# DeepakSridhar/fgdm

Hardware: AMD Instinct MI355X
Metric: 512x512 images/sec @ 50 DDIM steps, seg-ControlNet+CFG (higher is better)
Workload: dtype f16

## Files before the change

fgdm_amd/csrc/attention.hip:

```cpp
#include "common.h"
#include <type_traits>
#include <algorithm>
#include <stdlib.h>

#pragma clang diagnostic ignored "-Winline-asm"
#define ATT_THR 8.0f

template <int D>
__global__ __launch_bounds__(256) void attn_kernel(const half_t* __restrict__ Q, int ldq,
                                                   const half_t* __restrict__ K, int ldk,
                                                   const half_t* __restrict__ Vt, int ldvt,
                                                   half_t* __restrict__ O, int ldo,
                                                   int H, int T, int Tk, float sl2e) {
    constexpr int DP = (D + 15) / 16 * 16;
    constexpr int NKS = DP / 16;
    constexpr int DT = (D + 31) / 32;
    constexpr bool ONES = (DT * 32 > D);
    constexpr bool FOLD = (DP > D) && (D % 8 == 0);
    constexpr int PS = D / 16, PH = (D % 16) / 8;
    constexpr int KS = DP * 2 + 16;
    constexpr int VS = 64 * 2 + 8;
    constexpr int DC = D / 8;
    constexpr int KCH = (64 * DC + 255) / 256;
    constexpr int VCH = (D * 8 + 255) / 256;
    constexpr int KBYTES = 64 * KS, VBYTES = DT * 32 * VS;
    __shared__ __attribute__((aligned(16))) char smem[2 * (KBYTES + VBYTES)];

    const int tid = threadIdx.x, lane = tid & 63, wave = tid >> 6;
    const int lq = lane & 31, lh = lane >> 5;
    const int nqb = (T + 127) / 128;
    const int nb = gridDim.x;
    int logical;
    {
        const int bid = blockIdx.x, xcd = bid & 7, qd = nb >> 3, r = nb & 7;
        logical = (xcd < r ? xcd * (qd + 1) : r * (qd + 1) + (xcd - r) * qd) + (bid >> 3);
    }
    int qblk, b, head;
    if (Tk <= 128) {
        head = logical % H;
        const int rest = logical / H;
        qblk = rest % nqb; b = rest / nqb;
    } else {
        qblk = logical % nqb;
        const int bh = logical / nqb;
        b = bh / H; head = bh - b * H;
    }
    const int q = qblk * 128 + wave * 32 + lq;

    for (int buf = 0; buf < 2; ++buf) {
        char* Ksb = smem + buf * (KBYTES + VBYTES);
        char* Vsb = Ksb + KBYTES;
        if constexpr (DP > D) {
            for (int i = tid; i < 64 * (DP - D) / 8; i += 256) {
                const int key = i / ((DP - D) / 8), c = i % ((DP - D) / 8);
                h8 pad = (h8)(half_t)0;
                if (FOLD && c == 0) pad[0] = (half_t)1;
                *(h8*)(Ksb + key * KS + (D + c * 8) * 2) = pad;
            }
        }
        for (int i = tid; i < (DT * 32 - D) * 16; i += 256) {
            const int r = D + i / 16, c = i % 16;
            *(h4*)(Vsb + r * VS + c * 8) = (r == D) ? (h4)(half_t)1 : (h4)(half_t)0;
        }
    }

    h8 qf[NKS];
#pragma unroll
    for (int s = 0; s < NKS; ++s) {
        const int c = 16 * s + 8 * lh;
        qf[s] = (h8)(half_t)0;
        if (c < D && q < T) qf[s] = *(const h8*)(Q + ((size_t)b * T + q) * ldq + head * D + c);
        if constexpr (FOLD) {
#pragma unroll
            for (int j = 0; j < 8; ++j) qf[s][j] = (half_t)((float)qf[s][j] * sl2e);
        }
    }

    f32x16 oacc[DT];
#pragma unroll
    for (int t = 0; t < DT; ++t)
#pragma unroll
        for (int r = 0; r < 16; ++r) oacc[t][r] = 0.f;
    float m_run = FOLD ? 0.f : -INFINITY, l_run = 0.f;

    const half_t* Kb = K + (size_t)b * Tk * ldk + head * D;
    const half_t* Vb = Vt + ((size_t)b * H + head) * D * ldvt;

    const int wave_u = __builtin_amdgcn_readfirstlane(wave);
    int k_goff[KCH], k_loff[KCH], k_key[KCH], v_goff[VCH], v_loff[VCH];
#pragma unroll
    for (int u = 0; u < KCH; ++u) {
        const int i = tid + u * 256, key = i / DC, c = i - key * DC;
        k_key[u] = key; k_goff[u] = key * ldk + c * 8; k_loff[u] = key * KS + c * 16;
    }
#pragma unroll
    for (int u = 0; u < VCH; ++u) {
        const int i = tid + u * 256, r = i >> 3, c = i & 7;
        v_goff[u] = r * ldvt + c * 8; v_loff[u] = r * VS + c * 16;
    }
    h8 kreg[KCH], vreg[VCH];
    auto load_tile = [&](int k0, bool ragged) {
        const half_t* kb = Kb + (size_t)k0 * ldk;
        const half_t* vb = Vb + k0;
#pragma unroll
        for (int u = 0; u < KCH; ++u)
            if ((u * 4 + wave_u) * 64 < 64 * DC) {
                int off = k_goff[u];
                if (ragged) off += (min(k_key[u], Tk - 1 - k0) - k_key[u]) * ldk;
                kreg[u] = *(const h8*)(kb + off);
            }
#pragma unroll
        for (int u = 0; u < VCH; ++u)
            if ((u * 4 + wave_u) * 64 < D * 8) vreg[u] = *(const h8*)(vb + v_goff[u]);
    };
    auto store_tile = [&](auto bufc) {
        constexpr int buf = decltype(bufc)::value;
        char* Ksb = smem + buf * (KBYTES + VBYTES);
        char* Vsb = Ksb + KBYTES;
#pragma unroll
        for (int u = 0; u < KCH; ++u)
            if ((u * 4 + wave_u) * 64 < 64 * DC) *(h8*)(Ksb + k_loff[u]) = kreg[u];
#pragma unroll
        for (int u = 0; u < VCH; ++u)
            if ((u * 4 + wave_u) * 64 < D * 8) {
                const h8 v = vreg[u];
                h4 lo = {v[0], v[1], v[2], v[3]}, hi = {v[4], v[5], v[6], v[7]};
                *(h4*)(Vsb + v_loff[u]) = lo;
                *(h4*)(Vsb + v_loff[u] + 8) = hi;
            }
    };
    const int kfrag = lq * KS + 8 * lh * 2, vfrag = lq * VS + 4 * lh * 2;

    load_tile(0, Tk < 64);
    store_tile(std::integral_constant<int, 0>{});
    auto tile = [&](int k0, auto curc, auto nsubc) {
        constexpr int cur = decltype(curc)::value;
        constexpr int NSUB = decltype(nsubc)::value;
        const bool more = k0 + 64 < Tk;
        if (more) load_tile(k0 + 64, k0 + 128 > Tk);
        __syncthreads();
        const char* Ks = smem + cur * (KBYTES + VBYTES);
        const char* Vs = Ks + KBYTES;

        h8 kf[2][NKS];
#pragma unroll
        for (int sub = 0; sub < NSUB; ++sub)
#pragma unroll
            for (int s = 0; s < NKS; ++s) kf[sub][s] = *(const h8*)(Ks + kfrag + sub * 32 * KS + 16 * s * 2);
        __builtin_amdgcn_sched_barrier(0);
        f32x16 sacc[2];
#pragma unroll
        for (int sub = 0; sub < NSUB; ++sub) {
#pragma unroll
            for (int r = 0; r < 16; ++r) sacc[sub][r] = 0.f;
#pragma unroll
            for (int s = 0; s < NKS; ++s) sacc[sub] = __builtin_amdgcn_mfma_f32_32x32x16_f16(kf[sub][s], qf[s], sacc[sub], 0, 0, 0);
        }
        __builtin_amdgcn_sched_barrier(0);
        h4 v0f[2][2][DT], v1f[2][2][DT];
#pragma unroll
        for (int sub = 0; sub < NSUB; ++sub)
#pragma unroll
            for (int s = 0; s < 2; ++s)
#pragma unroll
                for (int t = 0; t < DT; ++t) {
                    const char* vp = Vs + vfrag + t * 32 * VS + (sub * 32 + 16 * s) * 2;
                    v0f[sub][s][t] = *(const h4*)vp;
                    v1f[sub][s][t] = *(const h4*)(vp + 16);
                }
        __builtin_amdgcn_sched_barrier(0);
        if (k0 + 64 > Tk) {
#pragma unroll
            for (int sub = 0; sub < NSUB; ++sub)
#pragma unroll
                for (int r = 0; r < 16; ++r) {
                    const int key = k0 + sub * 32 + (r & 3) + 8 * (r >> 2) + 4 * lh;
                    if (key >= Tk) sacc[sub][r] = -INFINITY;
                }
        }
        float psum = 0.f;
        if constexpr (FOLD) {
            float mx = sacc[0][0];
#pragma unroll
            for (int r = 1; r < 16; ++r) mx = fmaxf(mx, sacc[0][r]);
            if constexpr (NSUB == 2) {
#pragma unroll
                for (int r = 0; r < 16; ++r) mx = fmaxf(mx, sacc[1][r]);
            }
            mx = fmaxf(mx, __shfl_xor(mx, 32));
            const bool first = (k0 == 0);
            if (first || !__all(mx <= ATT_THR)) {
                const float m_new = first ? mx : m_run + fmaxf(mx, 0.f);
                const float m_hat = (float)(half_t)m_new;
                const float delta = m_run - m_hat;
                const float alpha = first ? 1.f : __builtin_amdgcn_exp2f(delta);
                m_run = m_hat;
#pragma unroll
                for (int t = 0; t < DT; ++t)
#pragma unroll
                    for (int r = 0; r < 16; ++r) oacc[t][r] *= alpha;
#pragma unroll
                for (int sub = 0; sub < NSUB; ++sub)
#pragma unroll
                    for (int r = 0; r < 16; ++r) sacc[sub][r] += delta;
                if (lh == PH) qf[PS][0] = (half_t)(-m_hat);
            }
#pragma unroll
            for (int sub = 0; sub < NSUB; ++sub)
#pragma unroll
                for (int r = 0; r < 16; ++r) sacc[sub][r] = __builtin_amdgcn_exp2f(sacc[sub][r]);
        } else {
        float mx = sacc[0][0];
#pragma unroll
        for (int r = 1; r < 16; ++r) mx = fmaxf(mx, sacc[0][r]);
        if constexpr (NSUB == 2) {
#pragma unroll
            for (int r = 0; r < 16; ++r) mx = fmaxf(mx, sacc[1][r]);
        }
        mx = fmaxf(mx, __shfl_xor(mx, 32)) * sl2e;
        if (!__all(mx - m_run <= ATT_THR)) {
            const float m_new = fmaxf(m_run, mx);
            const float alpha = __builtin_amdgcn_exp2f(m_run - m_new);
            m_run = m_new;
            l_run *= alpha;
#pragma unroll
            for (int t = 0; t < DT; ++t)
#pragma unroll
                for (int r = 0; r < 16; ++r) oacc[t][r] *= alpha;
        }
#pragma unroll
        for (int sub = 0; sub < NSUB; ++sub)
#pragma unroll
            for (int r = 0; r < 16; ++r) {
                const float p = __builtin_amdgcn_exp2f(sacc[sub][r] * sl2e - m_run);
                sacc[sub][r] = p;
                if constexpr (!ONES) psum += p;
            }
        }
        if constexpr (!ONES) l_run += psum;

#pragma unroll
        for (int sub = 0; sub < NSUB; ++sub) {
#pragma unroll
            for (int s = 0; s < 2; ++s) {
                h8 pf;
#pragma unroll
                for (int j = 0; j < 8; ++j) pf[j] = (half_t)sacc[sub][8 * s + j];
#pragma unroll
                for (int t = 0; t < DT; ++t) {
                    const h4 v0 = v0f[sub][s][t], v1 = v1f[sub][s][t];
                    const h8 vf = {v0[0], v0[1], v0[2], v0[3], v1[0], v1[1], v1[2], v1[3]};
                    oacc[t] = __builtin_amdgcn_mfma_f32_32x32x16_f16(vf, pf, oacc[t], 0, 0, 0);
                }
            }
        }
        if (more) store_tile(std::integral_constant<int, cur ^ 1>{});
    };
    using one_t = std::integral_constant<int, 1>;
    using two_t = std::integral_constant<int, 2>;
    for (int k0 = 0; k0 < Tk; k0 += 128) {
        if (k0 + 32 >= Tk) tile(k0, std::integral_constant<int, 0>{}, one_t{});
        else tile(k0, std::integral_constant<int, 0>{}, two_t{});
        if (k0 + 64 < Tk) {
            if (k0 + 96 >= Tk) tile(k0 + 64, std::integral_constant<int, 1>{}, one_t{});
            else tile(k0 + 64, std::integral_constant<int, 1>{}, two_t{});
        }
    }

    float l_tot;
    if constexpr (ONES) {
        constexpr int rr = D % 32;
        constexpr int reg = (rr & 3) + 4 * (rr >> 3);
        constexpr int owner_half = (rr >> 2) & 1;
        const float mine = oacc[D / 32][reg];
        const float other = __shfl_xor(mine, 32);
        l_tot = (lh == owner_half) ? mine : other;
    } else {
        l_tot = l_run + __shfl_xor(l_run, 32);
    }
    const float inv = 1.0f / l_tot;
    if (q < T) {
        half_t* op = O + ((size_t)b * T + q) * ldo + head * D;
#pragma unroll
        for (int t = 0; t < DT; ++t)
#pragma unroll
            for (int g = 0; g < 4; ++g) {
                const int dd = t * 32 + 8 * g + 4 * lh;
                if (dd < D) {
                    h4 pk = {(half_t)(oacc[t][4 * g] * inv), (half_t)(oacc[t][4 * g + 1] * inv),
                             (half_t)(oacc[t][4 * g + 2] * inv), (half_t)(oacc[t][4 * g + 3] * inv)};
                    *(h4*)(op + dd) = pk;
                }
            }
    }
}


template <int D>
__global__ __launch_bounds__(256) void attn_cross_kernel(const half_t* __restrict__ Q, int ldq,
                                                         const half_t* __restrict__ K, int ldk,
                                                         const half_t* __restrict__ Vt, int ldvt,
                                                         half_t* __restrict__ O, int ldo,
                                                         int H, int T, int Tk, float sl2e, int cpw) {
    constexpr int NS = 3, KEYS = NS * 32;
    constexpr int DP = (D + 15) / 16 * 16, NKS = DP / 16, DT = (D + 31) / 32;
    constexpr bool ONES = (DT * 32 > D);
    constexpr bool FOLD = (DP > D) && (D % 8 == 0);
    constexpr int KS = DP * 2 + 16;
    constexpr int VS = KEYS * 2 + 72;
    constexpr int DC = D / 8;
    constexpr bool RELAY = D <= 80;
    constexpr int RS = D * 2 + 8;
    constexpr int PCS = 32 * (D / 8), KP = (PCS + 63) / 64;
    __shared__ __attribute__((aligned(16))) char smem[KEYS * KS + DT * 32 * VS + (RELAY ? 4 * 32 * RS : 0)];
    char* Ks = smem;
    char* Vs = smem + KEYS * KS;

    const int tid = threadIdx.x, lane = tid & 63, wave = tid >> 6;
    const int lq = lane & 31, lh = lane >> 5;
    const int qpw = 128 * cpw;
    const int ncb = (T + qpw - 1) / qpw;
    const int nb = gridDim.x;
    int logical;
    {
        const int bid = blockIdx.x, xcd = bid & 7, qd = nb >> 3, r = nb & 7;
        logical = (xcd < r ? xcd * (qd + 1) : r * (qd + 1) + (xcd - r) * qd) + (bid >> 3);
    }
    const int head = logical % H, rest = logical / H;
    const int cblk = rest % ncb, b = rest / ncb;

    const half_t* Kb = K + (size_t)b * Tk * ldk + head * D;
    const half_t* Vb = Vt + ((size_t)b * H + head) * D * ldvt;
    constexpr int KPC = KEYS * (DP / 8), VPC = DT * 32 * (KEYS / 8);
    constexpr int KPT = (KPC + 255) / 256, VPT = (VPC + 255) / 256;
    h8 kst[KPT], vst[VPT];
#pragma unroll
    for (int u = 0; u < KPT; ++u) {
        const int i = tid + 256 * u, key = i / (DP / 8), c = i - key * (DP / 8);
        kst[u] = (h8)(half_t)0;
        if (i < KPC && c < DC) kst[u] = *(const h8*)(Kb + (size_t)min(key, Tk - 1) * ldk + c * 8);
    }
#pragma unroll
    for (int u = 0; u < VPT; ++u) {
        const int i = tid + 256 * u, r = i / (KEYS / 8), c = i - r * (KEYS / 8);
        vst[u] = (r == D) ? (h8)(half_t)1 : (h8)(half_t)0;
        if (i < VPC && r < D) vst[u] = *(const h8*)(Vb + (size_t)r * ldvt + c * 8);
    }
    char* scr = smem + KEYS * KS + DT * 32 * VS + (threadIdx.x >> 6) * 32 * RS;
    constexpr int NQ = RELAY ? KP : NKS;
    auto load_q = [&](int q0, h8 (&qr)[NQ]) {
        if constexpr (RELAY) {
#pragma unroll
            for (int u = 0; u < KP; ++u) {
                const int c = lane + 64 * u, row = c / (D / 8), ck = c - row * (D / 8);
                qr[u] = (h8)(half_t)0;
                if (c < PCS && q0 + row < T) qr[u] = *(const h8*)(Q + ((size_t)b * T + q0 + row) * ldq + head * D + ck * 8);
            }
        } else {
#pragma unroll
            for (int s2 = 0; s2 < NKS; ++s2) {
                const int c = 16 * s2 + 8 * lh;
                qr[s2] = (h8)(half_t)0;
                if (c < D && q0 + lq < T) qr[s2] = *(const h8*)(Q + ((size_t)b * T + q0 + lq) * ldq + head * D + c);
            }
        }
    };
    const int q_first = cblk * qpw + wave * 32;
    h8 qn[NQ];
    load_q(q_first, qn);
#pragma unroll
    for (int u = 0; u < KPT; ++u) {
        const int i = tid + 256 * u, key = i / (DP / 8), c = i - key * (DP / 8);
        if (i < KPC) *(h8*)(Ks + key * KS + c * 16) = kst[u];
    }
#pragma unroll
    for (int u = 0; u < VPT; ++u) {
        const int i = tid + 256 * u, r = i / (KEYS / 8), c = i - r * (KEYS / 8);
        if (i < VPC) {
            const h8 v = vst[u];
            const h4 lo = {v[0], v[1], v[2], v[3]}, hi = {v[4], v[5], v[6], v[7]};
            *(h4*)(Vs + r * VS + c * 16) = lo;
            *(h4*)(Vs + r * VS + c * 16 + 8) = hi;
        }
    }
    __syncthreads();

    const int kfrag = lq * KS + 8 * lh * 2, vfrag = lq * VS + 4 * lh * 2;
    for (int i = 0; i < cpw; ++i) {
        const int q0 = __builtin_amdgcn_readfirstlane(q_first + i * 128);
        if (q0 >= T) break;
        const int q = q0 + lq;
        h8 qf[NKS];
        if constexpr (RELAY) {
#pragma unroll
            for (int u = 0; u < KP; ++u) {
                const int c = lane + 64 * u, row = c / (D / 8), ck = c - row * (D / 8);
                if (c < PCS) {
                    const h4 lo = {qn[u][0], qn[u][1], qn[u][2], qn[u][3]}, hi = {qn[u][4], qn[u][5], qn[u][6], qn[u][7]};
                    *(h4*)(scr + row * RS + ck * 16) = lo;
                    *(h4*)(scr + row * RS + ck * 16 + 8) = hi;
                }
            }
            asm volatile("s_waitcnt lgkmcnt(0)" ::: "memory");
#pragma unroll
            for (int s2 = 0; s2 < NKS; ++s2) {
                const int c = 16 * s2 + 8 * lh;
                qf[s2] = (h8)(half_t)0;
                if (c < D) {
                    const h4 lo = *(const h4*)(scr + lq * RS + c * 2), hi = *(const h4*)(scr + lq * RS + c * 2 + 8);
                    qf[s2] = h8{lo[0], lo[1], lo[2], lo[3], hi[0], hi[1], hi[2], hi[3]};
                }
            }
            asm volatile("s_waitcnt lgkmcnt(0)" ::: "memory");
        } else {
#pragma unroll
            for (int s2 = 0; s2 < NKS; ++s2) qf[s2] = qn[s2];
        }
        if (i + 1 < cpw) load_q(q0 + 128, qn);
        if constexpr (FOLD) {
#pragma unroll
            for (int s2 = 0; s2 < NKS; ++s2)
#pragma unroll
                for (int j = 0; j < 8; ++j) qf[s2][j] = (half_t)((float)qf[s2][j] * sl2e);
        }
        f32x16 sacc[NS];
#pragma unroll
        for (int sub = 0; sub < NS; ++sub) {
#pragma unroll
            for (int r = 0; r < 16; ++r) sacc[sub][r] = 0.f;
#pragma unroll
            for (int s2 = 0; s2 < NKS; ++s2) {
                const h8 kf = *(const h8*)(Ks + kfrag + sub * 32 * KS + 16 * s2 * 2);
                sacc[sub] = __builtin_amdgcn_mfma_f32_32x32x16_f16(kf, qf[s2], sacc[sub], 0, 0, 0);
            }
        }
#pragma unroll
        for (int r = 0; r < 16; ++r) {
            const int key = (NS - 1) * 32 + (r & 3) + 8 * (r >> 2) + 4 * lh;
            if (key >= Tk) sacc[NS - 1][r] = -INFINITY;
        }
        float mx = sacc[0][0];
#pragma unroll
        for (int sub = 0; sub < NS; ++sub)
#pragma unroll
            for (int r = 0; r < 16; ++r) mx = fmaxf(mx, sacc[sub][r]);
        mx = fmaxf(mx, __shfl_xor(mx, 32));
        const float sc = FOLD ? 1.0f : sl2e;
        float psum = 0.f;
#pragma unroll
        for (int sub = 0; sub < NS; ++sub)
#pragma unroll
            for (int r = 0; r < 16; ++r) {
                const float pv = __builtin_amdgcn_exp2f((sacc[sub][r] - mx) * sc);
                sacc[sub][r] = pv;
                if constexpr (!ONES) psum += pv;
            }
        f32x16 oacc[DT];
#pragma unroll
        for (int t = 0; t < DT; ++t)
#pragma unroll
            for (int r = 0; r < 16; ++r) oacc[t][r] = 0.f;
#pragma unroll
        for (int sub = 0; sub < NS; ++sub)
#pragma unroll
            for (int s2 = 0; s2 < 2; ++s2) {
                h8 pf;
#pragma unroll
                for (int j = 0; j < 8; ++j) pf[j] = (half_t)sacc[sub][8 * s2 + j];
#pragma unroll
                for (int t = 0; t < DT; ++t) {
                    const char* vp = Vs + vfrag + t * 32 * VS + (sub * 32 + 16 * s2) * 2;
                    const h4 v0 = *(const h4*)vp, v1 = *(const h4*)(vp + 16);
                    const h8 vf = {v0[0], v0[1], v0[2], v0[3], v1[0], v1[1], v1[2], v1[3]};
                    oacc[t] = __builtin_amdgcn_mfma_f32_32x32x16_f16(vf, pf, oacc[t], 0, 0, 0);
                }
            }
        float l_tot;
        if constexpr (ONES) {
            constexpr int rr = D % 32;
            constexpr int reg = (rr & 3) + 4 * (rr >> 3);
            constexpr int owner_half = (rr >> 2) & 1;
            const float mine = oacc[D / 32][reg];
            const float other = __shfl_xor(mine, 32);
            l_tot = (lh == owner_half) ? mine : other;
        } else {
            l_tot = psum + __shfl_xor(psum, 32);
        }
        const float inv = 1.0f / l_tot;
        if constexpr (RELAY) {
#pragma unroll
            for (int t = 0; t < DT; ++t)
#pragma unroll
                for (int g = 0; g < 4; ++g) {
                    const int dd = t * 32 + 8 * g + 4 * lh;
                    if (dd < D) {
                        h4 pk = {(half_t)(oacc[t][4 * g] * inv), (half_t)(oacc[t][4 * g + 1] * inv),
                                 (half_t)(oacc[t][4 * g + 2] * inv), (half_t)(oacc[t][4 * g + 3] * inv)};
                        *(h4*)(scr + lq * RS + dd * 2) = pk;
                    }
                }
            asm volatile("s_waitcnt lgkmcnt(0)" ::: "memory");
#pragma unroll
            for (int u = 0; u < KP; ++u) {
                const int c = lane + 64 * u, row = c / (D / 8), ck = c - row * (D / 8);
                if (c < PCS && q0 + row < T) {
                    const h4 lo = *(const h4*)(scr + row * RS + ck * 16), hi = *(const h4*)(scr + row * RS + ck * 16 + 8);
                    *(h8*)(O + ((size_t)b * T + q0 + row) * ldo + head * D + ck * 8) = h8{lo[0], lo[1], lo[2], lo[3], hi[0], hi[1], hi[2], hi[3]};
                }
            }
            asm volatile("s_waitcnt lgkmcnt(0)" ::: "memory");
        } else if (q < T) {
            half_t* op = O + ((size_t)b * T + q) * ldo + head * D;
#pragma unroll
            for (int t = 0; t < DT; ++t)
#pragma unroll
                for (int g = 0; g < 4; ++g) {
                    const int dd = t * 32 + 8 * g + 4 * lh;
                    if (dd < D) {
                        h4 pk = {(half_t)(oacc[t][4 * g] * inv), (half_t)(oacc[t][4 * g + 1] * inv),
                                 (half_t)(oacc[t][4 * g + 2] * inv), (half_t)(oacc[t][4 * g + 3] * inv)};
                        *(h4*)(op + dd) = pk;
                    }
                }
        }
    }
}

template <int D>
__global__ __launch_bounds__(512) void attn_pp_kernel(const half_t* __restrict__ Q, int ldq,
                                                      const half_t* __restrict__ K, int ldk,
                                                      const half_t* __restrict__ Vt, int ldvt,
                                                      half_t* __restrict__ O, int ldo,
                                                      int H, int T, int Tk, float sl2e) {
    constexpr int DP = (D + 15) / 16 * 16, NKS = DP / 16, DT = (D + 31) / 32;
    constexpr bool ONES = (DT * 32 > D);
    constexpr bool FOLD = (DP > D) && (D % 8 == 0);
    constexpr int PS = D / 16, PH = (D % 16) / 8;
    constexpr int KS = DP * 2 + 16, VS = 64 * 2 + 8, DC = D / 8;
    constexpr int NCH = 64 * DC;
    constexpr int CH = (NCH + 511) / 512;
    constexpr int KBYTES = 64 * KS, VBYTES = DT * 32 * VS, PAIR = KBYTES + VBYTES;
    __shared__ __attribute__((aligned(16))) char smem[2 * PAIR];

    const int tid = threadIdx.x, lane = tid & 63;
    const int wave = __builtin_amdgcn_readfirstlane(tid >> 6);
    const int grp = wave >> 2;
    const int lq = lane & 31, lh = lane >> 5;
    const int nqb = (T + 255) / 256;
    const int nb = gridDim.x;
    int logical;
    {
        const int bid = blockIdx.x, xcd = bid & 7, qd = nb >> 3, r = nb & 7;
        logical = (xcd < r ? xcd * (qd + 1) : r * (qd + 1) + (xcd - r) * qd) + (bid >> 3);
    }
    const int qblk = logical % nqb, bh = logical / nqb;
    const int b = bh / H, head = bh - b * H;
    const int q = qblk * 256 + wave * 32 + lq;
    const int nt = (Tk + 63) / 64;

    for (int buf = 0; buf < 2; ++buf) {
        char* Ksb = smem + buf * PAIR;
        char* Vsb = Ksb + KBYTES;
        if constexpr (DP > D) {
            for (int i = tid; i < 64 * (DP - D) / 8; i += 512) {
                const int key = i / ((DP - D) / 8), c = i % ((DP - D) / 8);
                h8 pad = (h8)(half_t)0;
                if (FOLD && c == 0) pad[0] = (half_t)1;
                *(h8*)(Ksb + key * KS + (D + c * 8) * 2) = pad;
            }
        }
        for (int i = tid; i < (DT * 32 - D) * 16; i += 512) {
            const int r = D + i / 16, c = i % 16;
            *(h4*)(Vsb + r * VS + c * 8) = (r == D) ? (h4)(half_t)1 : (h4)(half_t)0;
        }
    }

    h8 qf[NKS];
#pragma unroll
    for (int s = 0; s < NKS; ++s) {
        const int c = 16 * s + 8 * lh;
        qf[s] = (h8)(half_t)0;
        if (c < D && q < T) qf[s] = *(const h8*)(Q + ((size_t)b * T + q) * ldq + head * D + c);
        if constexpr (FOLD) {
#pragma unroll
            for (int j = 0; j < 8; ++j) qf[s][j] = (half_t)((float)qf[s][j] * sl2e);
        }
    }
    f32x16 oacc[DT];
#pragma unroll
    for (int t = 0; t < DT; ++t)
#pragma unroll
        for (int r = 0; r < 16; ++r) oacc[t][r] = 0.f;
    float m_run = FOLD ? 0.f : -INFINITY, l_run = 0.f;

    const half_t* Kb = K + (size_t)b * Tk * ldk + head * D;
    const half_t* Vb = Vt + ((size_t)b * H + head) * D * ldvt;

    int k_goff[CH], k_loff[CH], k_key[CH], v_goff[CH], v_loff[CH];
#pragma unroll
    for (int u = 0; u < CH; ++u) {
        const int i = tid + u * 512;
        const int key = i / DC, c = i - key * DC;
        k_key[u] = key; k_goff[u] = key * ldk + c * 8; k_loff[u] = key * KS + c * 16;
        const int r = i >> 3, cv = i & 7;
        v_goff[u] = r * ldvt + cv * 8; v_loff[u] = r * VS + cv * 16;
    }
    h8 kreg[CH], vreg[CH];
    auto load_pair = [&](int kt, int vtile) {
        if (kt < nt) {
            const int k0 = kt * 64;
            const half_t* kb = Kb + (size_t)k0 * ldk;
            const bool ragged = k0 + 64 > Tk;
#pragma unroll
            for (int u = 0; u < CH; ++u)
                if ((u * 8 + wave) * 64 < NCH) {
                    int off = k_goff[u];
                    if (ragged) off += (min(k_key[u], Tk - 1 - k0) - k_key[u]) * ldk;
                    kreg[u] = *(const h8*)(kb + off);
                }
        }
        if (vtile >= 0 && vtile < nt) {
            const half_t* vb = Vb + vtile * 64;
#pragma unroll
            for (int u = 0; u < CH; ++u)
                if ((u * 8 + wave) * 64 < NCH) vreg[u] = *(const h8*)(vb + v_goff[u]);
        }
    };
    auto store_pair = [&](int kt, int vtile, int buf) {
        char* Ksb = smem + buf * PAIR;
        char* Vsb = Ksb + KBYTES;
        if (kt < nt) {
#pragma unroll
            for (int u = 0; u < CH; ++u)
                if ((u * 8 + wave) * 64 < NCH) *(h8*)(Ksb + k_loff[u]) = kreg[u];
        }
        if (vtile >= 0 && vtile < nt) {
#pragma unroll
            for (int u = 0; u < CH; ++u)
                if ((u * 8 + wave) * 64 < NCH) {
                    const h8 v = vreg[u];
                    h4 lo = {v[0], v[1], v[2], v[3]}, hi = {v[4], v[5], v[6], v[7]};
                    *(h4*)(Vsb + v_loff[u]) = lo;
                    *(h4*)(Vsb + v_loff[u] + 8) = hi;
                }
        }
    };
    auto barrier = [&]() { __syncthreads(); };
    const int kfrag = lq * KS + 8 * lh * 2, vfrag = lq * VS + 4 * lh * 2;

    f32x16 sacc[2];
    h8 pf[2][2];
    auto qk = [&](int buf) {
        const char* Ks = smem + buf * PAIR;
        h8 kf[2][NKS];
#pragma unroll
        for (int sub = 0; sub < 2; ++sub)
#pragma unroll
            for (int s = 0; s < NKS; ++s) kf[sub][s] = *(const h8*)(Ks + kfrag + sub * 32 * KS + 16 * s * 2);
        __builtin_amdgcn_sched_barrier(0);
#pragma unroll
        for (int sub = 0; sub < 2; ++sub) {
#pragma unroll
            for (int r = 0; r < 16; ++r) sacc[sub][r] = 0.f;
#pragma unroll
            for (int s = 0; s < NKS; ++s) sacc[sub] = __builtin_amdgcn_mfma_f32_32x32x16_f16(kf[sub][s], qf[s], sacc[sub], 0, 0, 0);
        }
    };
    auto pv = [&](int buf) {
        const char* Vs = smem + buf * PAIR + KBYTES;
#pragma unroll
        for (int sub = 0; sub < 2; ++sub)
#pragma unroll
            for (int s = 0; s < 2; ++s)
#pragma unroll
                for (int t = 0; t < DT; ++t) {
                    const char* vp = Vs + vfrag + t * 32 * VS + (sub * 32 + 16 * s) * 2;
                    const h4 v0 = *(const h4*)vp, v1 = *(const h4*)(vp + 16);
                    const h8 vf = {v0[0], v0[1], v0[2], v0[3], v1[0], v1[1], v1[2], v1[3]};
                    oacc[t] = __builtin_amdgcn_mfma_f32_32x32x16_f16(vf, pf[sub][s], oacc[t], 0, 0, 0);
                }
    };
    auto softmax = [&](int k0, bool first) {
// ... 264 lines not shown
        if constexpr ((ABL & 2) != 0) return;
        if (first || !__all(mx <= ATT_THR)) {
            const float m_new = first ? mx : m_run[X] + fmaxf(mx, 0.f);
            const float m_hat = (float)(half_t)m_new;
            const float delta = m_run[X] - m_hat;
            m_run[X] = m_hat;
            if (!first) {
                const float alpha = __builtin_amdgcn_exp2f(delta);
#pragma unroll
                for (int qg = 0; qg < 2; ++qg) {
                    const float aq = __shfl(alpha, 16 * qg + n16);
#pragma unroll
                    for (int t = 0; t < DT; ++t) oacc[X][t][qg] *= aq;
                }
            }
#pragma unroll
            for (int sub = 0; sub < 2; ++sub)
#pragma unroll
                for (int r = 0; r < 16; ++r) sacc[X][sub][r] += delta;
            if (h == PH) qf[X][PS][0] = (half_t)(-m_hat);
        }
    };
    auto expo = [&](int X, int sub, int r0, int r1) {
#pragma unroll
        for (int r = r0; r < r1; ++r) sacc[X][sub][r] = (ABL & 1) ? sacc[X][sub][r] : __builtin_amdgcn_exp2f(sacc[X][sub][r]);
    };
    auto pack = [&](int X, int sub) {
        unsigned pk[8];
#pragma unroll
        for (int i = 0; i < 8; ++i) {
            const h2 t2 = {(half_t)sacc[X][sub][2 * i], (half_t)sacc[X][sub][2 * i + 1]};
            pk[i] = __builtin_bit_cast(unsigned, t2);
        }
        u32x4 lo, hi;
#pragma unroll
        for (int i = 0; i < 4; ++i) {
            const auto r2 = __builtin_amdgcn_permlane16_swap(pk[i], pk[i + 4], false, false);
            lo[i] = r2[0]; hi[i] = r2[1];
        }
        pb[X][sub][0] = __builtin_bit_cast(h8, lo);
        pb[X][sub][1] = __builtin_bit_cast(h8, hi);
    };

    auto tile = [&](int kt, auto slotc) {
        constexpr int slot = decltype(slotc)::value;
        if (!(ABL & 4) && kt + 1 < nt) att_wait_vmcnt<NI>(); else att_wait_vmcnt<0>();
        __builtin_amdgcn_s_waitcnt(0xC07F);
        __builtin_amdgcn_s_barrier();
        if (!(ABL & 4) && kt + 2 < nt) issue(kt + 2, std::integral_constant<int, (slot + 2) % NSLOT>{});
        const char* sl = smem + slot * SLOT;
        const bool first = kt == 0;
#pragma unroll
        for (int sub = 0; sub < 2; ++sub)
#pragma unroll
            for (int s = 0; s < NKS; ++s) rd_k(sl, sub, s);
        ATT_SB();
#pragma unroll
        for (int sub = 0; sub < 2; ++sub)
#pragma unroll
            for (int s = 0; s < NKS; ++s) {
                qk(0, sub, s);
                if (sub * NKS + s < DT * 2) rd_v(sl, (sub * NKS + s) % DT, (sub * NKS + s) / DT);
                ATT_SB();
            }
        float mx = sacc[0][0][0];
        qk(1, 0, 0); mx = max_part(0, 0, mx); ATT_SB();
        qk(1, 0, 1); mx = max_part(0, 1, mx); ATT_SB();
        qk(1, 0, 2 % NKS); mx = max_cross(mx); ATT_SB();
#pragma unroll
        for (int s = 3; s < NKS; ++s) { qk(1, 0, s); ATT_SB(); }
        decide(0, mx, first);
        ATT_SB();
#pragma unroll
        for (int s = 0; s < NKS; ++s) {
            qk(1, 1, s);
            expo(0, 0, 16 * s / NKS, 16 * (s + 1) / NKS);
            ATT_SB();
        }
        pack(0, 0);
        ATT_SB();
        float mxb = sacc[1][0][0];
#pragma unroll
        for (int t = 0; t < DT; ++t)
#pragma unroll
            for (int qg = 0; qg < 2; ++qg) {
                const int i = t * 2 + qg, n = DT * 2;
                pv(0, 0, t, qg);
                expo(0, 1, 16 * i / n, 16 * (i + 1) / n);
                if (i == 1) mxb = max_part(1, 0, mxb);
                if (i == 3) mxb = max_part(1, 1, mxb);
                if (i == 4) mxb = max_cross(mxb);
                ATT_SB();
            }
        pack(0, 1);
        ATT_SB();
        decide(1, mxb, first);
        ATT_SB();
#pragma unroll
        for (int t = 0; t < DT; ++t)
#pragma unroll
            for (int qg = 0; qg < 2; ++qg) {
                const int i = t * 2 + qg, n = DT * 2;
                pv(0, 1, t, qg);
                expo(1, 0, 16 * i / n, 16 * (i + 1) / n);
                ATT_SB();
            }
        pack(1, 0);
        ATT_SB();
#pragma unroll
        for (int t = 0; t < DT; ++t)
#pragma unroll
            for (int qg = 0; qg < 2; ++qg) {
                const int i = t * 2 + qg, n = DT * 2;
                pv(1, 0, t, qg);
                expo(1, 1, 16 * i / n, 16 * (i + 1) / n);
                ATT_SB();
            }
        pack(1, 1);
        ATT_SB();
#pragma unroll
        for (int t = 0; t < DT; ++t)
#pragma unroll
            for (int qg = 0; qg < 2; ++qg) pv(1, 1, t, qg);
        ATT_SB();
    };
    for (int kt = 0; kt < nt; kt += NSLOT) {
        tile(kt, std::integral_constant<int, 0>{});
        if (kt + 1 < nt) tile(kt + 1, std::integral_constant<int, 1>{});
        if (kt + 2 < nt) tile(kt + 2, std::integral_constant<int, 2>{});
    }
#undef ATT_SB

    constexpr int LT = D / 16, LG = (D % 16) / 4, LR = D % 4;
#pragma unroll
    for (int X = 0; X < 2; ++X)
#pragma unroll
        for (int qg = 0; qg < 2; ++qg) {
            const float l = __shfl(oacc[X][LT][qg][LR], 16 * LG + n16);
            const float inv = 1.0f / l;
            half_t* op = O + ((size_t)b * T + q0w + 32 * X + 16 * qg + n16) * ldo + head * D;
#pragma unroll
            for (int t = 0; t < DT; ++t) {
                const int dd = 16 * t + 4 * g;
                if (dd < D) {
                    const h4 o4 = {(half_t)(oacc[X][t][qg][0] * inv), (half_t)(oacc[X][t][qg][1] * inv),
                                   (half_t)(oacc[X][t][qg][2] * inv), (half_t)(oacc[X][t][qg][3] * inv)};
                    *(h4*)(op + dd) = o4;
                }
            }
        }
}

template <int D, int NW, int ABL = 0>
__global__ __launch_bounds__(NW * 64, D <= 40 ? 2 : 1) void attn_dq32_kernel(const half_t* __restrict__ Q, int ldq,
                                                           const half_t* __restrict__ K, int ldk,
                                                           const half_t* __restrict__ Vt, int ldvt,
                                                           half_t* __restrict__ O, int ldo,
                                                           int H, int T, int Tk, float sl2e) {
    constexpr int DP = (D + 16) / 16 * 16, NKS = DP / 16;
    constexpr int DT = (D + 32) / 32;
    constexpr int DC = D / 8;
    constexpr int PS = D / 16, PH = (D % 16) / 8;
    constexpr int KROW = DC * 16, KBYTES = 64 * KROW, VDATA = D * 128, VBYTES = DT * 32 * 128, SLOT = KBYTES + VBYTES;
    constexpr int NSLOT = 3;
    constexpr int NDMA = (KBYTES + VDATA) / 1024, NI = (NDMA + NW - 1) / NW;
    static_assert(KBYTES % 1024 == 0 && VDATA % 1024 == 0 && NDMA >= NW, "whole wave-instructions per image");
    constexpr int ROT = (KROW / 4) % 8 == 4 ? 0 : DC / 2;
    static_assert(ROT == 0 || ((KROW / 4) % 16 == 8 && DC % 2 == 0), "K row stride");
    __shared__ __attribute__((aligned(1024))) char smem[NSLOT * SLOT + 64];

    const int tid = threadIdx.x, lane = tid & 63;
    const int wave = __builtin_amdgcn_readfirstlane(tid >> 6);
    const int n32 = lane & 31, h = lane >> 5;
    const int nqb = T / (NW * 64);
    const int nb = gridDim.x;
    int logical;
    {
        const int bid = blockIdx.x, xcd = bid & 7, qd = nb >> 3, r = nb & 7;
        logical = (xcd < r ? xcd * (qd + 1) : r * (qd + 1) + (xcd - r) * qd) + (bid >> 3);
    }
    const int qblk = logical % nqb, bh = logical / nqb;
    const int b = bh / H, head = bh - b * H;
    const int q0w = qblk * (NW * 64) + wave * 64;
    const int nt = Tk >> 6;

    char* const cst = smem + NSLOT * SLOT;
    if (tid < 2) {
        h8 v = (h8)(half_t)0;
        if (tid == 0) v[0] = (half_t)1;
        *(h8*)(cst + tid * 16) = v;
    }
    for (int i = tid; i < NSLOT * (DT * 32 - D) * 8; i += NW * 64) {
        const int sl_i = i / ((DT * 32 - D) * 8), rem = i - sl_i * ((DT * 32 - D) * 8), row = D + rem / 8, pc = rem & 7;
        *(h8*)(smem + sl_i * SLOT + KBYTES + row * 128 + pc * 16) = row == D ? (h8)(half_t)1 : (h8)(half_t)0;
    }

    const half_t* Kb = K + (size_t)b * Tk * ldk + head * D;
    const half_t* Vb = Vt + ((size_t)b * H + head) * D * ldvt;
    unsigned voff[NI], ldst[NI];
    bool isk[NI];
#pragma unroll
    for (int u = 0; u < NI; ++u) {
        int j = wave + NW * u;
        if (j >= NDMA) j -= NW;
        isk[u] = j < KBYTES / 1024;
        ldst[u] = (unsigned)j * 1024u;
        if (isk[u]) {
            const int L = 64 * j + lane, rp = L / DC, c = L - rp * DC;
            const int rho = rp & 31, a = rho >> 3;
            const int key = (rp & 32) + 16 * (a >> 1) + 8 * ((rho >> 2) & 1) + 4 * (a & 1) + (rho & 3);
            const int cs = (c + DC - ROT * ((rho >> 3) & 1)) % DC;
            voff[u] = (unsigned)(key * ldk + cs * 8) * 2u;
        } else {
            const int L = 64 * (j - KBYTES / 1024) + lane, d = L >> 3, x = L & 7;
            voff[u] = (unsigned)(d * ldvt + ((x ^ ((d >> 1) & 7)) * 8)) * 2u;
        }
    }
    const unsigned lds0 = (unsigned)(size_t)(__attribute__((address_space(3))) const void*)smem;
    auto issue = [&](int t, auto slotc) {
        const char* kb = (const char*)(Kb + (size_t)t * 64 * ldk);
        const char* vb = (const char*)(Vb + t * 64);
        const unsigned base = lds0 + (unsigned)decltype(slotc)::value * SLOT;
#pragma unroll
        for (int u = 0; u < NI; ++u) att_dma16(voff[u], isk[u] ? kb : vb, base + ldst[u]);
    };
    issue(0, std::integral_constant<int, 0>{});
    if (nt > 1) issue(1, std::integral_constant<int, 1>{});

    h8 qf[2][NKS];
#pragma unroll
    for (int X = 0; X < 2; ++X)
#pragma unroll
        for (int s = 0; s < NKS; ++s) {
            const int c = 16 * s + 8 * h;
            qf[X][s] = (h8)(half_t)0;
            if (c < D) qf[X][s] = *(const h8*)(Q + ((size_t)b * T + q0w + 32 * X + n32) * ldq + head * D + c);
#pragma unroll
            for (int e = 0; e < 8; ++e) qf[X][s][e] = (half_t)((float)qf[X][s][e] * sl2e);
        }
    f32x16 oacc[2][DT];
#pragma unroll
    for (int X = 0; X < 2; ++X)
#pragma unroll
        for (int t = 0; t < DT; ++t)
#pragma unroll
            for (int r = 0; r < 16; ++r) oacc[X][t][r] = 0.f;
    float m_run[2] = {0.f, 0.f};

    int k_lane[NKS];
#pragma unroll
    for (int s2 = 0; s2 < NKS; ++s2) k_lane[s2] = n32 * KROW + ((2 * s2 + h + ROT * ((n32 >> 3) & 1)) % DC) * 16;
    int v_lane[2][2];
#pragma unroll
    for (int sub = 0; sub < 2; ++sub)
#pragma unroll
        for (int s2 = 0; s2 < 2; ++s2) v_lane[sub][s2] = KBYTES + n32 * 128 + (((4 * sub + 2 * s2 + h) ^ ((n32 >> 1) & 7)) * 16);
    const char* const c_one = cst, *const c_zero = cst + 16;

    f32x16 sacc[2][2];
    h8 kf[2][NKS], vf[DT][2][2], pf[2][2][2];
    const f32x16 zero16 = {0.f, 0.f, 0.f, 0.f, 0.f, 0.f, 0.f, 0.f, 0.f, 0.f, 0.f, 0.f, 0.f, 0.f, 0.f, 0.f};
#define ATT_SB() __builtin_amdgcn_sched_barrier(0)
    auto rd_k = [&](const char* sl, int sub, int s) {
        const int ci0 = 2 * s;
        const char* p = sl + k_lane[s] + sub * 32 * KROW;
        if (ci0 + 1 >= DC) {
            const char* cp0 = ci0 < DC ? p : (ci0 == DC ? c_one : c_zero);
            const char* cp1 = ci0 + 1 == DC ? c_one : c_zero;
            p = h ? cp1 : cp0;
        }
        kf[sub][s] = *(const h8*)p;
    };
    auto rd_v = [&](const char* sl, int t, int sub, int s2) { vf[t][sub][s2] = *(const h8*)(sl + v_lane[sub][s2] + t * 32 * 128); };
    auto qk = [&](int X, int sub, int s) {
        if constexpr ((ABL & 32) != 0) { if (s == 0) asm volatile("" : "=v"(sacc[X][sub])); return; }
        sacc[X][sub] = __builtin_amdgcn_mfma_f32_32x32x16_f16(kf[sub][s], qf[X][s], s == 0 ? zero16 : sacc[X][sub], 0, 0, 0);
    };
    auto pv = [&](int X, int sub, int t, int s2) {
        if constexpr ((ABL & 16) != 0) { asm volatile("" : "+v"(oacc[X][t]) : "v"(vf[t][sub][s2]), "v"(pf[X][sub][s2])); return; }
        oacc[X][t] = __builtin_amdgcn_mfma_f32_32x32x16_f16(vf[t][sub][s2], pf[X][sub][s2], oacc[X][t], 0, 0, 0);
    };
    auto max_part = [&](int X, int sub, float mx) {
        if constexpr ((ABL & 2) != 0) return mx;
#pragma unroll
        for (int r = 0; r < 16; r += 2) mx = fmaxf(fmaxf(mx, sacc[X][sub][r]), sacc[X][sub][r + 1]);
        return mx;
    };
    auto max_cross = [&](float mx) {
        float lo = mx, hi = mx;
        asm volatile("s_nop 1\n\tv_permlane32_swap_b32 %0, %1" : "+v"(lo), "+v"(hi));
        return fmaxf(lo, hi);
    };
    auto decide = [&](int X, float mx, bool first) {
        if constexpr ((ABL & 2) != 0) return;
        if (first || !__all(mx <= ATT_THR)) {
            const float m_new = first ? mx : m_run[X] + fmaxf(mx, 0.f);
            const float m_hat = (float)(half_t)m_new;
            const float delta = m_run[X] - m_hat;
            m_run[X] = m_hat;
            if (!first) {
                const float alpha = __builtin_amdgcn_exp2f(delta);
#pragma unroll
                for (int t = 0; t < DT; ++t)
#pragma unroll
                    for (int r = 0; r < 16; ++r) oacc[X][t][r] *= alpha;
            }
#pragma unroll
            for (int sub = 0; sub < 2; ++sub)
#pragma unroll
                for (int r = 0; r < 16; ++r) sacc[X][sub][r] += delta;
            if (h == PH) qf[X][PS][0] = (half_t)(-m_hat);
        }
    };
    auto expo = [&](int X, int sub, int r0, int r1) {
#pragma unroll
        for (int r = r0; r < r1; ++r) sacc[X][sub][r] = (ABL & 1) ? sacc[X][sub][r] : __builtin_amdgcn_exp2f(sacc[X][sub][r]);
    };
    auto pack = [&](int X, int sub) {
#pragma unroll
        for (int s2 = 0; s2 < 2; ++s2)
#pragma unroll
            for (int e = 0; e < 8; ++e) pf[X][sub][s2][e] = (half_t)sacc[X][sub][8 * s2 + e];
    };
    constexpr int NPV = DT * 2;
    auto tile = [&](int kt, auto slotc) {
        constexpr int slot = decltype(slotc)::value;
        if (!(ABL & 4) && kt + 1 < nt) att_wait_vmcnt<NI>(); else att_wait_vmcnt<0>();
        __builtin_amdgcn_s_waitcnt(0xC07F);
        __builtin_amdgcn_s_barrier();
        if (!(ABL & 4) && kt + 2 < nt) issue(kt + 2, std::integral_constant<int, (slot + 2) % NSLOT>{});
        const char* sl = smem + slot * SLOT;
        const bool first = kt == 0;
#pragma unroll
        for (int sub = 0; sub < 2; ++sub)
#pragma unroll
            for (int s = 0; s < NKS; ++s) rd_k(sl, sub, s);
        ATT_SB();
#pragma unroll
        for (int sub = 0; sub < 2; ++sub)
#pragma unroll
            for (int s = 0; s < NKS; ++s) {
                const int i = sub * NKS + s;
                qk(0, sub, s);
                if (i < NPV) rd_v(sl, i / 2, 0, i & 1);
                ATT_SB();
            }
        float mx = sacc[0][0][0];
        qk(1, 0, 0); mx = max_part(0, 0, mx); ATT_SB();
        qk(1, 0, 1); mx = max_part(0, 1, mx); ATT_SB();
        qk(1, 0, 2 % NKS); mx = max_cross(mx); ATT_SB();
#pragma unroll
        for (int s = 3; s < NKS; ++s) { qk(1, 0, s); ATT_SB(); }
        decide(0, mx, first);
        ATT_SB();
#pragma unroll
        for (int s = 0; s < NKS; ++s) {
            qk(1, 1, s);
            expo(0, 0, 16 * s / NKS, 16 * (s + 1) / NKS);
            if (s < NPV) rd_v(sl, s / 2, 1, s & 1);
            ATT_SB();
        }
#pragma unroll
        for (int i = NKS; i < NPV; ++i) rd_v(sl, i / 2, 1, i & 1);
        pack(0, 0);
        ATT_SB();
        float mxb = sacc[1][0][0];
#pragma unroll
        for (int i = 0; i < NPV; ++i) {
            pv(0, 0, i / 2, i & 1);
            expo(0, 1, 16 * i / NPV, 16 * (i + 1) / NPV);
            if (i == NPV - 3) mxb = max_part(1, 0, mxb);
            if (i == NPV - 2) mxb = max_part(1, 1, mxb);
            if (i == NPV - 1) mxb = max_cross(mxb);
            ATT_SB();
        }
        pack(0, 1);
        ATT_SB();
        decide(1, mxb, first);
        ATT_SB();
#pragma unroll
        for (int i = 0; i < NPV; ++i) {
            pv(0, 1, i / 2, i & 1);
            expo(1, 0, 16 * i / NPV, 16 * (i + 1) / NPV);
            ATT_SB();
        }
        pack(1, 0);
        ATT_SB();
#pragma unroll
        for (int i = 0; i < NPV; ++i) {
            pv(1, 0, i / 2, i & 1);
            expo(1, 1, 16 * i / NPV, 16 * (i + 1) / NPV);
            ATT_SB();
        }
        pack(1, 1);
        ATT_SB();
#pragma unroll
        for (int i = 0; i < NPV; ++i) pv(1, 1, i / 2, i & 1);
        ATT_SB();
    };
    for (int kt = 0; kt < nt; kt += NSLOT) {
        tile(kt, std::integral_constant<int, 0>{});
        if (kt + 1 < nt) tile(kt + 1, std::integral_constant<int, 1>{});
        if (kt + 2 < nt) tile(kt + 2, std::integral_constant<int, 2>{});
    }
#undef ATT_SB

    constexpr int rr = D % 32, reg = (rr & 3) + 4 * (rr >> 3), owner_half = (rr >> 2) & 1;
#pragma unroll
    for (int X = 0; X < 2; ++X) {
        const float mine = oacc[X][D / 32][reg];
        const float other = __shfl_xor(mine, 32);
        const float inv = 1.0f / (h == owner_half ? mine : other);
        half_t* op = O + ((size_t)b * T + q0w + 32 * X + n32) * ldo + head * D;
#pragma unroll
        for (int t = 0; t < DT; ++t)
#pragma unroll
            for (int g4 = 0; g4 < 4; ++g4) {
                const int dd = t * 32 + 8 * g4 + 4 * h;
                if (dd < D) {
                    const h4 o4 = {(half_t)(oacc[X][t][4 * g4] * inv), (half_t)(oacc[X][t][4 * g4 + 1] * inv),
                                   (half_t)(oacc[X][t][4 * g4 + 2] * inv), (half_t)(oacc[X][t][4 * g4 + 3] * inv)};
                    *(h4*)(op + dd) = o4;
                }
            }
    }
}

int attention_launch(const half_t* Q, int ldq, const half_t* K, int ldk, const half_t* Vt, int ldvt, half_t* O,
                     int ldo, int B, int H, int T, int Tk, int d, int q_prescaled, hipStream_t s) {
    if (B <= 0 || H <= 0 || T <= 0 || Tk <= 0) return FGDM_ERR_ARG;
    if (ldvt < (Tk + 63) / 64 * 64 || (ldvt & 7) || (ldq & 7) || (ldk & 7) || (ldo & 3)) return FGDM_ERR_ARG;
    const float sl2e = q_prescaled ? 1.0f : 1.4426950408889634f / sqrtf((float)d);
    static const bool pp_on = !(getenv("FGDM_ATTN_PP") && atoi(getenv("FGDM_ATTN_PP")) == 0);
    static const int dq = getenv("FGDM_ATTN_DQ") ? atoi(getenv("FGDM_ATTN_DQ")) : 3;
    if (dq > 0 && d == 40 && T % 256 == 0 && Tk % 64 == 0 && Tk >= 128 && (size_t)64 * ldk * 2 < (1u << 31) &&
        (size_t)d * ldvt * 2 < (1u << 31)) {
        const dim3 gridq((T / 256) * H * B), blockq(256);
        static const int abl = getenv("FGDM_ATTN_ABL") ? atoi(getenv("FGDM_ATTN_ABL")) : 0;
        if (abl) {
            switch (abl + (dq == 3 ? 1000 : 0)) {
#define ATT_ABL_CASE(v) case v: FGDM_LAUNCH((attn_dq_kernel<40, 4, v>), gridq, blockq, 0, s, Q, ldq, K, ldk, Vt, ldvt, O, ldo, H, T, Tk, sl2e); break; \
                        case 1000 + v: FGDM_LAUNCH((attn_dq32_kernel<40, 4, v>), gridq, blockq, 0, s, Q, ldq, K, ldk, Vt, ldvt, O, ldo, H, T, Tk, sl2e); break;
                ATT_ABL_CASE(1) ATT_ABL_CASE(2) ATT_ABL_CASE(3) ATT_ABL_CASE(4) ATT_ABL_CASE(16) ATT_ABL_CASE(32) ATT_ABL_CASE(48) ATT_ABL_CASE(51) ATT_ABL_CASE(7)
#undef ATT_ABL_CASE
                default: return FGDM_ERR_ARG;
            }
            return hipGetLastError() == hipSuccess ? FGDM_OK : FGDM_ERR_HIP;
        }
        if (dq == 1) FGDM_LAUNCH((attn_dq_kernel<40, 4>), gridq, blockq, 0, s, Q, ldq, K, ldk, Vt, ldvt, O, ldo, H, T, Tk, sl2e);
        else FGDM_LAUNCH((attn_dq32_kernel<40, 4>), gridq, blockq, 0, s, Q, ldq, K, ldk, Vt, ldvt, O, ldo, H, T, Tk, sl2e);
        return hipGetLastError() == hipSuccess ? FGDM_OK : FGDM_ERR_HIP;
    }
    static const int dq80 = getenv("FGDM_ATTN_DQ80") ? atoi(getenv("FGDM_ATTN_DQ80")) : 1;
    if (dq80 > 0 && d == 80 && T % 256 == 0 && Tk % 64 == 0 && Tk >= 128 && (size_t)64 * ldk * 2 < (1u << 31) &&
        (size_t)d * ldvt * 2 < (1u << 31)) {
        const dim3 gridq((T / 256) * H * B), blockq(256);
        FGDM_LAUNCH((attn_dq32_kernel<80, 4>), gridq, blockq, 0, s, Q, ldq, K, ldk, Vt, ldvt, O, ldo, H, T, Tk, sl2e);
        return hipGetLastError() == hipSuccess ? FGDM_OK : FGDM_ERR_HIP;
    }
    if (pp_on && T >= 256 && Tk >= 256 && (d == 40 || d == 80)) {
        const dim3 grid2(((T + 255) / 256) * H * B), block2(512);
        if (d == 40) FGDM_LAUNCH(attn_pp_kernel<40>, grid2, block2, 0, s, Q, ldq, K, ldk, Vt, ldvt, O, ldo, H, T, Tk, sl2e);
        else FGDM_LAUNCH(attn_pp_kernel<80>, grid2, block2, 0, s, Q, ldq, K, ldk, Vt, ldvt, O, ldo, H, T, Tk, sl2e);
        return hipGetLastError() == hipSuccess ? FGDM_OK : FGDM_ERR_HIP;
    }
    static const int cross = getenv("FGDM_ATTN_CROSS") ? atoi(getenv("FGDM_ATTN_CROSS")) : 4;
    if (cross > 0 && Tk > 64 && Tk <= 96 && ldvt >= 96 && T >= 128) {
        const int cpw = std::min(cross, T / 128);
        const dim3 gridc(((T + 128 * cpw - 1) / (128 * cpw)) * H * B), blockc(256);
        switch (d) {
            case 40: FGDM_LAUNCH(attn_cross_kernel<40>, gridc, blockc, 0, s, Q, ldq, K, ldk, Vt, ldvt, O, ldo, H, T, Tk, sl2e, cpw); break;
            case 80: FGDM_LAUNCH(attn_cross_kernel<80>, gridc, blockc, 0, s, Q, ldq, K, ldk, Vt, ldvt, O, ldo, H, T, Tk, sl2e, cpw); break;
            case 160: FGDM_LAUNCH(attn_cross_kernel<160>, gridc, blockc, 0, s, Q, ldq, K, ldk, Vt, ldvt, O, ldo, H, T, Tk, sl2e, cpw); break;
            default: return FGDM_ERR_ARG;
        }
        return hipGetLastError() == hipSuccess ? FGDM_OK : FGDM_ERR_HIP;
    }
    const dim3 grid(((T + 127) / 128) * H * B), block(256);
    switch (d) {
        case 40: FGDM_LAUNCH(attn_kernel<40>, grid, block, 0, s, Q, ldq, K, ldk, Vt, ldvt, O, ldo, H, T, Tk, sl2e); break;
        case 80: FGDM_LAUNCH(attn_kernel<80>, grid, block, 0, s, Q, ldq, K, ldk, Vt, ldvt, O, ldo, H, T, Tk, sl2e); break;
        case 160: FGDM_LAUNCH(attn_kernel<160>, grid, block, 0, s, Q, ldq, K, ldk, Vt, ldvt, O, ldo, H, T, Tk, sl2e); break;
        default: return FGDM_ERR_ARG;
    }
    return hipGetLastError() == hipSuccess ? FGDM_OK : FGDM_ERR_HIP;
}
```

fgdm_amd/csrc/common.h:

```cpp
#pragma once
#include <hip/hip_runtime.h>
#include <stdint.h>

typedef _Float16 half_t;
typedef _Float16 h8 __attribute__((ext_vector_type(8)));
typedef _Float16 h4 __attribute__((ext_vector_type(4)));
typedef _Float16 h2 __attribute__((ext_vector_type(2)));
typedef float f32x16 __attribute__((ext_vector_type(16)));
typedef float f32x4 __attribute__((ext_vector_type(4)));

__device__ __forceinline__ float gelu_f(float x) {
    const float z = fminf(fabsf(x), 6.0f);
    float p = -4.7132482596e-04f;
    p = __builtin_fmaf(p, z, 7.0652551839e-03f);
    p = __builtin_fmaf(p, z, -5.1762067461e-02f);
    p = __builtin_fmaf(p, z, -4.6008771426e-01f);
    p = __builtin_fmaf(p, z, -1.1507295505e+00f);
    p = __builtin_fmaf(p, z, -4.8959157159e-05f - 1.0f);
    const float t = __builtin_amdgcn_exp2f(p);
    return __builtin_fmaf(fabsf(x), 0.5f - t, 0.5f * x);
}

typedef float f32x2 __attribute__((ext_vector_type(2)));
__device__ __forceinline__ f32x2 gelu2_f(f32x2 x) {
    const f32x2 ax = {fabsf(x[0]), fabsf(x[1])};
    const f32x2 z = {fminf(ax[0], 6.0f), fminf(ax[1], 6.0f)};
    auto c = [](float k) { return f32x2{k, k}; };
    f32x2 p = c(-4.7132482596e-04f);
    p = __builtin_elementwise_fma(p, z, c(7.0652551839e-03f));
    p = __builtin_elementwise_fma(p, z, c(-5.1762067461e-02f));
    p = __builtin_elementwise_fma(p, z, c(-4.6008771426e-01f));
    p = __builtin_elementwise_fma(p, z, c(-1.1507295505e+00f));
    p = __builtin_elementwise_fma(p, z, c(-4.8959157159e-05f - 1.0f));
    const f32x2 t = {__builtin_amdgcn_exp2f(p[0]), __builtin_amdgcn_exp2f(p[1])};
    return __builtin_elementwise_fma(ax, c(0.5f) - t, c(0.5f) * x);
}

__device__ __forceinline__ float silu_f(float x, float k = 1.0f) {
    return x * __builtin_amdgcn_rcpf(1.0f + __builtin_amdgcn_exp2f(-1.4426950408889634f * k * x));
}

#define FGDM_OK 0
#define FGDM_ERR_ARG -1
#define FGDM_ERR_HIP -2
#define FGDM_ERR_STATE -3
#define FGDM_ERR_NOMEM -4

enum IgemmMode { IG_LINEAR = 0, IG_CONV3 = 1, IG_CONV3_S2 = 2, IG_CONV3_UP2 = 3, IG_CONV3_S2_BR = 4 };
enum IgemmAct { ACT_NONE = 0, ACT_SILU = 1, ACT_RELU = 2, ACT_GEGLU = 3, ACT_QGELU = 4  };
enum IgemmOut { OUT_F16 = 0, OUT_F32 = 1, OUT_F32_NCHW = 2, OUT_F16_T = 3 };

struct IgemmArgs {
    const half_t* A0;
    const half_t* A1;
    const half_t* Wt;
    const float* bias;
    const float* rowvec;
    const half_t* resid;
    void* out;
    const half_t* zero;
    int C0, C1;
    int B, H, W;
    int Ho, Wo;
    int M, N;
    int K;
    int mode, act, out_kind;
    int ld_out, ld_res;
    int rv_stride;
    int rows_per_sample;
    float scale;
    int force_cfg;
    int splitk;
    float* ws;
    int debug;
    const float* ln_stats;
    const float* ln_u;
    int ln_slots;
    float ln_eps;
    float* stats_out;
    void* out2;
    int split_n, out_kind2, ld_out2;
};

int igemm_launch(const IgemmArgs& a, hipStream_t s);
void igemm_set_force_cfg(int cfg);
void igemm_set_twin_layers(bool on);
void igemm_set_pair_hint(int mult);
int igemm2_launch(const IgemmArgs& a, int cfg, hipStream_t s);
int igemm_stats_slots(const IgemmArgs& a);
int row_stats_slots(int C);
int row_stats_launch(const half_t* x, int rows, int C, float* stats , hipStream_t s);
int igemm_splitk_factor(const IgemmArgs& a);
int igemm_splitk_reduce(const IgemmArgs& a, hipStream_t s);
size_t igemm_npad(int n);

void groupnorm_set_group(bool on);
int groupnorm_launch(const half_t* x0, int C0, const half_t* x1, int C1, int B, int HW,
                     const float* gamma, const float* beta, float eps, int silu,
                     half_t* out, float* ws , hipStream_t s);
size_t groupnorm_ws_floats(int B, int HW);
int layernorm_launch(const half_t* x, int rows, int C, const float* gamma, const float* beta, float eps,
                     half_t* out, hipStream_t s);

int attention_launch(const half_t* Q, int ldq, const half_t* K, int ldk, const half_t* Vt, int ldvt,
                     half_t* O, int ldo, int B, int H, int T, int Tk, int d, int q_prescaled, hipStream_t s);

int nchw_f32_to_nhwc_f16(const float* x, half_t* y, int B, int C, int HW, int Cpad, hipStream_t s);
int f32_to_f16(const float* x, half_t* y, size_t n, hipStream_t s);
int silu_f32_to_f16(const float* x, half_t* y, size_t n, hipStream_t s);
int nhwc_f16_to_nchw_f32(const half_t* x, float* y, int B, int C, int HW, hipStream_t s);
int im2col3x3(const half_t* x, half_t* A, int B, int H, int W, int C, int stride, int Kpad, hipStream_t s);
int avgpool2(const half_t* x, half_t* y, int B, int H, int W, int C, hipStream_t s);
int add_f16(const half_t* a, const half_t* b, half_t* y, size_t n, hipStream_t s);
int add_f16_to_f32(const float* a, const half_t* b, float* y, size_t n, hipStream_t s);
int timestep_embed(const int64_t* t, const float* t_float, half_t* y, int B, int dim, int rows_pad, hipStream_t s);
int vae_prequant(const float* z, const float* wb, float scale, half_t* y, int B, int HW, hipStream_t s);
int vae_moments(const float* h, const float* wb, float* moments, int B, int HW, hipStream_t s);
int posterior_sample(const float* moments, const float* noise, float scale, float* z, int B, int zc, int HW, hipStream_t s);
int softmax_rows(const float* S, half_t* P, int rows, int cols, hipStream_t s);
int image_to_u8(const float* x, uint8_t* y, int B, int C, int HW, int mode, hipStream_t s);
int resize_linear_u8(const uint8_t* src, uint8_t* dst, int B, int H, int W, int C, int Ho, int Wo, hipStream_t s);
int u8_to_hint(const uint8_t* src, float* dst, int B, int HW, int C, hipStream_t s);
int embed_tokens(const int64_t* ids, const float* tok, const float* pos, float* out, int rows, int T, int W, int vocab,
                 hipStream_t s);
int layernorm32_launch(const float* x, int rows, int C, const float* gamma, const float* beta, float eps, half_t* out16,
                       float* out32, hipStream_t s);
int f16_to_f32(const half_t* x, float* y, size_t n, hipStream_t s);
int small_attention_launch(const half_t* qkv, int ld, int koff, int voff, half_t* out, int ldo, int B, int heads, int T,
                           int d, int causal, hipStream_t s);
int transpose_pad_keys(const half_t* v, half_t* vt, int B, int Tk, int C, int Tkpad, hipStream_t s);
int ddim_step(const float* x, const float* e_cond, const float* e_uncond, float cfg_scale,
              float a_t, float a_prev, float sigma_t, float sqrt_one_minus_at, const float* noise,
              float* x_prev, float* pred_x0, float* e_out, size_t n, hipStream_t s);
int plms_combine(const float* e_t, const float* e1, const float* e2, const float* e3, int order,
                 float* e_prime, size_t n, hipStream_t s);
int axpby(const float* a, float ca, const float* b, float cb, float* y, size_t n, hipStream_t s);
int mask_blend(const float* a, const float* b, const float* m, float* y, size_t n, hipStream_t s);
int ancestral_step(const float* x, const float* eps, float sqrt_recip, float sqrt_recipm1, float coef1, float coef2,
                   float std, const float* noise, float* out, size_t n, hipStream_t s);

#define HIP_TRY(expr) do { hipError_t _e = (expr); if (_e != hipSuccess) return FGDM_ERR_HIP; } while (0)

#include <functional>
#define FGDM_MAX_GROUP 5
typedef int (*IgemmGroupFn)(const IgemmArgs* const* a, int n, unsigned grid_x, hipStream_t s);
bool fgdm_recording();
void fgdm_record(std::function<int(hipStream_t)> run, const void* pair_key = nullptr, IgemmGroupFn pair = nullptr,
                 const IgemmArgs* ia = nullptr, unsigned grid_x = 0);
#define FGDM_GROUP_BLOB 96
typedef int (*GenericGroupFn)(const void* const* args, int n, unsigned grid_x, hipStream_t s);
void fgdm_record_generic(std::function<int(hipStream_t)> run, const void* key, GenericGroupFn fn, const void* args, size_t nbytes,
                         unsigned grid_x, unsigned long long shape);
#define FGDM_LAUNCH(kernel, grid, block, smem, stream, ...)                                                                  \
    do {                                                                                                                     \
        if (fgdm_recording()) {                                                                                              \
            fgdm_record([=](hipStream_t fgdm_s_) -> int {                                                                    \
                hipLaunchKernelGGL(kernel, grid, block, smem, fgdm_s_, __VA_ARGS__);                                         \
                return hipGetLastError() == hipSuccess ? FGDM_OK : FGDM_ERR_HIP;                                             \
            });                                                                                                              \
        } else {                                                                                                             \
            hipLaunchKernelGGL(kernel, grid, block, smem, stream, __VA_ARGS__);                                              \
        }                                                                                                                    \
    } while (0)
```

fgdm_amd/csrc/engine.hip:

```cpp
#include "common.h"
#include "../../include/fgdm.h"

#include <algorithm>
#include <array>
#include <cmath>
#include <cstdlib>
#include <cstdio>
#include <cstring>
#include <map>
#include <memory>
#include <string>
#include <unordered_map>
#include <vector>

namespace {

struct Arena {
    struct Blk { char* p; size_t sz; bool free; };
    std::vector<std::vector<Blk>> slabs;
    std::vector<char*> bases;
    size_t slab_bytes = (size_t)4 << 30;
    size_t in_use = 0, peak = 0;
    bool scoped = false;
    std::vector<void*> live;
// ... 63 lines not shown
    float* bias = nullptr;
    int N = 0, K = 0;
    bool im2col = false;
    int cin_pad = 0;
    int k_real = 0;
    float* ln_u = nullptr;
    float ln_eps = 1e-5f;
};
struct NormW { float* g = nullptr; float* b = nullptr; int C = 0; };

enum LType { L_CONV, L_RES, L_ATTN, L_DOWN, L_UP };
struct Layer {
    LType type = L_CONV;
    int cin = 0, cout = 0, heads = 0;
    bool down = false;
    std::string pre;
    GemmW conv;
    NormW gn1, gn2; GemmW c1, c2, skip; int emb_off = 0;
    NormW gn, ln1, ln2, ln3;
    GemmW pin, pout, qkv1, o1, q2, k2, v2, o2, ffp, ffo;
};
typedef std::vector<Layer> Block;

struct AdapterBlk { int ic = 0, oc = 0; bool down = false; std::string pre; GemmW in_conv, b1, b2; };

struct Net {
    std::string prefix;
    bool control = false;
    GemmW time0, time2, emb_all;
    int emb_total = 0;
    std::vector<Block> input, output;
    Block middle;
    NormW out_gn; GemmW out_conv;
    bool has_adapter = false;
    GemmW ad_conv_in; std::vector<AdapterBlk> ad_body;
    std::vector<GemmW> xad_conv_in; std::vector<std::vector<AdapterBlk>> xad_body;
    Tensor xad_sum[4]; bool xad_valid = false;
    bool time_adapter = false; Block tad_body;
    std::vector<GemmW> zero_convs; GemmW mid_out;
    std::vector<int> zero_ch;
    GemmW hint_convs[8];
    Tensor guided;
};

struct VRes { int cin = 0, cout = 0; std::string pre; NormW n1, n2; GemmW c1, c2, nin; };
struct VLevel { std::vector<VRes> blocks; bool up = false; std::string up_pre; GemmW upconv; };
struct VAttn { std::string pre; NormW norm; GemmW q, k, v, o; };
struct VDown { std::vector<VRes> blocks; bool down = false; std::string down_pre; GemmW downconv; };
struct VEnc {
    bool on = false;
    GemmW conv_in, conv_out;
    std::vector<VDown> levels;
    VRes mid1, mid2;
    VAttn attn;
    NormW norm_out;
    float* qc = nullptr;
};
struct Vae {
    bool on = false, packed = false;
    std::string prefix;
    int top = 0, factor = 1;
    GemmW conv_in, conv_out;
    VRes mid1, mid2;
    VAttn attn;
    std::vector<VLevel> levels;
    NormW norm_out;
    float* pq = nullptr;
    VEnc enc;
};

struct ClipLayer { std::string pre; NormW ln1, ln2; GemmW qkv, o, fc1, fc2; };
struct Clip {
    bool on = false, packed = false;
    std::string prefix;
    float* tok = nullptr;
    float* pos = nullptr;
    std::vector<ClipLayer> layers;
    NormW final_ln;
};

static int roundup(int x, int m) { return (x + m - 1) / m * m; }

enum ProfClass { PC_IGEMM = 0, PC_ATTN = 1, PC_NORM = 2, PC_ELEM = 3, PC_COUNT = 4 };
struct RecOp {
    enum Kind { RUN, PROF_BEGIN, PROF_END } kind = RUN;
    std::function<int(hipStream_t)> run;
    const void* pair_key = nullptr;
    IgemmGroupFn pair = nullptr;
    IgemmArgs ia{};
    unsigned grid_x = 0;
    GenericGroupFn gfn = nullptr;
    unsigned long long gshape = 0;
    alignas(8) char gargs[FGDM_GROUP_BLOB] = {0};
    int cls = 0;
    double w = 0, bytes = 0;
    char tag[56] = {0};
};
thread_local std::vector<RecOp>* g_rec = nullptr;

struct Prof {
    bool on = false;
    std::vector<hipEvent_t> pool;
    size_t used = 0;
    struct Rec { int cls; size_t e0, e1; double w; char tag[56]; };
    std::vector<Rec> recs;
    double work[PC_COUNT] = {0, 0, 0, 0};
    double bytes[PC_COUNT] = {0, 0, 0, 0};
    hipEvent_t get() {
        if (used == pool.size()) { hipEvent_t e; if (hipEventCreate(&e) != hipSuccess) return nullptr; pool.push_back(e); }
        return pool[used++];
    }
    int stride = 1;
    long counter = 0;
    bool armed = false;
    void begin(int cls, hipStream_t s, double w, const char* tag = "", double nbytes = 0.0) {
        if (g_rec) {
            if (!on) return;
            RecOp o; o.kind = RecOp::PROF_BEGIN; o.cls = cls; o.w = w; o.bytes = nbytes;
            snprintf(o.tag, sizeof(o.tag), "%s", tag);
            g_rec->push_back(std::move(o));
            return;
        }
        armed = false;
        if (!on || (counter++ % stride) != 0) return;
        armed = true;
        hipEvent_t e = get();
        if (!e) return;
        (void)hipEventRecord(e, s);
        Rec r{cls, used - 1, 0, w, {0}};
        snprintf(r.tag, sizeof(r.tag), "%s", tag);
        recs.push_back(r);
        work[cls] += w;
        bytes[cls] += nbytes;
    }
    void end(hipStream_t s) {
        if (g_rec) {
            if (!on) return;
            RecOp o; o.kind = RecOp::PROF_END;
            g_rec->push_back(std::move(o));
            return;
        }
        if (!on || !armed || recs.empty()) return;
        armed = false;
        hipEvent_t e = get();
        if (!e) return;
        (void)hipEventRecord(e, s);
        recs.back().e1 = used - 1;
    }
};

}

bool fgdm_recording() { return g_rec != nullptr; }
void fgdm_record(std::function<int(hipStream_t)> run, const void* pair_key, IgemmGroupFn pair, const IgemmArgs* ia, unsigned grid_x) {
    RecOp o;
    o.run = std::move(run);
    o.pair_key = pair_key; o.pair = pair; o.grid_x = grid_x;
    if (ia) o.ia = *ia;
    g_rec->push_back(std::move(o));
}

void fgdm_record_generic(std::function<int(hipStream_t)> run, const void* key, GenericGroupFn fn, const void* args, size_t nbytes,
                         unsigned grid_x, unsigned long long shape) {
    RecOp o;
    o.run = std::move(run);
    if (fn && args && nbytes <= FGDM_GROUP_BLOB) {
        o.pair_key = key; o.gfn = fn; o.grid_x = grid_x; o.gshape = shape;
        memcpy(o.gargs, args, nbytes);
    }
    g_rec->push_back(std::move(o));
}

#define CHK0(x) do { int _rc0 = (x); if (_rc0 != FGDM_OK) return _rc0; } while (0)
struct fgdm_engine {
    fgdm_config cfg{};
    int device = -1;
    bool device_ready = false, finalized = false;
    std::string err;
    std::vector<std::string> order;
    std::unordered_map<std::string, ParamSlot> params;
    Net unet;
    std::vector<Net> cns;
    Vae vae;
    Clip clip;
    struct CtxKV { Tensor k, vt; };
    std::unordered_map<const Layer*, CtxKV> ctx_cache;
    int ctx_B = 0, ctx_T = 0;
    Arena arena;
    half_t* zero = nullptr;
    std::unordered_map<std::string, std::vector<void*>> weight_allocs;
    std::unordered_map<std::string, bool> comp_dirty, comp_packed;
    std::string cur_comp;
    bool ln_fold = true;
    hipStream_t s = nullptr;
    std::vector<std::unique_ptr<Arena>> cn_arena;
    Arena* ar = &arena;
    hipStream_t s2 = nullptr;
    hipEvent_t ev_fork = nullptr, ev_join = nullptr;
    bool twin_streams = false;
    bool pair_launch = true;
    int group_max = FGDM_MAX_GROUP;
    bool gn_group = true;
    long paired_launches = 0, replayed_launches = 0, paired_problems = 0;
    struct Deferred { const GemmW* w; Tensor src; int idx; float scale; Arena* owner; };
    Prof prof;

    int fail(int code, const std::string& m) { err = m; return code; }

    void reg(const std::string& name, std::vector<int64_t> shape) {
        order.push_back(name);
        params[name].shape = std::move(shape);
    }
    void reg_wb(const std::string& pre, std::vector<int64_t> wshape) {
        const int64_t n = wshape[0];
        reg(pre + ".weight", std::move(wshape));
        reg(pre + ".bias", {n});
    }
    void reg_res(const std::string& p, int cin, int cout, int temb) {
        reg_wb(p + "in_layers.0", {cin});
        reg_wb(p + "in_layers.2", {cout, cin, 3, 3});
        reg_wb(p + "emb_layers.1", {cout, temb});
        reg_wb(p + "out_layers.0", {cout});
        reg_wb(p + "out_layers.3", {cout, cout, 3, 3});
        if (cin != cout) reg_wb(p + "skip_connection", {cout, cin, 1, 1});
    }
    void reg_attn(const std::string& p, int ch, int ctx) {
        reg_wb(p + "norm", {ch});
        reg_wb(p + "proj_in", {ch, ch, 1, 1});
        const std::string t = p + "transformer_blocks.0.";
        reg(t + "attn1.to_q.weight", {ch, ch});
        reg(t + "attn1.to_k.weight", {ch, ch});
        reg(t + "attn1.to_v.weight", {ch, ch});
        reg_wb(t + "attn1.to_out.0", {ch, ch});
        reg_wb(t + "ff.net.0.proj", {8 * ch, ch});
        reg_wb(t + "ff.net.2", {ch, 4 * ch});
        reg(t + "attn2.to_q.weight", {ch, ch});
        reg(t + "attn2.to_k.weight", {ch, ctx});
        reg(t + "attn2.to_v.weight", {ch, ctx});
        reg_wb(t + "attn2.to_out.0", {ch, ch});
        reg_wb(t + "norm1", {ch});
        reg_wb(t + "norm2", {ch});
        reg_wb(t + "norm3", {ch});
        reg_wb(p + "proj_out", {ch, ch, 1, 1});
    }
    void reg_block(const std::string& pre, Block& blk, int temb, int ctx) {
        for (size_t j = 0; j < blk.size(); ++j) {
            Layer& l = blk[j];
            l.pre = pre + std::to_string(j) + ".";
            switch (l.type) {
                case L_CONV: reg_wb(l.pre.substr(0, l.pre.size() - 1), {l.cout, l.cin, 3, 3}); break;
                case L_RES: reg_res(l.pre, l.cin, l.cout, temb); break;
                case L_ATTN: reg_attn(l.pre, l.cin, ctx); break;
                case L_DOWN: reg_wb(l.pre + "op", {l.cin, l.cin, 3, 3}); break;
                case L_UP: reg_wb(l.pre + "conv", {l.cin, l.cin, 3, 3}); break;
            }
        }
    }
    static Layer mk(LType t, int cin, int cout, int heads = 0) {
        Layer l; l.type = t; l.cin = cin; l.cout = cout; l.heads = heads; return l;
    }
    bool in_ares(int ds) const {
        for (int i = 0; i < cfg.n_attention_resolutions; ++i) if (cfg.attention_resolutions[i] == ds) return true;
        return false;
    }
    void build_net(Net& n, const std::string& prefix, bool control, int adapter_kind) {
        const bool adapter = adapter_kind == 1;
        n.prefix = prefix; n.control = control; n.has_adapter = adapter_kind != 0; n.time_adapter = adapter_kind == 2;
        const int mc = cfg.model_channels, temb = 4 * mc, ctx = cfg.context_dim, heads = cfg.num_heads;
        reg_wb(prefix + "time_embed.0", {temb, mc});
        reg_wb(prefix + "time_embed.2", {temb, temb});
        if (adapter) {
            static const int chs[4] = {320, 640, 1280, 1280};
            const std::string ap = prefix + "adapter.";
            for (int i = 0; i < 4; ++i)
                for (int j = 0; j < 2; ++j) {
                    AdapterBlk b;
                    b.down = (i != 0 && j == 0);
                    b.ic = b.down ? chs[i - 1] : chs[i];
                    b.oc = chs[i];
                    b.pre = ap + "body." + std::to_string(i * 2 + j) + ".";
                    if (b.ic != b.oc) reg_wb(b.pre + "in_conv", {b.oc, b.ic, 1, 1});
                    reg_wb(b.pre + "block1", {b.oc, b.oc, 3, 3});
                    reg_wb(b.pre + "block2", {b.oc, b.oc, 1, 1});
                    n.ad_body.push_back(b);
                }
            reg_wb(ap + "conv_in", {chs[0], cfg.in_channels, 3, 3});
            const int nx = control ? 0 : cfg.n_extra_adapters;
            n.xad_conv_in.resize(nx); n.xad_body.resize(nx);
            for (int kk = 0; kk < nx; ++kk) {
                const std::string xp = prefix + "adapters." + std::to_string(kk) + ".";
                for (int i = 0; i < 4; ++i)
                    for (int j = 0; j < 2; ++j) {
                        AdapterBlk b;
                        b.down = (i != 0 && j == 0);
                        b.ic = b.down ? chs[i - 1] : chs[i];
                        b.oc = chs[i];
                        b.pre = xp + "body." + std::to_string(i * 2 + j) + ".";
                        if (b.ic != b.oc) reg_wb(b.pre + "in_conv", {b.oc, b.ic, 1, 1});
                        reg_wb(b.pre + "block1", {b.oc, b.oc, 3, 3});
                        reg_wb(b.pre + "block2", {b.oc, b.oc, 1, 1});
                        n.xad_body[kk].push_back(b);
                    }
                reg_wb(xp + "conv_in", {chs[0], cfg.in_channels, 3, 3});
            }
        }
        if (n.time_adapter) {
            static const int chs[4] = {320, 640, 1280, 1280};
            const std::string ap = prefix + "adapter.";
            for (int i = 0; i < 4; ++i)
                for (int j = 0; j < 2; ++j) {
                    const bool down = (i != 0 && j == 0);
                    Layer l = mk(L_RES, down ? chs[i - 1] : chs[i], chs[i]);
                    l.down = down;
                    l.pre = ap + "body." + std::to_string(i * 2 + j) + ".";
                    reg_res(l.pre, l.cin, l.cout, temb);
                    n.tad_body.push_back(l);
                }
            reg_wb(ap + "conv_in", {chs[0], cfg.in_channels, 3, 3});
        }
        std::vector<int> chans;
        int ch = mc, ds = 1;
        n.input.push_back({mk(L_CONV, cfg.in_channels, mc)});
        chans.push_back(mc);
        for (int level = 0; level < cfg.n_levels; ++level) {
            const int mult = cfg.channel_mult[level];
            for (int r = 0; r < cfg.num_res_blocks; ++r) {
                Block b{mk(L_RES, ch, mult * mc)};
                ch = mult * mc;
                if (in_ares(ds)) b.push_back(mk(L_ATTN, ch, ch, heads));
                n.input.push_back(b);
                chans.push_back(ch);
            }
            if (level != cfg.n_levels - 1) {
                n.input.push_back({mk(L_DOWN, ch, ch)});
                chans.push_back(ch);
                ds *= 2;
            }
        }
        n.middle = {mk(L_RES, ch, ch), mk(L_ATTN, ch, ch, heads), mk(L_RES, ch, ch)};
        for (size_t i = 0; i < n.input.size(); ++i) reg_block(prefix + "input_blocks." + std::to_string(i) + ".", n.input[i], temb, ctx);
        if (control) {
            for (size_t i = 0; i < n.input.size(); ++i) {
                const int zc = n.input[i].back().type == L_DOWN ? n.input[i].back().cin : n.input[i][0].cout;
                n.zero_ch.push_back(zc);
                reg_wb(prefix + "zero_convs." + std::to_string(i) + ".0", {zc, zc, 1, 1});
            }
            static const int hc[7] = {16, 16, 32, 32, 96, 96, 256};
            int prev = cfg.hint_channels;
            for (int k = 0; k < 8; ++k) {
                const int oc = k < 7 ? hc[k] : mc;
                reg_wb(prefix + "input_hint_block." + std::to_string(2 * k), {oc, prev, 3, 3});
                prev = oc;
            }
            reg_block(prefix + "middle_block.", n.middle, temb, ctx);
            reg_wb(prefix + "middle_block_out.0", {ch, ch, 1, 1});
// ... 880 lines not shown
        for (Tensor& t : unet.xad_sum) { if (t.p) (void)hipFree(t.p); t = Tensor{}; }
        unet.xad_valid = false;
    }
    int set_adapter_conds(const float* const* conds, int nc, int B, int H, int W) {
        if (!finalized) return fail(FGDM_ERR_STATE, "weights not finalized");
        Net& n = unet;
        drop_adapter_conds();
        if (nc == 0) return FGDM_OK;
        if (nc < 0 || nc > (int)n.xad_body.size() || !conds) return fail(FGDM_ERR_ARG, "more conds than extra adapters (n_extra_adapters)");
        if (B <= 0 || (H & 7) || (W & 7)) return fail(FGDM_ERR_ARG, "latent size must be divisible by 8 for the adapter");
        for (int kk = 0; kk < nc; ++kk) {
            Tensor c4 = talloc(B, H, W, 4), f[4];
            if (!c4.p) return fail(FGDM_ERR_NOMEM, "workspace");
            if (nchw_f32_to_nhwc_f16(conds[kk], c4.p, B, 4, H * W, 4, s) != FGDM_OK) return fail(FGDM_ERR_HIP, "layout kernel");
            CHK(adapter_run(n.xad_conv_in[kk], n.xad_body[kk], c4, f));
            tfree(c4);
            for (int i = 0; i < 4; ++i) {
                Tensor& acc = n.xad_sum[i];
                if (kk == 0) {
                    acc = f[i];
                    if (hipMalloc(&acc.p, acc.numel() * sizeof(half_t)) != hipSuccess) return fail(FGDM_ERR_NOMEM, "hipMalloc (adapter cache)");
                    HIP_TRY(hipMemcpyAsync(acc.p, f[i].p, acc.numel() * sizeof(half_t), hipMemcpyDeviceToDevice, s));
                } else if (add_f16(acc.p, f[i].p, acc.p, acc.numel(), s) != FGDM_OK) {
                    return fail(FGDM_ERR_HIP, "add kernel");
                }
                tfree(f[i]);
            }
        }
        n.xad_valid = true;
        return FGDM_OK;
    }

    int time_adapter_fwd(Net& n, const Tensor& x4, const EmbCtx& ec, Tensor feats[4]) {
        Tensor cur;
        CHK(conv3(n.ad_conv_in, x4, nullptr, 1, false, Epi{}, &cur));
        for (size_t k = 0; k < n.tad_body.size(); ++k) {
            Tensor y;
            CHK(res_fwd(n.tad_body[k], cur, nullptr, ec, &y));
            bool keep = false;
            for (int f = 0; f < 4; ++f) if (feats[f].p == cur.p) keep = true;
            if (!keep) tfree(cur);
            cur = y;
            if (k % 2 == 1) feats[k / 2] = cur;
        }
        return FGDM_OK;
    }

    int run_block(const std::string& prefix, const float* x, int C, const float* x_skip, int Cs, const float* emb,
                  const float* ctx, int B, int H, int W, float* out, int64_t cap, int64_t* out_numel) {
        if (!finalized) return fail(FGDM_ERR_STATE, "weights not finalized");
        if (B <= 0 || H <= 0 || W <= 0 || C <= 0) return fail(FGDM_ERR_ARG, "bad shape");
        Net* net = nullptr;
        const Block* blk = nullptr;
        auto scan = [&](Net& n) {
            auto chk = [&](const Block& b) {
                if (b.empty() || blk) return;
                const std::string& lp = b[0].pre;
                if (lp.size() >= 2 && lp.compare(0, lp.size() - 2, prefix) == 0 && lp.size() - 2 == prefix.size()) { blk = &b; net = &n; }
            };
            for (auto& b : n.input) chk(b);
            chk(n.middle);
            for (auto& b : n.output) chk(b);
        };
        scan(unet);
        for (auto& n : cns) scan(n);
        Block single;
        if (!blk) {
            auto scan1 = [&](Net& n) {
                auto chk = [&](const Block& b) { for (const Layer& l : b) if (single.empty() && l.pre == prefix) { single.push_back(l); net = &n; } };
                for (auto& b : n.input) chk(b);
                chk(n.middle);
                for (auto& b : n.output) chk(b);
            };
            scan1(unet);
            for (auto& n : cns) scan1(n);
            if (!single.empty()) blk = &single;
        }
        const bool adapter = !blk && unet.has_adapter && !unet.time_adapter && prefix == unet.prefix + "adapter.";
        if (!blk && !adapter) return fail(FGDM_ERR_ARG, "fgdm_run_block: no such block: " + prefix);
        const int HW = H * W;
        auto emit = [&](const Tensor& t, int64_t& off) -> int {
            if (off + (int64_t)t.numel() > cap) return fail(FGDM_ERR_ARG, "fgdm_run_block: output buffer too small");
            if (nhwc_f16_to_nchw_f32(t.p, out + off, t.B, t.C, t.H * t.W, s) != FGDM_OK) return fail(FGDM_ERR_HIP, "layout kernel");
            off += (int64_t)t.numel();
            return FGDM_OK;
        };
        int64_t off = 0;
        Tensor xin = talloc(B, H, W, C);
        if (!xin.p) return fail(FGDM_ERR_NOMEM, "workspace");
        if (nchw_f32_to_nhwc_f16(x, xin.p, B, C, HW, C, s) != FGDM_OK) return fail(FGDM_ERR_HIP, "layout kernel");
        if (adapter) {
            if (C != 4) return fail(FGDM_ERR_ARG, "adapter input has 4 channels");
            Tensor fa[4];
            CHK(adapter_fwd(unet, xin, fa));
            for (int i = 0; i < 4; ++i) { CHK(emit(fa[i], off)); tfree(fa[i]); }
            tfree(xin);
            if (out_numel) *out_numel = off;
            return FGDM_OK;
        }
        Tensor xsk, ctx16;
        if (x_skip) {
            xsk = talloc(B, H, W, Cs);
            if (!xsk.p) return fail(FGDM_ERR_NOMEM, "workspace");
            if (nchw_f32_to_nhwc_f16(x_skip, xsk.p, B, Cs, HW, Cs, s) != FGDM_OK) return fail(FGDM_ERR_HIP, "layout kernel");
        }
        if ((*blk)[0].cin != C + (x_skip ? Cs : 0) || (C & 63) || (x_skip && (Cs & 63)))
            return fail(FGDM_ERR_ARG, "fgdm_run_block: channel count does not match the block");
        bool needs_ctx = false, needs_emb = false;
        for (const Layer& l : *blk) { needs_ctx |= l.type == L_ATTN; needs_emb |= l.type == L_RES; }
        if ((needs_ctx && !ctx) || (needs_emb && !emb)) return fail(FGDM_ERR_ARG, "fgdm_run_block: this block needs ctx / emb");
        if (needs_ctx) {
            ctx16 = talloc(B, 1, 77, cfg.context_dim);
            if (!ctx16.p) return fail(FGDM_ERR_NOMEM, "workspace");
            if (f32_to_f16(ctx, ctx16.p, ctx16.numel(), s) != FGDM_OK) return fail(FGDM_ERR_HIP, "convert kernel");
        }
        float* emb_all = nullptr;
        if (needs_emb) {
            const int temb = 4 * cfg.model_channels;
            Tensor e2 = talloc(1, 1, B, temb);
            emb_all = (float*)ar->alloc((size_t)B * net->emb_total * sizeof(float));
            if (!e2.p || !emb_all) return fail(FGDM_ERR_NOMEM, "workspace");
            if (silu_f32_to_f16(emb, e2.p, e2.numel(), s) != FGDM_OK) return fail(FGDM_ERR_HIP, "silu kernel");
            { Epi e; e.out_kind = OUT_F32; e.out = emb_all; e.ld_out = net->emb_total; e.rps = 1; CHK(linear(net->emb_all, e2, e, nullptr)); }
            tfree(e2);
        }
        EmbCtx ec{emb_all, net->emb_total};
        Tensor y;
        CHK(block_fwd(*blk, xin, false, x_skip ? &xsk : nullptr, ec, ctx16, nullptr, &y));
        CHK(emit(y, off));
        tfree(y); tfree(xin);
        if (xsk.p) tfree(xsk);
        if (ctx16.p) tfree(ctx16);
        if (emb_all) ar->release(emb_all);
        if (out_numel) *out_numel = off;
        return FGDM_OK;
    }

    int ensure_device() {
        if (device_ready) return FGDM_OK;
        if (hipSetDevice(device) != hipSuccess) return fail(FGDM_ERR_HIP, "hipSetDevice failed (no GPU?)");
        if (hipMalloc(&zero, 4096) != hipSuccess || hipMemset(zero, 0, 4096) != hipSuccess) return fail(FGDM_ERR_HIP, "hipMalloc failed");
        if (cfg.workspace_bytes > 0) arena.slab_bytes = (size_t)cfg.workspace_bytes;
        device_ready = true;
        return FGDM_OK;
    }

    int run_op(RecOp& o) {
        switch (o.kind) {
            case RecOp::PROF_BEGIN: prof.begin(o.cls, s, o.w, o.tag, o.bytes); return FGDM_OK;
            case RecOp::PROF_END: prof.end(s); return FGDM_OK;
            default: ++replayed_launches; return o.run(s);
        }
    }
    struct Unit { size_t first, last; long launch; };
    static Unit unit_at(std::vector<RecOp>& v, size_t i) {
        if (v[i].kind == RecOp::PROF_BEGIN && i + 2 < v.size() + 0 && v[i + 1].kind == RecOp::RUN && v[i + 2].kind == RecOp::PROF_END)
            return Unit{i, i + 2, (v[i + 1].pair || v[i + 1].gfn) ? (long)(i + 1) : -1};
        if (v[i].kind == RecOp::RUN) return Unit{i, i, (v[i].pair || v[i].gfn) ? (long)i : -1};
        return Unit{i, i, -1};
    }
    int run_unit(std::vector<RecOp>& v, const Unit& u) {
        for (size_t k = u.first; k <= u.last; ++k) CHK(run_op(v[k]));
        return FGDM_OK;
    }
    int replay_group(std::vector<std::vector<RecOp>*> L) {
        constexpr int LOOK = 24;
        while (L.size() > FGDM_MAX_GROUP) {
            std::vector<RecOp>& v = *L.back();
            for (size_t i = 0; i < v.size();) { const Unit u = unit_at(v, i); CHK(run_unit(v, u)); i = u.last + 1; }
            L.pop_back();
        }
        std::vector<size_t> at(L.size(), 0);
        for (size_t lead = 0; lead < L.size(); ++lead) {
            std::vector<RecOp>& A = *L[lead];
            while (at[lead] < A.size()) {
                const Unit ua = unit_at(A, at[lead]);
                size_t who[FGDM_MAX_GROUP];
                Unit un[FGDM_MAX_GROUP];
                int n = 0;
                if (ua.launch >= 0) {
                    who[n] = lead; un[n++] = ua;
                    for (size_t m = lead + 1; m < L.size(); ++m) {
                        std::vector<RecOp>& B = *L[m];
                        size_t jj = at[m];
                        for (int d = 0; d < LOOK && jj < B.size(); ++d) {
                            const Unit u = unit_at(B, jj);
                            if (u.launch >= 0 && B[u.launch].pair_key == A[ua.launch].pair_key && B[u.launch].grid_x == A[ua.launch].grid_x &&
                                B[u.launch].gshape == A[ua.launch].gshape) {
                                who[n] = m; un[n++] = u;
                                break;
                            }
                            jj = u.last + 1;
                        }
                    }
                }
                if (n < 2) { CHK(run_unit(A, ua)); at[lead] = ua.last + 1; continue; }
                for (int k = 1; k < n; ++k) {
                    std::vector<RecOp>& B = *L[who[k]];
                    while (at[who[k]] < un[k].first) { const Unit u = unit_at(B, at[who[k]]); CHK(run_unit(B, u)); at[who[k]] = u.last + 1; }
                }
                const IgemmArgs* av[FGDM_MAX_GROUP];
                const void* gv[FGDM_MAX_GROUP];
                double w = 0.0, bytes = 0.0;
                const RecOp* br = nullptr;
                for (int k = 0; k < n; ++k) {
                    std::vector<RecOp>& B = *L[who[k]];
                    av[k] = &B[un[k].launch].ia;
                    gv[k] = B[un[k].launch].gargs;
                    if (un[k].first != un[k].last) { w += B[un[k].first].w; bytes += B[un[k].first].bytes; if (!br) br = &B[un[k].first]; }
                }
                if (br) prof.begin(br->cls, s, w, br->tag, bytes);
                if (A[ua.launch].pair) CHK(A[ua.launch].pair(av, n, A[ua.launch].grid_x, s));
                else CHK(A[ua.launch].gfn(gv, n, A[ua.launch].grid_x, s));
                if (br) prof.end(s);
                ++paired_launches; ++replayed_launches; paired_problems += n;
                for (int k = 0; k < n; ++k) at[who[k]] = un[k].last + 1;
            }
        }
        return FGDM_OK;
    }

    int zero_conv_into(const GemmW& zw, const Tensor& src, Tensor& dst, float scale) {
        Epi e;
        e.scale = scale;
        if (src.B * 2 == dst.B) {
            for (int half = 0; half < 2; ++half) {
                half_t* d = dst.p + (size_t)half * (dst.numel() / 2);
                e.resid = d; e.ld_res = dst.C; e.out = d; e.ld_out = dst.C;
                CHK(linear(zw, src, e, nullptr));
            }
            return FGDM_OK;
        }
        e.resid = dst.p; e.ld_res = dst.C; e.out = dst.p; e.ld_out = dst.C;
        return linear(zw, src, e, nullptr);
    }

    int controlnet_fwd(Net& n, const Tensor& x4, const int64_t* t, const float* tf, const Tensor& ctx16, const float* scales,
                       std::vector<Tensor>* hs, Tensor* h_mid, bool only_mid, float* out32, int64_t out_cap, bool pairs = false,
                       std::vector<Deferred>* defer = nullptr) {
        const int B = x4.B;
        struct TwinGuard { TwinGuard() { igemm_set_twin_layers(true); } ~TwinGuard() { igemm_set_twin_layers(false); } } twin_guard;
        const bool shared = pairs && !out32 && 2 * n.guided.B == B && n.input.size() > 1;
        if (!n.guided.p) return fail(FGDM_ERR_STATE, "fgdm_set_hint has not been called for this ControlNet");
        if (!(n.guided.B == B || 2 * n.guided.B == B) || n.guided.H != x4.H || n.guided.W != x4.W)
            return fail(FGDM_ERR_ARG, "cached hint does not match the batch / latent size");
        float* emb = nullptr;
        CHK(embed(n, t, tf, B, &emb));
        EmbCtx ec{emb, n.emb_total};
        Tensor h;
        int64_t off = 0;
        auto zero_conv = [&](const GemmW& zw, const Tensor& src, int idx) -> int {
            Epi e;
            if (out32) {
                const int64_t cnt = (int64_t)src.numel();
                if (off + cnt > out_cap) return fail(FGDM_ERR_ARG, "fgdm_controlnet: output buffer too small");
                e.out_kind = OUT_F32_NCHW; e.out = out32 + off; e.ld_out = src.H * src.W;
                off += cnt;
                return linear(zw, src, e, nullptr);
            }
            if (idx >= 0 && only_mid) return FGDM_OK;
            e.scale = scales ? scales[idx < 0 ? (int)n.input.size() : idx] : 1.f;
            if (defer) { defer->push_back({&zw, src, idx, e.scale, ar}); return FGDM_OK; }
            return zero_conv_into(zw, src, idx < 0 ? *h_mid : (*hs)[idx], e.scale);
        };
        for (size_t i = 0; i < n.input.size(); ++i) {
            Tensor nxt;
            if (i == 0) {
                const Layer& l = n.input[0][0];
                if (shared) {
                    Tensor xh = x4; xh.B = B / 2;
                    CHK(block_fwd(n.input[0], xh, false, nullptr, ec, ctx16, n.guided.p, &nxt));
                } else if (n.guided.B == B) {
                    CHK(block_fwd(n.input[0], x4, false, nullptr, ec, ctx16, n.guided.p, &nxt));
                } else {
                    nxt = talloc(B, x4.H, x4.W, l.cout);
                    if (!nxt.p) return fail(FGDM_ERR_NOMEM, "workspace");
                    for (int half = 0; half < 2; ++half) {
                        Tensor xs = x4; xs.B = B / 2; xs.p = x4.p + (size_t)half * xs.numel();
                        Epi e; e.resid = n.guided.p; e.ld_res = l.cout;
                        e.out = nxt.p + (size_t)half * (nxt.numel() / 2); e.ld_out = l.cout;
                        CHK(conv3(l.conv, xs, nullptr, 1, false, e, nullptr));
                    }
                }
            } else if (shared && i == 1) {
                CHK(block_fwd_shared(n.input[1], h, !defer, ec, ctx16, &nxt));
            } else {
                CHK(block_fwd(n.input[i], h, !defer, nullptr, ec, ctx16, nullptr, &nxt));
            }
            h = nxt;
            CHK(zero_conv(n.zero_convs[i], h, (int)i));
        }
        Tensor m;
        CHK(block_fwd(n.middle, h, !defer, nullptr, ec, ctx16, nullptr, &m));
        CHK(zero_conv(n.mid_out, m, -1));
        if (!defer) tfree(m);
        ar->release(emb);
        return FGDM_OK;
    }

    int apply_model(const float* x, const int64_t* t, const float* tf, const float* ctx, const float* pcond,
                    const float* scales, int B, int H, int W, int flags, float* eps_out) {
        if (!finalized) return fail(FGDM_ERR_STATE, "weights not finalized");
        if (B <= 0 || H <= 0 || W <= 0) return fail(FGDM_ERR_ARG, "bad shape");
        Net& n = unet;
        const int HW = H * W;
        Tensor x4 = talloc(B, H, W, 4), ctx16;
        if (ctx) ctx16 = talloc(B, 1, 77, cfg.context_dim);
        else if (ctx_B != B) return fail(FGDM_ERR_STATE, "ctx is NULL but no context of this batch size was registered (fgdm_set_context)");
        if (!x4.p || (ctx && !ctx16.p)) return fail(FGDM_ERR_NOMEM, "workspace");
        if (nchw_f32_to_nhwc_f16(x, x4.p, B, 4, HW, 4, s) != FGDM_OK) return fail(FGDM_ERR_HIP, "layout kernel");
        if (ctx && f32_to_f16(ctx, ctx16.p, ctx16.numel(), s) != FGDM_OK) return fail(FGDM_ERR_HIP, "convert kernel");
        float* emb = nullptr;
        CHK(embed(n, t, tf, B, &emb));
        EmbCtx ec{emb, n.emb_total};

        const bool use_adapter = n.has_adapter && !(flags & FGDM_FLAG_USE_ORIGINAL);
        const bool pairs = (flags & FGDM_FLAG_CFG_PAIRS) && (B % 2 == 0) && n.input.size() > 1;
        const int Bs = pairs ? B / 2 : B;
        Tensor x4s = x4; x4s.B = Bs;
        Tensor fa[4];
        if (use_adapter) {
            if (pcond) {
                Tensor p4 = talloc(Bs, H, W, 4);
                if (!p4.p) return fail(FGDM_ERR_NOMEM, "workspace");
                if (nchw_f32_to_nhwc_f16(pcond, p4.p, Bs, 4, HW, 4, s) != FGDM_OK) return fail(FGDM_ERR_HIP, "layout kernel");
                CHK(n.time_adapter ? time_adapter_fwd(n, p4, ec, fa) : adapter_fwd(n, p4, fa));
                tfree(p4);
            } else {
                CHK(n.time_adapter ? time_adapter_fwd(n, x4s, ec, fa) : adapter_fwd(n, x4s, fa));
            }
        }
        const bool with_cn = !cns.empty() && !(flags & FGDM_FLAG_NO_CONTROL);
        const bool twin = twin_streams && with_cn && s2 && !(flags & FGDM_FLAG_ONLY_MID_CONTROL);
        std::vector<Deferred> deferred;
        const bool paired = pair_launch && with_cn && !twin && !(flags & FGDM_FLAG_ONLY_MID_CONTROL);
        std::vector<std::vector<RecOp>> rec_cn(paired ? cns.size() : 0);
        std::vector<RecOp> rec_un;
        struct RecGuard { ~RecGuard() { g_rec = nullptr; igemm_set_pair_hint(1); } } rec_guard;
        if (paired) {
            static const bool fat = !(getenv("FGDM_PAIR_FAT_TILES") && atoi(getenv("FGDM_PAIR_FAT_TILES")) == 0);
            if (fat) igemm_set_pair_hint(std::min<int>(group_max, 1 + (int)cns.size()));
            groupnorm_set_group(gn_group);
            int rc = FGDM_OK;
            for (size_t c = 0; c < cns.size() && rc == FGDM_OK; ++c) {
                ar = cn_arena[c].get();
                g_rec = &rec_cn[c];
                rc = controlnet_fwd(cns[c], x4, t, tf, ctx16, scales ? scales + 13 * c : nullptr, nullptr, nullptr, false, nullptr, 0, pairs,
                                    &deferred);
            }
            g_rec = nullptr;
            ar = &arena;
            if (rc != FGDM_OK) return rc;
            g_rec = &rec_un;
        }
        if (twin) {
            if (hipEventRecord(ev_fork, s) != hipSuccess || hipStreamWaitEvent(s2, ev_fork, 0) != hipSuccess) return fail(FGDM_ERR_HIP, "stream fork");
            hipStream_t main_s = s;
            s = s2; ar = cn_arena[0].get();
            int rc = FGDM_OK;
            for (size_t c = 0; c < cns.size() && rc == FGDM_OK; ++c)
                rc = controlnet_fwd(cns[c], x4, t, tf, ctx16, scales ? scales + 13 * c : nullptr, nullptr, nullptr, false, nullptr, 0, pairs,
                                    &deferred);
            s = main_s; ar = &arena;
            if (rc != FGDM_OK) return rc;
            if (hipEventRecord(ev_join, s2) != hipSuccess) return fail(FGDM_ERR_HIP, "stream join");
        }
        struct TwinOff { ~TwinOff() { igemm_set_twin_layers(false); } } twin_off;
        igemm_set_twin_layers(with_cn);
        std::vector<Tensor> hs;
        Tensor h;
        int k = 0;
        Tensor h0s;
        for (size_t i = 0; i < n.input.size(); ++i) {
            Tensor nxt;
            if (pairs && i == 0) {
                CHK(block_fwd(n.input[0], x4s, false, nullptr, ec, ctx16, nullptr, &h0s));
                CHK(dup_rows(h0s, &nxt));
            } else if (pairs && i == 1) {
                CHK(block_fwd_shared(n.input[1], h0s, true, ec, ctx16, &nxt));
            } else {
                CHK(block_fwd(n.input[i], i == 0 ? x4 : h, false, nullptr, ec, ctx16, nullptr, &nxt));
            }
            if (use_adapter && (i + 1) % 3 == 0) {
                if (k >= 4 || fa[k].numel() * (size_t)(B / Bs) != nxt.numel()) return fail(FGDM_ERR_ARG, "adapter feature shape mismatch (latent size must be divisible by 8)");
                for (int half = 0; half < B / Bs; ++half) {
                    half_t* dst = nxt.p + (size_t)half * fa[k].numel();
                    if (n.xad_valid) {
                        if (n.xad_sum[k].numel() != nxt.numel()) return fail(FGDM_ERR_ARG, "registered adapter conds do not match this batch / latent size");
                        const half_t* xs = n.xad_sum[k].p + (size_t)half * fa[k].numel();
                        if (add_f16(dst, xs, dst, fa[k].numel(), s) != FGDM_OK) return fail(FGDM_ERR_HIP, "add kernel");
                    }
                    if (add_f16(dst, fa[k].p, dst, fa[k].numel(), s) != FGDM_OK) return fail(FGDM_ERR_HIP, "add kernel");
                }
                tfree(fa[k]);
                ++k;
            }
            h = nxt;
            hs.push_back(h);
        }
        Tensor hm;
        CHK(block_fwd(n.middle, h, false, nullptr, ec, ctx16, nullptr, &hm));
        igemm_set_twin_layers(false);
        if (paired) {
            g_rec = nullptr;
            igemm_set_pair_hint(1);
            std::vector<std::vector<RecOp>*> lists{&rec_un};
            for (size_t c = 0; c < rec_cn.size(); ++c) {
                if ((int)lists.size() == group_max) { CHK(replay_group(lists)); lists.clear(); }
                lists.push_back(&rec_cn[c]);
            }
            CHK(replay_group(lists));
        }
        if (twin || paired) {
            if (twin && hipStreamWaitEvent(s, ev_join, 0) != hipSuccess) return fail(FGDM_ERR_HIP, "stream join");
            for (const Deferred& d : deferred) CHK(zero_conv_into(*d.w, d.src, d.idx < 0 ? hm : hs[d.idx], d.scale));
            for (Deferred& d : deferred) { d.owner->release(d.src.p); d.src.p = nullptr; }
        } else if (with_cn) {
            for (size_t c = 0; c < cns.size(); ++c)
                CHK(controlnet_fwd(cns[c], x4, t, tf, ctx16, scales ? scales + 13 * c : nullptr, &hs, &hm,
                                   (flags & FGDM_FLAG_ONLY_MID_CONTROL) != 0, nullptr, 0, pairs));
        }
        h = hm;
        for (size_t i = 0; i < n.output.size(); ++i) {
            Tensor skip = hs.back();
            hs.pop_back();
            Tensor nxt;
            CHK(block_fwd(n.output[i], h, true, &skip, ec, ctx16, nullptr, &nxt));
            tfree(skip);
            h = nxt;
        }
        Tensor g;
        CHK(gnorm(n.out_gn, h, nullptr, 1e-5f, true, &g));
        tfree(h);
        { Epi e; e.out_kind = OUT_F32_NCHW; e.out = eps_out; e.ld_out = HW; CHK(conv3(n.out_conv, g, nullptr, 1, false, e, nullptr)); }
        tfree(g);
        tfree(x4);
        if (ctx16.p) tfree(ctx16);
        ar->release(emb);
        return FGDM_OK;
    }

    int clip_encode(const int64_t* ids, int B, int T, float* out) {
        if (!clip.on) return fail(FGDM_ERR_STATE, "engine was created without a text encoder (clip_layers = 0)");
        if (!clip.packed) return fail(FGDM_ERR_STATE, "weights not finalized");
        if (B <= 0 || T <= 0 || T > cfg.clip_max_len) return fail(FGDM_ERR_ARG, "bad shape (T must be <= clip_max_len)");
        const int W = cfg.clip_width, rows = B * T;
        Tensor n, qkv, a, f;
        float* h = (float*)ar->alloc((size_t)rows * W * sizeof(float));
        float* h2 = (float*)ar->alloc((size_t)rows * W * sizeof(float));
        if (!h || !h2) return fail(FGDM_ERR_NOMEM, "workspace");
        if (embed_tokens(ids, clip.tok, clip.pos, h, rows, T, W, cfg.clip_vocab, s) != FGDM_OK) return fail(FGDM_ERR_HIP, "embedding kernel");
        auto ln32 = [&](const NormW& nw, const float* src, Tensor* dst) -> int {
            *dst = talloc(1, 1, rows, W);
            if (!dst->p) return fail(FGDM_ERR_NOMEM, "workspace");
            return layernorm32_launch(src, rows, W, nw.g, nw.b, 1e-5f, dst->p, nullptr, s) == FGDM_OK ? FGDM_OK : fail(FGDM_ERR_HIP, "layernorm");
        };
        for (const ClipLayer& l : clip.layers) {
            CHK(ln32(l.ln1, h, &n));
            CHK(linear(l.qkv, n, Epi{}, &qkv));
            tfree(n);
            a = talloc(1, 1, rows, W);
            if (!a.p) return fail(FGDM_ERR_NOMEM, "workspace");
            if (small_attention_launch(qkv.p, 3 * W, W, 2 * W, a.p, W, B, cfg.clip_heads, T, W / cfg.clip_heads, 1, s) != FGDM_OK)
                return fail(FGDM_ERR_HIP, "text attention kernel");
            tfree(qkv);
            Tensor br;
            CHK(linear(l.o, a, Epi{}, &br));
            tfree(a);
            if (add_f16_to_f32(h, br.p, h2, br.numel(), s) != FGDM_OK) return fail(FGDM_ERR_HIP, "add kernel");
            tfree(br);
            CHK(ln32(l.ln2, h2, &n));
            { Epi e; e.act = ACT_QGELU; CHK(linear(l.fc1, n, e, &f)); }
            tfree(n);
            CHK(linear(l.fc2, f, Epi{}, &br));
            tfree(f);
            if (add_f16_to_f32(h2, br.p, h, br.numel(), s) != FGDM_OK) return fail(FGDM_ERR_HIP, "add kernel");
            tfree(br);
        }
        if (layernorm32_launch(h, rows, W, clip.final_ln.g, clip.final_ln.b, 1e-5f, nullptr, out, s) != FGDM_OK) return fail(FGDM_ERR_HIP, "layernorm");
        ar->release(h); ar->release(h2);
        return FGDM_OK;
    }

    int vres_fwd(const VRes& r, const Tensor& x, Tensor* out) {
        Tensor g1, h, g2, sk;
        CHK(gnorm(r.n1, x, nullptr, 1e-6f, true, &g1));
        CHK(conv3(r.c1, g1, nullptr, 1, false, Epi{}, &h));
        tfree(g1);
        CHK(gnorm(r.n2, h, nullptr, 1e-6f, true, &g2));
        tfree(h);
        Epi e2;
        if (r.cin != r.cout) { CHK(linear(r.nin, x, Epi{}, &sk)); e2.resid = sk.p; e2.ld_res = sk.C; }
        else { e2.resid = x.p; e2.ld_res = x.C; }
        CHK(conv3(r.c2, g2, nullptr, 1, false, e2, out));
        tfree(g2);
// ... 51 lines not shown
            CHK(vres_fwd(v.mid1, h, &t)); tfree(h); h = t;
            CHK(vattn_fwd(v.attn, h, &t)); tfree(h); h = t;
            CHK(vres_fwd(v.mid2, h, &t)); tfree(h); h = t;
            for (const VLevel& lv : v.levels) {
                for (const VRes& r : lv.blocks) { CHK(vres_fwd(r, h, &t)); tfree(h); h = t; }
                if (lv.up) { CHK(conv3(lv.upconv, h, nullptr, 1, true, Epi{}, &t)); tfree(h); h = t; }
            }
            Tensor g;
            CHK(gnorm(v.norm_out, h, nullptr, 1e-6f, true, &g));
            tfree(h);
            { Epi e; e.out_kind = OUT_F32_NCHW; e.out = out + (size_t)b0 * out_per_img; e.ld_out = g.H * g.W;
              CHK(conv3(v.conv_out, g, nullptr, 1, false, e, nullptr)); }
            tfree(g);
        }
        return FGDM_OK;
    }

    int vae_encode(const float* image, int B, int H, int W, float* moments) {
        if (!vae.on || !vae.enc.on) return fail(FGDM_ERR_STATE, "engine was created without a first-stage encoder (vae_encoder = 0)");
        if (!vae.packed) return fail(FGDM_ERR_STATE, "weights not finalized");
        const VEnc& en = vae.enc;
        const int f = vae.factor;
        if (B <= 0 || H <= 0 || W <= 0 || H % f || W % f || (((H / f) * (W / f)) & 63))
            return fail(FGDM_ERR_ARG, "first-stage encoder: H and W must be multiples of " + std::to_string(f) + " and (H/" + std::to_string(f) +
                                      ")*(W/" + std::to_string(f) + ") a multiple of 64 (smallest image 64 x 64)");
        const int hw = (H / f) * (W / f), zc2 = 2 * cfg.vae_z_channels;
        const size_t big = (size_t)H * W * cfg.vae_ch * sizeof(half_t) * 8;
        const int chunk = (int)std::max<size_t>(1, std::min<size_t>((size_t)B, ((size_t)3 << 30) / std::max<size_t>(big, 1)));
        for (int b0 = 0; b0 < B; b0 += chunk) {
            const int nb = std::min(chunk, B - b0);
            Tensor x4 = talloc(nb, H, W, en.conv_in.cin_pad), h, t;
            if (!x4.p) return fail(FGDM_ERR_NOMEM, "workspace");
            if (nchw_f32_to_nhwc_f16(image + (size_t)b0 * 3 * H * W, x4.p, nb, 3, H * W, x4.C, s) != FGDM_OK) return fail(FGDM_ERR_HIP, "layout kernel");
            CHK(conv3(en.conv_in, x4, nullptr, 1, false, Epi{}, &h));
            tfree(x4);
            for (const VDown& lv : en.levels) {
                for (const VRes& r : lv.blocks) { CHK(vres_fwd(r, h, &t)); tfree(h); h = t; }
                if (lv.down) { CHK(conv3(lv.downconv, h, nullptr, FGDM_STRIDE2_PAD_BR, false, Epi{}, &t)); tfree(h); h = t; }
            }
            CHK(vres_fwd(en.mid1, h, &t)); tfree(h); h = t;
            CHK(vattn_fwd(en.attn, h, &t)); tfree(h); h = t;
            CHK(vres_fwd(en.mid2, h, &t)); tfree(h); h = t;
            Tensor g;
            CHK(gnorm(en.norm_out, h, nullptr, 1e-6f, true, &g));
            tfree(h);
            float* h32 = (float*)ar->alloc((size_t)nb * hw * zc2 * sizeof(float));
            if (!h32) return fail(FGDM_ERR_NOMEM, "workspace");
            { Epi e; e.out_kind = OUT_F32; e.out = h32; e.ld_out = zc2; CHK(conv3(en.conv_out, g, nullptr, 1, false, e, nullptr)); }
            tfree(g);
            if (vae_moments(h32, en.qc, moments + (size_t)b0 * zc2 * hw, nb, hw, s) != FGDM_OK) return fail(FGDM_ERR_HIP, "moments kernel");
            ar->release(h32);
        }
        return FGDM_OK;
    }

    int set_hint(int cn, const float* hint, int B, int Hh, int Wh) {
        if (!finalized) return fail(FGDM_ERR_STATE, "weights not finalized");
        if (cn < 0 || cn >= (int)cns.size()) return fail(FGDM_ERR_ARG, "no such ControlNet");
        if ((Hh & 7) || (Wh & 7) || B <= 0) return fail(FGDM_ERR_ARG, "hint size must be a multiple of 8");
        Net& n = cns[cn];
        const int mc = cfg.model_channels, Hl = Hh / 8, Wl = Wh / 8;
        if (n.guided.p && (n.guided.B != B || n.guided.H != Hl || n.guided.W != Wl)) { (void)hipFree(n.guided.p); n.guided.p = nullptr; }
        if (!n.guided.p) {
            n.guided.B = B; n.guided.H = Hl; n.guided.W = Wl; n.guided.C = mc;
            if (hipMalloc(&n.guided.p, n.guided.numel() * sizeof(half_t)) != hipSuccess) return fail(FGDM_ERR_NOMEM, "hipMalloc (hint cache)");
        }
        const int hc = n.hint_convs[0].cin_pad;
        const int chunk = std::max(1, std::min(B, (int)(((size_t)512 << 20) / ((size_t)Hh * Wh * 192 * 2 + 1))));
        for (int b0 = 0; b0 < B; b0 += chunk) {
            const int nb = std::min(chunk, B - b0);
            Tensor cur = talloc(nb, Hh, Wh, hc);
            if (!cur.p) return fail(FGDM_ERR_NOMEM, "workspace");
            if (nchw_f32_to_nhwc_f16(hint + (size_t)b0 * cfg.hint_channels * Hh * Wh, cur.p, nb, cfg.hint_channels, Hh * Wh, hc, s) != FGDM_OK)
                return fail(FGDM_ERR_HIP, "layout kernel");
            for (int k = 0; k < 8; ++k) {
                const int stride = (k == 2 || k == 4 || k == 6) ? 2 : 1;
                Epi e;
                e.act = k < 7 ? ACT_SILU : ACT_NONE;
                Tensor nxt;
                if (k == 7) { e.out = n.guided.p + (size_t)b0 * Hl * Wl * mc; e.ld_out = mc; }
                CHK(conv3(n.hint_convs[k], cur, nullptr, stride, false, e, k == 7 ? nullptr : &nxt));
                tfree(cur);
                cur = nxt;
            }
        }
        return FGDM_OK;
    }
};

static hipStream_t as_stream(void* p) { return (hipStream_t)p; }

struct TmpDev {
    std::vector<void*> ptrs;
    ~TmpDev() { for (void* p : ptrs) (void)hipFree(p); }
    template <typename T> T* up(const std::vector<T>& h) {
        T* d = nullptr;
        if (hipMalloc(&d, std::max<size_t>(h.size() * sizeof(T), 256)) != hipSuccess) return nullptr;
        (void)hipMemcpy(d, h.data(), h.size() * sizeof(T), hipMemcpyHostToDevice);
        ptrs.push_back(d);
        return d;
    }
};
static half_t* g_zero_page() {
    static half_t* z = nullptr;
    if (!z) { if (hipMalloc(&z, 4096) != hipSuccess) return nullptr; (void)hipMemset(z, 0, 4096); }
    return z;
}


static int make_desc(const fgdm_config* cfg, fgdm_engine** out) {
    fgdm_engine* e = new fgdm_engine();
    e->cfg = *cfg;
    const int rc = e->build();
    if (rc != FGDM_OK) { delete e; return rc; }
    *out = e;
    return FGDM_OK;
}

template <typename F> static int scoped_call(fgdm_engine* e, void* stream, F f) {
    e->s = as_stream(stream);
    e->ar = &e->arena;
    e->arena.begin_scope();
    for (auto& a : e->cn_arena) a->begin_scope();
    const int rc = f();
    e->s = as_stream(stream);
    e->ar = &e->arena;
    if (rc != FGDM_OK && e->s2) (void)hipStreamSynchronize(e->s2);
    e->arena.end_scope(rc != FGDM_OK);
    for (auto& a : e->cn_arena) a->end_scope(rc != FGDM_OK);
    return rc;
}

extern "C" {

static std::string g_create_err;

int fgdm_create(const fgdm_config* cfg, int device, fgdm_engine** out) {
    if (!cfg || !out) return FGDM_ERR_ARG;
    fgdm_engine* e = nullptr;
    int rc = make_desc(cfg, &e);
    if (rc != FGDM_OK) { g_create_err = "unsupported configuration"; return rc; }
    e->device = device;
    if (const char* v = getenv("FGDM_LN_FOLD")) e->ln_fold = atoi(v) != 0;
    rc = e->ensure_device();
    if (rc != FGDM_OK) {
        g_create_err = e->err + " [" + hipGetErrorString(hipGetLastError()) + "]";
        delete e;
        return rc;
    }
    if (const char* v = getenv("FGDM_TWIN_STREAMS")) e->twin_streams = atoi(v) != 0;
    if (const char* v = getenv("FGDM_PAIR_LAUNCH")) e->pair_launch = atoi(v) != 0;
    if (const char* v = getenv("FGDM_GROUP_MAX")) e->group_max = std::max(2, std::min(FGDM_MAX_GROUP, atoi(v)));
    if (const char* v = getenv("FGDM_GN_GROUP")) e->gn_group = atoi(v) != 0;
    if (e->twin_streams && !e->cns.empty()) {
        if (hipStreamCreateWithFlags(&e->s2, hipStreamNonBlocking) != hipSuccess ||
            hipEventCreateWithFlags(&e->ev_fork, hipEventDisableTiming) != hipSuccess ||
            hipEventCreateWithFlags(&e->ev_join, hipEventDisableTiming) != hipSuccess) {
            g_create_err = "second stream could not be created";
            delete e;
            return FGDM_ERR_HIP;
        }
    }
    for (size_t c = 0; c < e->cns.size(); ++c) {
        e->cn_arena.emplace_back(new Arena());
        if (e->cfg.workspace_bytes > 0) e->cn_arena.back()->slab_bytes = (size_t)e->cfg.workspace_bytes;
    }
    *out = e;
    return FGDM_OK;
}

void fgdm_destroy(fgdm_engine* e) {
    if (!e) return;
    for (hipEvent_t ev : e->prof.pool) (void)hipEventDestroy(ev);
    for (auto& kv : e->weight_allocs) for (void* p : kv.second) (void)hipFree(p);
    if (e->zero) (void)hipFree(e->zero);
    for (auto& n : e->cns) if (n.guided.p) (void)hipFree(n.guided.p);
    e->drop_context();
    e->drop_adapter_conds();
    if (getenv("FGDM_PAIR_DEBUG") && e->replayed_launches)
        fprintf(stderr, "[fgdm] grouped twin launches: %ld of %ld replayed launches were fused (%ld problems)\n", e->paired_launches, e->replayed_launches, e->paired_problems);
    if (e->s2) { (void)hipStreamSynchronize(e->s2); (void)hipStreamDestroy(e->s2); }
    if (e->ev_fork) (void)hipEventDestroy(e->ev_fork);
    if (e->ev_join) (void)hipEventDestroy(e->ev_join);
    delete e;
}

const char* fgdm_last_error(const fgdm_engine* e) { return e ? e->err.c_str() : g_create_err.c_str(); }

static fgdm_engine* g_desc = nullptr;
static fgdm_config g_desc_cfg;
static fgdm_engine* desc_for(const fgdm_config* cfg) {
    if (g_desc && memcmp(&g_desc_cfg, cfg, sizeof(*cfg)) == 0) return g_desc;
    if (g_desc) { delete g_desc; g_desc = nullptr; }
    if (make_desc(cfg, &g_desc) != FGDM_OK) return nullptr;
    g_desc_cfg = *cfg;
    return g_desc;
}
int fgdm_param_count(const fgdm_config* cfg) {
    if (!cfg) return FGDM_ERR_ARG;
    fgdm_engine* d = desc_for(cfg);
    return d ? (int)d->order.size() : FGDM_ERR_ARG;
}
int fgdm_param_info(const fgdm_config* cfg, int index, char* name, int name_cap, int64_t* shape, int* ndim) {
    if (!cfg || !name || !shape || !ndim) return FGDM_ERR_ARG;
    fgdm_engine* d = desc_for(cfg);
    if (!d || index < 0 || index >= (int)d->order.size()) return FGDM_ERR_ARG;
    const std::string& n = d->order[index];
    if ((int)n.size() + 1 > name_cap) return FGDM_ERR_ARG;
    memcpy(name, n.c_str(), n.size() + 1);
    const auto& sh = d->params[n].shape;
    *ndim = (int)sh.size();
    for (size_t i = 0; i < sh.size(); ++i) shape[i] = sh[i];
    return FGDM_OK;
}

int fgdm_load_tensor(fgdm_engine* e, const char* key, const void* data, int dtype, const int64_t* shape, int ndim) {
    if (!e || !key || !data || !shape) return FGDM_ERR_ARG;
    auto it = e->params.find(key);
    if (it == e->params.end()) return e->fail(FGDM_ERR_ARG, std::string("unknown parameter key: ") + key);
    ParamSlot& ps = it->second;
    if ((int)ps.shape.size() != ndim) return e->fail(FGDM_ERR_ARG, std::string("rank mismatch for ") + key);
    for (int i = 0; i < ndim; ++i)
        if (ps.shape[i] != shape[i]) return e->fail(FGDM_ERR_ARG, std::string("shape mismatch for ") + key);
    const size_t n = ps.numel();
    ps.host.resize(n);
    if (dtype == FGDM_DTYPE_F32) {
        if (hipMemcpy(ps.host.data(), data, n * sizeof(float), hipMemcpyDefault) != hipSuccess) return e->fail(FGDM_ERR_HIP, "hipMemcpy failed");
    } else if (dtype == FGDM_DTYPE_F16) {
        std::vector<half_t> tmp(n);
        if (hipMemcpy(tmp.data(), data, n * sizeof(half_t), hipMemcpyDefault) != hipSuccess) return e->fail(FGDM_ERR_HIP, "hipMemcpy failed");
        for (size_t i = 0; i < n; ++i) ps.host[i] = (float)tmp[i];
    } else {
        return e->fail(FGDM_ERR_ARG, "unsupported dtype");
    }
    ps.loaded = true;
    e->comp_dirty[e->component_of(key)] = true;
    e->finalized = false;
    return FGDM_OK;
}

int fgdm_finalize_weights(fgdm_engine* e) {
    if (!e) return FGDM_ERR_ARG;
    int rc = e->ensure_device();
    if (rc != FGDM_OK) return rc;
    e->drop_context();
    e->drop_adapter_conds();
    for (auto& n : e->cns) if (n.guided.p) { (void)hipFree(n.guided.p); n.guided = Tensor{}; }
    rc = e->repack(e->unet.prefix, [&] { return e->pack_net(e->unet); });
    if (rc != FGDM_OK) return rc;
    for (auto& n : e->cns) { rc = e->repack(n.prefix, [&] { return e->pack_net(n); }); if (rc != FGDM_OK) return rc; }
    if (e->vae.on) { rc = e->repack(e->vae.prefix, [&] { return e->pack_vae(); }); if (rc != FGDM_OK) return rc; }
    if (e->clip.on) { rc = e->repack(e->clip.prefix, [&] { return e->pack_clip(); }); if (rc != FGDM_OK) return rc; }
    e->finalized = true;
    return FGDM_OK;
}

int fgdm_profile_begin(fgdm_engine* e, int stride) {
    if (!e) return FGDM_ERR_ARG;
    e->prof.on = true;
    e->prof.stride = stride > 0 ? stride : 1;
    e->prof.counter = 0;
    e->prof.used = 0;
    e->prof.recs.clear();
    for (int c = 0; c < PC_COUNT; ++c) { e->prof.work[c] = 0; e->prof.bytes[c] = 0; }
    return FGDM_OK;
}
int fgdm_profile_end(fgdm_engine* e, double* out) {
    if (!e || !out) return FGDM_ERR_ARG;
    e->prof.on = false;
    if (hipDeviceSynchronize() != hipSuccess) return e->fail(FGDM_ERR_HIP, "hipDeviceSynchronize failed");
    for (int c = 0; c < PC_COUNT * 4; ++c) out[c] = 0;
    for (auto& r : e->prof.recs) {
        if (!r.e1) continue;
        float ms = 0.f;
        if (hipEventElapsedTime(&ms, e->prof.pool[r.e0], e->prof.pool[r.e1]) != hipSuccess) continue;
        out[r.cls * 4 + 0] += ms;
        out[r.cls * 4 + 1] += 1;
    }
    for (int c = 0; c < PC_COUNT; ++c) { out[c * 4 + 2] = e->prof.work[c]; out[c * 4 + 3] = e->prof.bytes[c]; }
    if (const char* path = getenv("FGDM_PROF_DUMP")) {
        std::map<std::string, std::array<double, 3>> agg;
        for (auto& r : e->prof.recs) {
            if (!r.e1) continue;
            float ms = 0.f;
            if (hipEventElapsedTime(&ms, e->prof.pool[r.e0], e->prof.pool[r.e1]) != hipSuccess) continue;
            auto& a = agg[r.tag];
            a[0] += 1; a[1] += ms; a[2] += r.w;
        }
        if (FILE* f = fopen(path, "w")) {
            for (auto& kv : agg) fprintf(f, "%s\t%.0f\t%.4f\t%.6g\n", kv.first.c_str(), kv.second[0], kv.second[1], kv.second[2]);
            fclose(f);
        }
    }
    return FGDM_OK;
}
int fgdm_workspace_stats(fgdm_engine* e, int64_t* peak_bytes, int64_t* reserved_bytes) {
    if (!e || !peak_bytes || !reserved_bytes) return FGDM_ERR_ARG;
    size_t pk = e->arena.peak, r = 0;
    for (auto& sl : e->arena.slabs) for (auto& b : sl) r += b.sz;
    for (auto& a : e->cn_arena) {
        pk += a->peak;
        for (auto& sl : a->slabs) for (auto& b : sl) r += b.sz;
    }
    *peak_bytes = (int64_t)pk;
    *reserved_bytes = (int64_t)r;
    return FGDM_OK;
// ... 502 lines not shown
```

fgdm_amd/csrc/igemm2.hip:

```cpp
#include "common.h"
#include <algorithm>
#include <type_traits>

#pragma clang diagnostic ignored "-Winline-asm"
#define LDS_AS __attribute__((address_space(3)))
#define GLB_AS __attribute__((address_space(1)))

namespace {

__device__ __forceinline__ void glds16(const void* g, unsigned lds_wave_addr) {
    unsigned keep;
    asm volatile("s_mov_b32 %0, m0\n\ts_mov_b32 m0, %2\n\ts_nop 0\n\tglobal_load_lds_dwordx4 %1, off\n\ts_mov_b32 m0, %0"
                 : "=&s"(keep)
                 : "v"(g), "s"(lds_wave_addr)
                 : "memory", "m0");
}
__device__ __forceinline__ void glds16_m0(const void* g, unsigned lds_wave_addr) {
    asm volatile("s_mov_b32 m0, %1\n\ts_nop 0\n\tglobal_load_lds_dwordx4 %0, off" ::"v"(g), "s"(lds_wave_addr) : "memory", "m0");
}
__device__ __forceinline__ void glds16_sv(unsigned voff, const void* sbase, unsigned lds_wave_addr) {
    asm volatile("s_mov_b32 m0, %2\n\ts_nop 0\n\tglobal_load_lds_dwordx4 %0, %1" ::"v"(voff), "s"(sbase), "s"(lds_wave_addr) : "memory", "m0");
}
__device__ __forceinline__ unsigned lds_addr(const void* p) { return (unsigned)(size_t)(LDS_AS const void*)p; }
__device__ __forceinline__ float ln_scale(float acc, float mean, float rstd, float u) {
// ... 855 lines not shown
            const char* wbase = (const char*)a.Wt + ((size_t)(kt + STAGES - 1) << 6);
            const unsigned lbase = lds0 + (unsigned)((kt + STAGES - 1) & 3) * STAGE_BYTES;
#pragma unroll
            for (int j = 0; j < NI; ++j) {
                __builtin_amdgcn_sched_barrier(0);
                if constexpr (REFILL) {
#pragma unroll
                    for (int p2 = 0; p2 < LPS; ++p2)
                        if (p2 * NI / LPS == j) {
                            if (p2 < LA) glds16_m0(a_ok[p2] ? sbase + a_b0[p2] : (const char*)a.zero, lbase + (unsigned)(wave + p2 * NW) * 1024u);
                            else glds16_sv(b_b[p2 - LA], wbase, lbase + (unsigned)b_lds[p2 - LA]);
                        }
                }
                { const int jn = j + WD; wr[jn % RW] = jn < NI ? rdW(kt, jn) : rdW(kt + 1, jn - NI); }
#pragma unroll
                for (int i = 0; i < MI; ++i)
                    if (i * NI / MI == j) nxt[i] = rdX(kt + 1, i);
#pragma unroll
                for (int i = 0; i < MI; ++i)
                    acc[j][i] = __builtin_amdgcn_mfma_f32_16x16x32_f16(wr[j % RW], cur[i], acc[j][i], 0, 0, 0);
            }
            __builtin_amdgcn_sched_barrier(0);
        };
        {
            const int nr = max(nk - (STAGES - 1), 0);
            int kt = 0;
            for (; kt + 1 < nr; kt += 2) {
                step(std::true_type{}, kt, xa, xb);
                step(std::true_type{}, kt + 1, xb, xa);
            }
            if (kt < nr) {
                step(std::true_type{}, kt, xa, xb);
                ++kt;
#pragma unroll
                for (int i = 0; i < MI; ++i) xa[i] = xb[i];
            }
            if (kt < nk) step(std::false_type{}, kt, xa, xb);
            if (kt + 1 < nk) step(std::false_type{}, kt + 1, xb, xa);
            if (kt + 2 < nk) step(std::false_type{}, kt + 2, xa, xb);
            wait_vmcnt<0>();
        }
        asm volatile("s_waitcnt lgkmcnt(0)" ::: "memory");
        __builtin_amdgcn_s_barrier();
        local += 1;
        const bool more = local < t_count;
        const int m0c = m0, n0c = n0;
        if (more) {
            logical = t_first + local * t_step;
            m0 = (logical / ntn) * BM; n0 = (logical % ntn) * BN;
            setup(m0, n0);
            if (nk > 0) issue_stage(0);
            if (nk > 1) issue_stage(1);
        }
        const float* bias_l = ops + set * OPS_FLOATS, *mr_l = bias_l + BN, *u_l = mr_l + 2 * BM;
        if constexpr (LN) {
            const float* uw = u_l + wn * TN;
#pragma unroll
            for (int j = 0; j < NI; ++j) {
                const f32x4 uq = *(const f32x4*)(uw + j * MS + lq);
#pragma unroll
                for (int i = 0; i < MI; ++i) {
                    const int trow = wm * TM + i * MS + lrow;
                    const float mean = mr_l[2 * trow], rstd = mr_l[2 * trow + 1];
#pragma unroll
                    for (int e = 0; e < 4; ++e) acc[j][i][e] = ln_scale(acc[j][i][e], mean, rstd, uq[e]);
                }
            }
        }
        constexpr int OUT_TN = TN / 2, PITCH = OUT_TN * 2 + 8, CPR = OUT_TN / 8, WB_IT = (32 * CPR + 63) / 64, CST_BYTES = 32 * PITCH;
        static_assert(NW * CST_BYTES <= 2 * STAGE_BYTES, "epilogue staging must fit ring slots 2 and 3");
        char* cst = smem + 2 * STAGE_BYTES + wave * CST_BYTES;
        const int ocol0 = (n0c + wn * TN) >> 1, nvalid = a.N / 2;
        const float* bw = bias_l + wn * TN;
#pragma unroll
        for (int ip = 0; ip < TM / 32; ++ip) {
#pragma unroll
            for (int hf = 0; hf < 2; ++hf) {
                const int i = ip * 2 + hf;
                const int prow = hf * MS + lrow;
#pragma unroll
                for (int j = 0; j < NI; ++j) {
                    if (j & 2) continue;
                    const int wc = j * MS + lq;
                    const f32x4 bq = *(const f32x4*)(bw + wc);
                    float v[4];
#pragma unroll
                    for (int e = 0; e < 4; ++e) v[e] = acc[j][i][e] + bq[e];
                    const f32x4 gq = *(const f32x4*)(bw + wc + 32);
                    const f32x2 g01 = gelu2_f(f32x2{acc[j + 2][i][0] + gq[0], acc[j + 2][i][1] + gq[1]});
                    const f32x2 g23 = gelu2_f(f32x2{acc[j + 2][i][2] + gq[2], acc[j + 2][i][3] + gq[3]});
                    v[0] *= g01[0]; v[1] *= g01[1]; v[2] *= g23[0]; v[3] *= g23[1];
#pragma unroll
                    for (int e = 0; e < 4; ++e) v[e] *= a.scale;
                    const int oc = (j >> 2) * 32 + (j & 1) * 16 + lq;
                    const h4 pk = {(half_t)v[0], (half_t)v[1], (half_t)v[2], (half_t)v[3]};
                    *(h4*)(cst + prow * PITCH + oc * 2) = pk;
                }
            }
            asm volatile("s_waitcnt lgkmcnt(0)" ::: "memory");
#pragma unroll
            for (int it = 0; it < WB_IT; ++it) {
                const int c = lane + it * 64, pr = c / CPR, ck = c - pr * CPR;
                const int grow = m0c + wm * TM + ip * 32 + pr, gcol = ocol0 + ck * 8;
                if (c < 32 * CPR && grow < a.M && gcol < nvalid) {
                    const char* sp = cst + pr * PITCH + ck * 16;
                    const h4 lo = *(const h4*)sp, hi = *(const h4*)(sp + 8);
                    *(h8*)((half_t*)a.out + (size_t)grow * a.ld_out + gcol) = h8{lo[0], lo[1], lo[2], lo[3], hi[0], hi[1], hi[2], hi[3]};
                }
            }
            asm volatile("s_waitcnt lgkmcnt(0)" ::: "memory");
        }
        if (!more) break;
        set ^= 1;
        stage_ops(m0, n0, set, m0 == m0c);
        asm volatile("s_waitcnt lgkmcnt(0)" ::: "memory");
        __builtin_amdgcn_s_barrier();
        if (nk > 2) issue_stage(2);
        first = false;
    }
}

template <bool LN>
int launch_geglu_persist(const IgemmArgs& a, int ntiles, int contiguous, hipStream_t s) {
    constexpr int smem = 4 * (256 + 256) * ROWB + 2 * (256 + 2 * 256 + 256) * 4;
    static_assert(smem <= 160 * 1024, "LDS budget");
    static bool attr_set = false;
    auto k = igemm2_geglu_persist_kernel<LN>;
    if (!attr_set) {
        HIP_TRY(hipFuncSetAttribute((const void*)k, hipFuncAttributeMaxDynamicSharedMemorySize, smem));
        attr_set = true;
    }
    FGDM_LAUNCH(k, dim3(256), dim3(512), smem, s, a, ntiles, contiguous);
    return hipGetLastError() == hipSuccess ? FGDM_OK : FGDM_ERR_HIP;
}

template <int BM, int BN, int WM, int WN, int STAGES, bool CONV, bool GEGLU, bool SPLIT, int MS, bool LN, int PATH, int PIPE, bool ABL>
int launch2p(const IgemmArgs& a, hipStream_t s) {
    constexpr int ring = ring_bytes<BM, BN, STAGES, PIPE>();
    constexpr int smem = ring + (1 + RV_MAX) * BN * 4 + (2 * BM + BN) * 4;
    static_assert(smem <= 160 * 1024, "LDS budget");
    static bool attr_set = false;
    auto k = igemm2_kernel<BM, BN, WM, WN, STAGES, CONV, GEGLU, SPLIT, MS, LN, PATH, PIPE, ABL>;
    if (!attr_set) {
        HIP_TRY(hipFuncSetAttribute((const void*)k, hipFuncAttributeMaxDynamicSharedMemorySize, smem));
        attr_set = true;
    }
    const int ntm = (a.M + BM - 1) / BM, ntn = (a.N + BN - 1) / BN;
    const unsigned gx = (unsigned)(ntm * ntn * (SPLIT ? a.splitk : 1));
    if (fgdm_recording()) {
        auto single = [=](hipStream_t rs) -> int {
            hipLaunchKernelGGL(k, dim3(gx), dim3(WM * WN * 64), smem, rs, a);
            return hipGetLastError() == hipSuccess ? FGDM_OK : FGDM_ERR_HIP;
        };
        if constexpr (PIPE != 0 && PATH != 0 && !SPLIT && !ABL && MS == 16) {
            static bool pair_attr_set = false;
            auto kp = igemm2_pair_kernel<BM, BN, WM, WN, STAGES, CONV, GEGLU, SPLIT, MS, LN, PATH, PIPE, ABL>;
            if (!pair_attr_set) {
                HIP_TRY(hipFuncSetAttribute((const void*)kp, hipFuncAttributeMaxDynamicSharedMemorySize, smem));
                pair_attr_set = true;
            }
            IgemmGroupFn pf = [](const IgemmArgs* const* av, int n, unsigned grid_x, hipStream_t rs) -> int {
                if (n < 2 || n > FGDM_MAX_GROUP) return FGDM_ERR_ARG;
                IgemmArgsG pg;
                for (int i = 0; i < FGDM_MAX_GROUP; ++i) pg.g[i] = *av[i < n ? i : 0];
                hipLaunchKernelGGL((igemm2_pair_kernel<BM, BN, WM, WN, STAGES, CONV, GEGLU, SPLIT, MS, LN, PATH, PIPE, ABL>), dim3(grid_x, n),
                                   dim3(WM * WN * 64), smem, rs, pg);
                return hipGetLastError() == hipSuccess ? FGDM_OK : FGDM_ERR_HIP;
            };
            fgdm_record(single, (const void*)kp, pf, &a, gx);
        } else {
            fgdm_record(single);
        }
        return FGDM_OK;
    }
    hipLaunchKernelGGL(k, dim3(gx), dim3(WM * WN * 64), smem, s, a);
    return hipGetLastError() == hipSuccess ? FGDM_OK : FGDM_ERR_HIP;
}
template <int BM, bool GEGLU, bool LN>
int epilogue_path(const IgemmArgs& a) {
    if (a.out_kind != OUT_F16 || !(a.act == ACT_NONE || GEGLU)) return 0;
    if (a.out2 && a.out_kind2 != OUT_F16) {
        const bool staged = LN && a.out_kind2 == OUT_F16_T && a.rows_per_sample % 32 == 0 && a.M % 32 == 0 && a.ld_out2 % 8 == 0 &&
                            ((size_t)a.out2 & 15) == 0;
        if (!staged || a.rowvec) return 0;
    }
    if (!a.rowvec) return 1;
    return (BM - 1) / a.rows_per_sample + 2 <= RV_MAX ? 2 : 0;
}
template <int BM, int BN, int WM, int WN, int STAGES, bool CONV, bool GEGLU, bool SPLIT, int MS, bool LN, bool FAST, int PIPE>
int launch2(const IgemmArgs& a, hipStream_t s) {
    static const bool fast_on = !(getenv("FGDM_IGEMM_EPI_PATHS") && atoi(getenv("FGDM_IGEMM_EPI_PATHS")) == 0);
    if constexpr (FAST && !SPLIT && !LN) {
        if (a.debug)
            return epilogue_path<BM, GEGLU, LN>(a) == 1 ? launch2p<BM, BN, WM, WN, STAGES, CONV, GEGLU, SPLIT, MS, LN, 1, (PIPE == 2 ? 1 : PIPE), true>(a, s)
                                                        : FGDM_ERR_ARG;
    }
    if (a.debug) return FGDM_ERR_ARG;
    if constexpr (SPLIT) return launch2p<BM, BN, WM, WN, STAGES, CONV, GEGLU, SPLIT, MS, LN, 0, PIPE, false>(a, s);
    if constexpr (FAST && !SPLIT) {
        switch (fast_on ? epilogue_path<BM, GEGLU, LN>(a) : 0) {
            case 1: return launch2p<BM, BN, WM, WN, STAGES, CONV, GEGLU, SPLIT, MS, LN, 1, PIPE, false>(a, s);
            case 2: if constexpr (!GEGLU && !LN) return launch2p<BM, BN, WM, WN, STAGES, CONV, GEGLU, SPLIT, MS, LN, 2, PIPE, false>(a, s);
            default: break;
        }
    }
    return launch2p<BM, BN, WM, WN, STAGES, CONV, GEGLU, SPLIT, MS, LN, 0, 0, false>(a, s);
}
template <int BM, int BN, bool GEGLU, int MS, int PIPE, int WM, int WN>
int launch2m(const IgemmArgs& a, hipStream_t s) {
    constexpr int PL = PIPE == 2 ? 1 : PIPE;
    return a.mode == IG_LINEAR ? launch2<BM, BN, WM, WN, 4, false, GEGLU, false, MS, false, MS == 16, PL>(a, s)
                               : launch2<BM, BN, WM, WN, 4, true, GEGLU, false, MS, false, MS == 16, (GEGLU ? PL : PIPE)>(a, s);
}
template <int BM, int BN, bool GEGLU, int MS, int PIPE, int WM, int WN>
int launch2ln(const IgemmArgs& a, hipStream_t s) {
    return launch2<BM, BN, WM, WN, 4, false, GEGLU, false, MS, true, MS == 16, (PIPE == 2 ? 1 : PIPE)>(a, s);
}
template <int BM, int BN, int MS, int PIPE, int WM = 4, int WN = 2>
int launch_tile(const IgemmArgs& a, hipStream_t s) {
    const bool g = a.act == ACT_GEGLU;
    if (a.ln_stats) {
        if constexpr (BN == 256) { if (g) return launch2ln<BM, BN, true, MS, PIPE, WM, WN>(a, s); }
        if constexpr (BN == 128) return FGDM_ERR_ARG;
        else return launch2ln<BM, BN, false, MS, PIPE, WM, WN>(a, s);
    }
    if constexpr (BN == 256) { if (g) return launch2m<BM, BN, true, MS, PIPE, WM, WN>(a, s); }
    return launch2m<BM, BN, false, MS, PIPE, WM, WN>(a, s);
}

__global__ __launch_bounds__(256) void splitk_reduce_kernel(const IgemmArgs a) {
    const size_t total4 = (size_t)a.M * a.N / 4, plane = (size_t)a.M * a.N;
    for (size_t i = (size_t)blockIdx.x * 256 + threadIdx.x; i < total4; i += (size_t)gridDim.x * 256) {
        const size_t e0 = i * 4;
        const int row = (int)(e0 / a.N), col = (int)(e0 - (size_t)row * a.N);
        f32x4 v = *(const f32x4*)(a.ws + e0);
        for (int s = 1; s < a.splitk; ++s) {
            const f32x4 u = *(const f32x4*)(a.ws + (size_t)s * plane + e0);
            v[0] += u[0]; v[1] += u[1]; v[2] += u[2]; v[3] += u[3];
        }
        h4 r = {(half_t)0, (half_t)0, (half_t)0, (half_t)0};
        if (a.resid) r = *(const h4*)(a.resid + (size_t)row * a.ld_res + col);
        h4 o;
#pragma unroll
        for (int e = 0; e < 4; ++e) {
            float x = v[e] + (a.bias ? a.bias[col + e] : 0.f);
            if (a.rowvec) x += a.rowvec[(size_t)(row / a.rows_per_sample) * a.rv_stride + col + e];
            if (a.act == ACT_SILU) x = silu_f(x);
            else if (a.act == ACT_RELU) x = fmaxf(x, 0.f);
            else if (a.act == ACT_QGELU) x = silu_f(x, 1.702f);
            const half_t y = (half_t)(x * a.scale);
            o[e] = a.resid ? (half_t)((float)y + (float)r[e]) : y;
        }
        *(h4*)((half_t*)a.out + (size_t)row * a.ld_out + col) = o;
    }
}

}

static thread_local bool g_twin_layers = false;
void igemm_set_twin_layers(bool on) { g_twin_layers = on; }

int igemm_splitk_factor(const IgemmArgs& a) {
    if (a.force_cfg || a.act == ACT_GEGLU || a.out_kind != OUT_F16 || a.N % 320 || (a.K & 31)) return 1;
    const int nk = a.K >> 5;
    static const bool fat = !(getenv("FGDM_SPLITK_FAT") && atoi(getenv("FGDM_SPLITK_FAT")) == 0);
    if (fat && a.rows_per_sample > 64 && a.rows_per_sample <= 256 && (nk >= 540 || (nk >= 360 && !g_twin_layers))) return 2;
    if (a.rows_per_sample > 64 || nk < 96) return 1;
    return (fat && nk >= 360) ? 8 : 4;
}
int igemm_splitk_reduce(const IgemmArgs& a, hipStream_t s) {
    const size_t total4 = (size_t)a.M * a.N / 4;
    const int grid = (int)std::min<size_t>(2048, (total4 + 255) / 256);
    FGDM_LAUNCH(splitk_reduce_kernel, dim3(grid), dim3(256), 0, s, a);
    return hipGetLastError() == hipSuccess ? FGDM_OK : FGDM_ERR_HIP;
}

static bool halo_geometry(const IgemmArgs& a) {
    if (a.mode != IG_CONV3 || a.Ho != a.H || a.Wo != a.W || (a.C0 & 63) || (a.C1 & 63) || (a.K % 288) || a.debug) return false;
    if ((a.W == 16 || a.W == 32 || a.W == 64) && (a.H * a.W) % 256 == 0) return true;
    return a.W == 8 && a.H == 8;
}

int igemm2_launch(const IgemmArgs& a, int cfg, hipStream_t s) {
    if ((a.K & 31) || (a.C0 & 31) || (a.C1 & 31)) return FGDM_ERR_ARG;
    static const int pipe_default = getenv("FGDM_IGEMM_PIPE") ? atoi(getenv("FGDM_IGEMM_PIPE")) : 1;
    const int tile = cfg & 15, psel = cfg >> 4;
    const size_t px = a.mode == IG_LINEAR ? (size_t)a.M : (size_t)a.B * a.H * a.W;
    const bool small = px * (size_t)std::max(a.C0, a.C1) * 2 < (1ull << 32) && (size_t)(a.N + 320) * a.K * 2 < (1ull << 32);
    const bool pipe = (psel == 0 ? pipe_default != 0 : psel == 2) && small;
    const int bn = (tile == 1 || tile == 4) ? 256 : tile == 6 ? 128 : tile == 7 ? 160 : 320;
    if (a.N % bn) return FGDM_ERR_ARG;
    if (a.act == ACT_GEGLU && bn != 256) return FGDM_ERR_ARG;
    if (a.splitk > 1) {
        if ((tile != 2 && tile != 0) || a.ln_stats) return FGDM_ERR_ARG;
        static const bool halo_sk = !(getenv("FGDM_IGEMM_HALO") && atoi(getenv("FGDM_IGEMM_HALO")) == 0);
        const int nk_all = a.K >> 5;
        if (halo_sk && pipe && halo_geometry(a) && nk_all % a.splitk == 0 && (nk_all / a.splitk) % 9 == 0)
            return tile == 0 ? launch2<256, 320, 4, 2, 4, true, false, true, 16, false, false, 2>(a, s)
                             : launch2<128, 320, 4, 2, 4, true, false, true, 16, false, false, 2>(a, s);
        if (tile == 0 && pipe)
            return a.mode == IG_LINEAR ? launch2<256, 320, 4, 2, 4, false, false, true, 16, false, false, 1>(a, s)
                                       : launch2<256, 320, 4, 2, 4, true, false, true, 16, false, false, 1>(a, s);
        if (pipe)
            return a.mode == IG_LINEAR ? launch2<128, 320, 4, 2, 4, false, false, true, 16, false, false, 1>(a, s)
                                       : launch2<128, 320, 4, 2, 4, true, false, true, 16, false, false, 1>(a, s);
        return a.mode == IG_LINEAR ? launch2<128, 320, 4, 2, 4, false, false, true, 16, false, false, 0>(a, s)
                                   : launch2<128, 320, 4, 2, 4, true, false, true, 16, false, false, 0>(a, s);
    }
    if (a.ln_stats && a.mode != IG_LINEAR) return FGDM_ERR_ARG;
    static const int persist_mode = getenv("FGDM_IGEMM_PERSIST") ? atoi(getenv("FGDM_IGEMM_PERSIST")) : 1;
    const bool persist_on = persist_mode != 0;
    if (persist_on && tile == 1 && pipe && a.act == ACT_GEGLU && a.mode == IG_LINEAR && !a.C1 && a.out_kind == OUT_F16 && !a.rowvec &&
        !a.resid && !a.out2 && !a.stats_out && !a.debug && a.N % 256 == 0) {
        const int ntiles = ((a.M + 255) / 256) * (a.N / 256);
        if (ntiles > 256) return a.ln_stats ? launch_geglu_persist<true>(a, ntiles, persist_mode == 2, s) : launch_geglu_persist<false>(a, ntiles, persist_mode == 2, s);
    }
    static const bool halo_on = !(getenv("FGDM_IGEMM_HALO") && atoi(getenv("FGDM_IGEMM_HALO")) == 0);
    const bool halo = halo_on && pipe && halo_geometry(a);
    switch (tile) {
        case 0: return halo ? launch_tile<256, 320, 16, 2>(a, s) : pipe ? launch_tile<256, 320, 16, 1>(a, s) : launch_tile<256, 320, 16, 0>(a, s);
        case 1: return pipe ? launch_tile<256, 256, 16, 1>(a, s) : launch_tile<256, 256, 16, 0>(a, s);
        case 2: return halo ? launch_tile<128, 320, 16, 2>(a, s) : pipe ? launch_tile<128, 320, 16, 1>(a, s) : launch_tile<128, 320, 16, 0>(a, s);
        case 3: return launch_tile<256, 320, 32, 0>(a, s);
        case 4: return launch_tile<256, 256, 32, 0>(a, s);
        case 5: return launch_tile<128, 320, 32, 0>(a, s);
        case 6: return pipe ? launch_tile<256, 128, 16, 1>(a, s) : launch_tile<256, 128, 16, 0>(a, s);
        case 7: return a.mode != IG_LINEAR ? FGDM_ERR_ARG : pipe ? launch_tile<64, 160, 16, 1, 2, 2>(a, s) : launch_tile<64, 160, 16, 0, 2, 2>(a, s);
        default: return FGDM_ERR_ARG;
    }
}
```

fgdm_amd/csrc/norm.hip:

```cpp
#include "common.h"
#include <algorithm>
#include <cstdlib>
#include <cstring>

#define GN_PIX_PER_CHUNK 256

__device__ __forceinline__ const half_t* src_octet(const half_t* x0, int C0, const half_t* x1, int C1,
                                                   size_t pix, int o) {
    const int c = o << 3;
    return c < C0 ? x0 + pix * C0 + c : x1 + pix * C1 + (c - C0);
}

__global__ __launch_bounds__(256) void gn_stats_kernel(const half_t* __restrict__ x0, int C0,
                                                        const half_t* __restrict__ x1, int C1, int HW,
                                                        float* __restrict__ partial, int pix_per_chunk) {
    extern __shared__ float red[];
    const int C = C0 + C1, P = C >> 3, cpg = C >> 5;
    const int b = blockIdx.y, chunk = blockIdx.x, nchunk = gridDim.x;
    const int tid = threadIdx.x;
    const int p_begin = chunk * pix_per_chunk;
    const int p_end = min(HW, p_begin + pix_per_chunk);
    const int PI = P <= 256 ? 256 / P : 1;
    const int nslot = P <= 256 ? 1 : 2;
    for (int slot = 0; slot < nslot; ++slot) {
        int o, pi;
        bool active;
        if (P <= 256) { o = tid % P; pi = tid / P; active = pi < PI; }
        else { o = tid + slot * 256; pi = 0; active = o < P; }
        if (active) {
            float s[8], q[8];
#pragma unroll
            for (int e = 0; e < 8; ++e) { s[e] = 0.f; q[e] = 0.f; }
            int p = p_begin + pi;
            for (; p + 3 * PI < p_end; p += 4 * PI) {
                h8 v[4];
#pragma unroll
                for (int u = 0; u < 4; ++u) v[u] = *(const h8*)src_octet(x0, C0, x1, C1, (size_t)b * HW + p + u * PI, o);
#pragma unroll
                for (int u = 0; u < 4; ++u)
#pragma unroll
                    for (int e = 0; e < 8; ++e) { const float f = (float)v[u][e]; s[e] += f; q[e] += f * f; }
            }
            for (; p < p_end; p += PI) {
                const h8 v = *(const h8*)src_octet(x0, C0, x1, C1, (size_t)b * HW + p, o);
#pragma unroll
                for (int e = 0; e < 8; ++e) { const float f = (float)v[e]; s[e] += f; q[e] += f * f; }
            }
#pragma unroll
            for (int e = 0; e < 8; ++e) {
                red[((size_t)pi * C + (o << 3) + e) * 2] = s[e];
                red[((size_t)pi * C + (o << 3) + e) * 2 + 1] = q[e];
            }
        }
    }
    __syncthreads();
    if (tid < 64) {
        const int g = tid >> 1, which = tid & 1;
        float acc = 0.f;
        for (int pi = 0; pi < PI; ++pi)
            for (int c = g * cpg; c < (g + 1) * cpg; ++c) acc += red[((size_t)pi * C + c) * 2 + which];
        partial[((size_t)b * nchunk + chunk) * 64 + tid] = acc;
    }
}

__global__ __launch_bounds__(256) void gn_apply_kernel(const half_t* __restrict__ x0, int C0,
                                                        const half_t* __restrict__ x1, int C1, int HW,
                                                        const float* __restrict__ partial, int nchunk,
                                                        float inv_count, float eps,
                                                        const float* __restrict__ gamma,
                                                        const float* __restrict__ beta, int silu,
                                                        half_t* __restrict__ out) {
    extern __shared__ __attribute__((aligned(16))) float sc[];
    const int C = C0 + C1, P = C >> 3, cpg = C >> 5;
    const int b = blockIdx.y;
    float* scale = sc;
    float* shift = sc + C;
    float* stats = sc + 2 * C;
    {
        const int g = threadIdx.x >> 3, part = threadIdx.x & 7;
        double s = 0.0, q = 0.0;
        for (int c = part; c < nchunk; c += 8) {
            s += (double)partial[((size_t)b * nchunk + c) * 64 + g * 2];
            q += (double)partial[((size_t)b * nchunk + c) * 64 + g * 2 + 1];
        }
#pragma unroll
        for (int off = 4; off > 0; off >>= 1) { s += __shfl_xor(s, off); q += __shfl_xor(q, off); }
        if (part == 0) {
            const double mean = s * inv_count;
            double var = q * inv_count - mean * mean;
            if (var < 0.0) var = 0.0;
            stats[g * 2] = (float)mean;
            stats[g * 2 + 1] = (float)(1.0 / sqrt(var + (double)eps));
        }
    }
    __syncthreads();
    for (int c = threadIdx.x; c < C; c += 256) {
        const int g = c / cpg;
        const float mean = stats[g * 2], rstd = stats[g * 2 + 1];
        const float w = gamma[c] * rstd;
        scale[c] = w;
        shift[c] = beta[c] - mean * w;
    }
    __syncthreads();
    const unsigned total = (unsigned)HW * (unsigned)P;
    for (unsigned i0 = blockIdx.x * 1024u + threadIdx.x; i0 < total; i0 += gridDim.x * 1024u) {
        h8 v[4];
        unsigned pix[4];
        int oct[4];
#pragma unroll
        for (int u = 0; u < 4; ++u) {
            const unsigned i = i0 + (unsigned)u * 256u;
            pix[u] = i / (unsigned)P;
            oct[u] = (int)(i - pix[u] * (unsigned)P);
            if (i < total) v[u] = *(const h8*)src_octet(x0, C0, x1, C1, (size_t)b * HW + pix[u], oct[u]);
        }
#pragma unroll
        for (int u = 0; u < 4; ++u) {
            if (i0 + (unsigned)u * 256u >= total) break;
            h8 r;
            const f32x4 sc0 = *(const f32x4*)(scale + (oct[u] << 3)), sc1 = *(const f32x4*)(scale + (oct[u] << 3) + 4);
            const f32x4 sh0 = *(const f32x4*)(shift + (oct[u] << 3)), sh1 = *(const f32x4*)(shift + (oct[u] << 3) + 4);
#pragma unroll
            for (int e = 0; e < 8; ++e) {
                float f = (float)v[u][e] * (e < 4 ? sc0[e & 3] : sc1[e & 3]) + (e < 4 ? sh0[e & 3] : sh1[e & 3]);
                if (silu) f = silu_f(f);
                r[e] = (half_t)f;
            }
            *(h8*)(out + ((size_t)b * HW + pix[u]) * C + (oct[u] << 3)) = r;
        }
    }
}

struct GnProb { const half_t* x0; const half_t* x1; const float* gamma; const float* beta; half_t* out; };
struct GnArgsG { GnProb p[FGDM_MAX_GROUP]; int C0, C1, B, HW, NG, silu; float eps; };
struct GnRec { GnProb p; int C0, C1, B, HW, NG, silu; float eps; int np_sel; unsigned smem; };
static_assert(sizeof(GnRec) <= FGDM_GROUP_BLOB, "GroupNorm record must fit the recorder's blob");

template <int NT>
__device__ __forceinline__ void gn_fused_body(const half_t* __restrict__ x0, int C0,
                                                        const half_t* __restrict__ x1, int C1, int B, int HW, int NG,
                                                        float eps, const float* __restrict__ gamma,
                                                        const float* __restrict__ beta, int silu,
                                                        half_t* __restrict__ out) {
    extern __shared__ __attribute__((aligned(16))) char gsm[];
    const int C = C0 + C1, cpg = C >> 5, CW = NG * cpg, OW = CW >> 3;
    const int NS = 32 / NG, xcd = blockIdx.x & 7, k = blockIdx.x >> 3;
    const int b = (k / NS) * 8 + xcd, c_lo = (k % NS) * CW;
    if (b >= B) return;
    const int tid = threadIdx.x;
    half_t* tile = (half_t*)gsm;
    float* red = (float*)(gsm + (size_t)HW * CW * 2);
    const int PI = NT / OW;
    float* stats = red + (size_t)PI * CW * 2;
    float* scale = stats + 8;
    float* shift = scale + CW;
    const int o = tid % OW, pi = tid / OW;
    if (pi < PI) {
        float sm[8], sq[8];
#pragma unroll
        for (int e = 0; e < 8; ++e) { sm[e] = 0.f; sq[e] = 0.f; }
        int p = pi;
        for (; p + 7 * PI < HW; p += 8 * PI) {
            h8 v[8];
#pragma unroll
            for (int u = 0; u < 8; ++u) v[u] = *(const h8*)src_octet(x0, C0, x1, C1, (size_t)b * HW + p + u * PI, (c_lo >> 3) + o);
#pragma unroll
            for (int u = 0; u < 8; ++u) {
                *(h8*)(tile + (size_t)(p + u * PI) * CW + (o << 3)) = v[u];
#pragma unroll
                for (int e = 0; e < 8; ++e) { const float f = (float)v[u][e]; sm[e] += f; sq[e] += f * f; }
            }
        }
        for (; p < HW; p += PI) {
            const h8 v = *(const h8*)src_octet(x0, C0, x1, C1, (size_t)b * HW + p, (c_lo >> 3) + o);
            *(h8*)(tile + (size_t)p * CW + (o << 3)) = v;
#pragma unroll
            for (int e = 0; e < 8; ++e) { const float f = (float)v[e]; sm[e] += f; sq[e] += f * f; }
        }
#pragma unroll
        for (int e = 0; e < 8; ++e) {
            red[((size_t)pi * CW + (o << 3) + e) * 2] = sm[e];
            red[((size_t)pi * CW + (o << 3) + e) * 2 + 1] = sq[e];
        }
    }
    __syncthreads();
    for (int i = tid; i < 2 * CW; i += NT) {
        float acc = 0.f;
        for (int l = 0; l < PI; ++l) acc += red[(size_t)l * CW * 2 + i];
        red[i] = acc;
    }
    __syncthreads();
    if (tid < 2 * NG) {
        const int g = tid >> 1, which = tid & 1;
        double acc = 0.0;
        for (int c = g * cpg; c < (g + 1) * cpg; ++c) acc += (double)red[c * 2 + which];
        stats[tid] = (float)(acc / ((double)HW * cpg));
    }
    __syncthreads();
    if (tid < NG) {
        const double mean = stats[2 * tid];
        double var = (double)stats[2 * tid + 1] - mean * mean;
        if (var < 0.0) var = 0.0;
        stats[2 * tid + 1] = (float)(1.0 / sqrt(var + (double)eps));
    }
    __syncthreads();
    for (int c = tid; c < CW; c += NT) {
        const int g = c / cpg;
        const float w = gamma[c_lo + c] * stats[2 * g + 1];
        scale[c] = w;
        shift[c] = beta[c_lo + c] - stats[2 * g] * w;
    }
    __syncthreads();
    const int total = HW * OW;
    for (int i = tid; i < total; i += NT) {
        const int p = i / OW, oo = i - p * OW;
        const h8 v = *(const h8*)(tile + (size_t)p * CW + (oo << 3));
        h8 r;
        const f32x4 sc0 = *(const f32x4*)(scale + (oo << 3)), sc1 = *(const f32x4*)(scale + (oo << 3) + 4);
        const f32x4 sh0 = *(const f32x4*)(shift + (oo << 3)), sh1 = *(const f32x4*)(shift + (oo << 3) + 4);
#pragma unroll
        for (int e = 0; e < 8; ++e) {
            float f = (float)v[e] * (e < 4 ? sc0[e & 3] : sc1[e & 3]) + (e < 4 ? sh0[e & 3] : sh1[e & 3]);
            if (silu) f = silu_f(f);
            r[e] = (half_t)f;
        }
        *(h8*)(out + ((size_t)b * HW + p) * C + c_lo + (oo << 3)) = r;
    }
}

template <int NT>
__global__ __launch_bounds__(NT) void gn_fused_kernel(const half_t* __restrict__ x0, int C0, const half_t* __restrict__ x1, int C1, int B, int HW,
                                                        int NG, float eps, const float* __restrict__ gamma, const float* __restrict__ beta,
                                                        int silu, half_t* __restrict__ out) {
    gn_fused_body<NT>(x0, C0, x1, C1, B, HW, NG, eps, gamma, beta, silu, out);
}
template <int NT>
__global__ __launch_bounds__(NT) void gn_fused_group_kernel(const GnArgsG g) {
    const GnProb& p = g.p[blockIdx.y];
    gn_fused_body<NT>(p.x0, g.C0, p.x1, g.C1, g.B, g.HW, g.NG, g.eps, p.gamma, p.beta, g.silu, p.out);
}

template <int NP>
__device__ __forceinline__ void gn_reg_body(const half_t* __restrict__ x0, int C0,
                                                      const half_t* __restrict__ x1, int C1, int B, int HW, int NG,
                                                      float eps, const float* __restrict__ gamma,
                                                      const float* __restrict__ beta, int silu,
                                                      half_t* __restrict__ out) {
    extern __shared__ __attribute__((aligned(16))) char gsm[];
    const int C = C0 + C1, cpg = C >> 5, CW = NG * cpg, OW = CW >> 3;
    const int NS = 32 / NG, xcd = blockIdx.x & 7, k = blockIdx.x >> 3;
    const int b = (k / NS) * 8 + xcd, c_lo = (k % NS) * CW;
    if (b >= B) return;
    const int tid = threadIdx.x;
    const int PI = 1024 / OW;
    float* red = (float*)gsm;
    float* stats = red + (size_t)PI * CW * 2;
    float* scale = stats + 8;
    float* shift = scale + CW;
    const int o = tid % OW, pi = tid / OW;
    const bool active = pi < PI;
    h8 v[NP];
    if (active) {
#pragma unroll
        for (int u = 0; u < NP; ++u) {
            const int p = pi + u * PI;
            v[u] = (h8)(half_t)0;
            if (p < HW) v[u] = *(const h8*)src_octet(x0, C0, x1, C1, (size_t)b * HW + p, (c_lo >> 3) + o);
        }
        float sm[8], sq[8];
#pragma unroll
        for (int e = 0; e < 8; ++e) { sm[e] = 0.f; sq[e] = 0.f; }
#pragma unroll
        for (int u = 0; u < NP; ++u)
#pragma unroll
            for (int e = 0; e < 8; ++e) { const float f = (float)v[u][e]; sm[e] += f; sq[e] += f * f; }
#pragma unroll
        for (int e = 0; e < 8; ++e) {
            red[((size_t)pi * CW + (o << 3) + e) * 2] = sm[e];
            red[((size_t)pi * CW + (o << 3) + e) * 2 + 1] = sq[e];
        }
    }
    __syncthreads();
    for (int i = tid; i < 2 * CW; i += 1024) {
        float acc = 0.f;
        for (int l = 0; l < PI; ++l) acc += red[(size_t)l * CW * 2 + i];
        stats[8 + 2 * CW + i] = acc;
    }
    __syncthreads();
    const float* tot = stats + 8 + 2 * CW;
    if (tid < 2 * NG) {
        const int g = tid >> 1, which = tid & 1;
        double acc = 0.0;
        for (int c = g * cpg; c < (g + 1) * cpg; ++c) acc += (double)tot[c * 2 + which];
        stats[tid] = (float)(acc / ((double)HW * cpg));
    }
    __syncthreads();
    if (tid < NG) {
        const double mean = stats[2 * tid];
        double var = (double)stats[2 * tid + 1] - mean * mean;
        if (var < 0.0) var = 0.0;
        stats[2 * tid + 1] = (float)(1.0 / sqrt(var + (double)eps));
    }
    __syncthreads();
    for (int c = tid; c < CW; c += 1024) {
        const int g = c / cpg;
        const float w = gamma[c_lo + c] * stats[2 * g + 1];
        scale[c] = w;
        shift[c] = beta[c_lo + c] - stats[2 * g] * w;
    }
    __syncthreads();
    if (active) {
        const f32x4 sc0 = *(const f32x4*)(scale + (o << 3)), sc1 = *(const f32x4*)(scale + (o << 3) + 4);
        const f32x4 sh0 = *(const f32x4*)(shift + (o << 3)), sh1 = *(const f32x4*)(shift + (o << 3) + 4);
#pragma unroll
        for (int u = 0; u < NP; ++u) {
            const int p = pi + u * PI;
            if (p < HW) {
                h8 r;
#pragma unroll
                for (int e = 0; e < 8; ++e) {
                    float f = (float)v[u][e] * (e < 4 ? sc0[e & 3] : sc1[e & 3]) + (e < 4 ? sh0[e & 3] : sh1[e & 3]);
                    if (silu) f = silu_f(f);
                    r[e] = (half_t)f;
                }
                *(h8*)(out + ((size_t)b * HW + p) * C + c_lo + (o << 3)) = r;
            }
        }
    }
}

template <int NP>
__global__ __launch_bounds__(1024) void gn_reg_kernel(const half_t* __restrict__ x0, int C0, const half_t* __restrict__ x1, int C1, int B, int HW,
                                                      int NG, float eps, const float* __restrict__ gamma, const float* __restrict__ beta,
                                                      int silu, half_t* __restrict__ out) {
    gn_reg_body<NP>(x0, C0, x1, C1, B, HW, NG, eps, gamma, beta, silu, out);
}
template <int NP>
__global__ __launch_bounds__(1024) void gn_reg_group_kernel(const GnArgsG g) {
    const GnProb& p = g.p[blockIdx.y];
    gn_reg_body<NP>(p.x0, g.C0, p.x1, g.C1, g.B, g.HW, g.NG, g.eps, p.gamma, p.beta, g.silu, p.out);
}

static unsigned long long gn_shape_hash(const GnRec& r, int kind) {
    unsigned long long h = 1469598103934665603ull;
    const int v[10] = {kind, r.C0, r.C1, r.B, r.HW, r.NG, r.silu, r.np_sel, (int)r.smem, 0};
    for (int i = 0; i < 9; ++i) { h ^= (unsigned)v[i]; h *= 1099511628211ull; }
    unsigned e; memcpy(&e, &r.eps, 4);
    h ^= e; h *= 1099511628211ull;
    return h;
}
static bool gn_same_shape(const GnRec& a, const GnRec& b) {
    return a.C0 == b.C0 && a.C1 == b.C1 && a.B == b.B && a.HW == b.HW && a.NG == b.NG && a.silu == b.silu && a.eps == b.eps &&
           a.np_sel == b.np_sel && a.smem == b.smem;
}
template <typename SingleFn, typename GroupFn>
static int gn_group_dispatch(const void* const* args, int n, unsigned grid_x, hipStream_t s, unsigned block, SingleFn single, GroupFn group) {
    const GnRec& r0 = *(const GnRec*)args[0];
    if (n == 1) return single(r0, grid_x, s);
    bool same = n <= FGDM_MAX_GROUP;
    for (int k = 1; k < n && same; ++k) same = gn_same_shape(r0, *(const GnRec*)args[k]);
    if (!same) {
        for (int k = 0; k < n; ++k) { const int rc = single(*(const GnRec*)args[k], grid_x, s); if (rc != FGDM_OK) return rc; }
        return FGDM_OK;
    }
    GnArgsG g{};
    for (int k = 0; k < n; ++k) g.p[k] = ((const GnRec*)args[k])->p;
    g.C0 = r0.C0; g.C1 = r0.C1; g.B = r0.B; g.HW = r0.HW; g.NG = r0.NG; g.silu = r0.silu; g.eps = r0.eps;
    return group(g, r0, grid_x, (unsigned)n, s);
}
#define GN_SINGLE(KERNEL) [](const GnRec& r, unsigned gx, hipStream_t st) -> int {                                                       \
        hipLaunchKernelGGL(KERNEL, dim3(gx), dim3(GN_BLOCK), r.smem, st, r.p.x0, r.C0, r.p.x1, r.C1, r.B, r.HW, r.NG, r.eps, r.p.gamma,   \
                           r.p.beta, r.silu, r.p.out);                                                                                 \
        return hipGetLastError() == hipSuccess ? FGDM_OK : FGDM_ERR_HIP; }
#define GN_GROUP(KERNEL) [](const GnArgsG& g, const GnRec& r, unsigned gx, unsigned n, hipStream_t st) -> int {                            \
        hipLaunchKernelGGL(KERNEL, dim3(gx, n), dim3(GN_BLOCK), r.smem, st, g);                                                       \
        return hipGetLastError() == hipSuccess ? FGDM_OK : FGDM_ERR_HIP; }
static int gn_group_fn(const void* const* args, int n, unsigned grid_x, hipStream_t s) {
    const int sel = ((const GnRec*)args[0])->np_sel;
    switch (sel) {
#define GN_BLOCK 1024
        case 6: return gn_group_dispatch(args, n, grid_x, s, 1024, GN_SINGLE(gn_reg_kernel<6>), GN_GROUP(gn_reg_group_kernel<6>));
        case 11: return gn_group_dispatch(args, n, grid_x, s, 1024, GN_SINGLE(gn_reg_kernel<11>), GN_GROUP(gn_reg_group_kernel<11>));
        case 16: return gn_group_dispatch(args, n, grid_x, s, 1024, GN_SINGLE(gn_reg_kernel<16>), GN_GROUP(gn_reg_group_kernel<16>));
        case 21: return gn_group_dispatch(args, n, grid_x, s, 1024, GN_SINGLE(gn_reg_kernel<21>), GN_GROUP(gn_reg_group_kernel<21>));
#undef GN_BLOCK
#define GN_BLOCK 256
        case 256: return gn_group_dispatch(args, n, grid_x, s, 256, GN_SINGLE(gn_fused_kernel<256>), GN_GROUP(gn_fused_group_kernel<256>));
#undef GN_BLOCK
#define GN_BLOCK 512
        case 512: return gn_group_dispatch(args, n, grid_x, s, 512, GN_SINGLE(gn_fused_kernel<512>), GN_GROUP(gn_fused_group_kernel<512>));
#undef GN_BLOCK
        default: return FGDM_ERR_ARG;
    }
}
static thread_local bool g_gn_group = true;
void groupnorm_set_group(bool on) { g_gn_group = on; }
static int gn_single_pass_launch(const GnRec& r, unsigned grid_x, hipStream_t s) {
    const void* args[1] = {&r};
    if (!fgdm_recording()) return gn_group_fn(args, 1, grid_x, s);
    const GnRec rc = r;
    fgdm_record_generic([rc, grid_x](hipStream_t rs) -> int { const void* a1[1] = {&rc}; return gn_group_fn(a1, 1, grid_x, rs); },
                        (const void*)&gn_group_fn, g_gn_group ? gn_group_fn : nullptr, &r, sizeof(r), grid_x, gn_shape_hash(r, r.np_sel));
    return FGDM_OK;
}

size_t groupnorm_ws_floats(int B, int HW) {
    const int nchunk = (HW + 63) / 64;
    return (size_t)B * nchunk * 64 + (size_t)B * 64;
}

int groupnorm_launch(const half_t* x0, int C0, const half_t* x1, int C1, int B, int HW, const float* gamma,
                     const float* beta, float eps, int silu, half_t* out, float* ws, hipStream_t s) {
    const int C = C0 + C1;
    if ((C & 31) || (C0 & 7) || (C1 & 7) || C > 4096 || B <= 0 || HW <= 0 || (size_t)HW * (C >> 3) >= (1u << 31)) return FGDM_ERR_ARG;
    auto try_reg = [&]() -> int {
        static const int reg_hw = getenv("FGDM_GN_REG") ? atoi(getenv("FGDM_GN_REG")) : 1024;
        const bool reg_on = HW <= reg_hw;
        const int cpg = C >> 5;
        static const int ng_max = getenv("FGDM_GN_REG_NG") ? atoi(getenv("FGDM_GN_REG_NG")) : 4;
        for (int NG = ng_max; reg_on && NG >= 1; NG >>= 1) {
            const int CW = NG * cpg;
            if (CW & 7) continue;
            const int OW = CW >> 3;
            if (OW < 5 || OW > 64) continue;
            const int PI = 1024 / OW, np = (HW + PI - 1) / PI;
            if (np > 21) continue;
            const size_t smem = ((size_t)PI * CW * 2 + 8 + 2 * (size_t)CW + 2 * (size_t)CW) * sizeof(float);
            if (smem > 150 * 1024) continue;
            static bool attr_set = false;
            if (!attr_set) {
                if (hipFuncSetAttribute((const void*)gn_reg_kernel<6>, hipFuncAttributeMaxDynamicSharedMemorySize, 150 * 1024) != hipSuccess ||
                    hipFuncSetAttribute((const void*)gn_reg_kernel<11>, hipFuncAttributeMaxDynamicSharedMemorySize, 150 * 1024) != hipSuccess ||
                    hipFuncSetAttribute((const void*)gn_reg_kernel<16>, hipFuncAttributeMaxDynamicSharedMemorySize, 150 * 1024) != hipSuccess ||
                    hipFuncSetAttribute((const void*)gn_reg_kernel<21>, hipFuncAttributeMaxDynamicSharedMemorySize, 150 * 1024) != hipSuccess)
                    return FGDM_ERR_HIP;
                attr_set = true;
            }
            static bool attr2_set = false;
            if (!attr2_set) {
                if (hipFuncSetAttribute((const void*)gn_reg_group_kernel<6>, hipFuncAttributeMaxDynamicSharedMemorySize, 150 * 1024) != hipSuccess ||
                    hipFuncSetAttribute((const void*)gn_reg_group_kernel<11>, hipFuncAttributeMaxDynamicSharedMemorySize, 150 * 1024) != hipSuccess ||
                    hipFuncSetAttribute((const void*)gn_reg_group_kernel<16>, hipFuncAttributeMaxDynamicSharedMemorySize, 150 * 1024) != hipSuccess ||
                    hipFuncSetAttribute((const void*)gn_reg_group_kernel<21>, hipFuncAttributeMaxDynamicSharedMemorySize, 150 * 1024) != hipSuccess)
                    return FGDM_ERR_HIP;
                attr2_set = true;
            }
            GnRec r{{x0, x1, gamma, beta, out}, C0, C1, B, HW, NG, silu, eps, np <= 6 ? 6 : np <= 11 ? 11 : np <= 16 ? 16 : 21, (unsigned)smem};
            return gn_single_pass_launch(r, (unsigned)((32 / NG) * 8 * ((B + 7) / 8)), s);
        }
        return 1;
    };
    if ((size_t)HW * C >= 64 * 2560) { const int rc = try_reg(); if (rc != 1) return rc; }
    {
        const int cpg = C >> 5;
        static const int max_kb = getenv("FGDM_GN_FUSED_MAXKB") ? atoi(getenv("FGDM_GN_FUSED_MAXKB")) : 64;
        for (int pass = 0; pass < 2; ++pass)
        for (int NG = 4; NG >= 1; NG >>= 1) {
            const int CW = NG * cpg;
            const size_t slice = (size_t)HW * CW * 2;
            if ((CW & 7) || CW > 320 || slice > (size_t)std::min(pass == 0 ? 40 : 64, max_kb) * 1024) continue;
            const int NT = slice > 40 * 1024 ? 512 : 256;
            const int OW = CW >> 3, PI = NT / OW;
            const size_t smem = slice + ((size_t)PI * CW * 2 + 8 + 2 * (size_t)CW) * sizeof(float);
            if (smem > 150 * 1024) continue;
            static bool attr_set = false;
            if (!attr_set) {
                if (hipFuncSetAttribute((const void*)gn_fused_kernel<256>, hipFuncAttributeMaxDynamicSharedMemorySize, 150 * 1024) != hipSuccess ||
                    hipFuncSetAttribute((const void*)gn_fused_kernel<512>, hipFuncAttributeMaxDynamicSharedMemorySize, 150 * 1024) != hipSuccess)
                    return FGDM_ERR_HIP;
                attr_set = true;
            }
            static bool attr2_set = false;
            if (!attr2_set) {
                if (hipFuncSetAttribute((const void*)gn_fused_group_kernel<256>, hipFuncAttributeMaxDynamicSharedMemorySize, 150 * 1024) != hipSuccess ||
                    hipFuncSetAttribute((const void*)gn_fused_group_kernel<512>, hipFuncAttributeMaxDynamicSharedMemorySize, 150 * 1024) != hipSuccess)
                    return FGDM_ERR_HIP;
                attr2_set = true;
            }
            GnRec r{{x0, x1, gamma, beta, out}, C0, C1, B, HW, NG, silu, eps, NT, (unsigned)smem};
            return gn_single_pass_launch(r, (unsigned)((32 / NG) * 8 * ((B + 7) / 8)), s);
        }
    }
    { const int rc = try_reg(); if (rc != 1) return rc; }
    static const int ppc_env = getenv("FGDM_GN_CHUNK") ? atoi(getenv("FGDM_GN_CHUNK")) : GN_PIX_PER_CHUNK;
    const int ppc = (ppc_env >= 64 && ppc_env % 64 == 0) ? ppc_env : GN_PIX_PER_CHUNK;
    const int nchunk = (HW + ppc - 1) / ppc;
    float* partial = ws;
    const int P = C >> 3, PI = P <= 256 ? 256 / P : 1;
    FGDM_LAUNCH(gn_stats_kernel, dim3(nchunk, B), dim3(256), (size_t)PI * C * 2 * sizeof(float), s, x0, C0, x1,
                       C1, HW, partial, ppc);
    const float inv_count = 1.0f / ((float)HW * (float)(C / 32));
    const size_t total = (size_t)HW * (C >> 3);
    int gx = (int)((total + 1023) / 1024);
    const int cap = 256 / (B < 8 ? B : 8);
    if (gx > cap) gx = cap;
    if (gx < 1) gx = 1;
    FGDM_LAUNCH(gn_apply_kernel, dim3(gx, B), dim3(256), (2 * C + 64) * sizeof(float), s, x0, C0, x1, C1, HW,
                       partial, nchunk, inv_count, eps, gamma, beta, silu, out);
    return hipGetLastError() == hipSuccess ? FGDM_OK : FGDM_ERR_HIP;
}

template <int NO>
__global__ __launch_bounds__(256) void ln_kernel(const half_t* __restrict__ x, int rows, int C,
                                                 const float* __restrict__ gamma, const float* __restrict__ beta,
                                                 float eps, half_t* __restrict__ out) {
    const int lane = threadIdx.x & 63;
    const int row = blockIdx.x * 4 + (threadIdx.x >> 6);
    if (row >= rows) return;
    const int P = C >> 3;
    h8 v[NO];
    float sum = 0.f;
#pragma unroll
    for (int k = 0; k < NO; ++k) {
        const int o = lane + k * 64;
        if (o < P) {
            v[k] = *(const h8*)(x + (size_t)row * C + (o << 3));
#pragma unroll
            for (int e = 0; e < 8; ++e) sum += (float)v[k][e];
        }
    }
#pragma unroll
    for (int off = 32; off > 0; off >>= 1) sum += __shfl_xor(sum, off);
    const float mean = sum / (float)C;
    float sq = 0.f;
#pragma unroll
    for (int k = 0; k < NO; ++k) {
        const int o = lane + k * 64;
        if (o < P) {
#pragma unroll
            for (int e = 0; e < 8; ++e) { const float d = (float)v[k][e] - mean; sq += d * d; }
        }
    }
#pragma unroll
    for (int off = 32; off > 0; off >>= 1) sq += __shfl_xor(sq, off);
    const float rstd = rsqrtf(sq / (float)C + eps);
#pragma unroll
    for (int k = 0; k < NO; ++k) {
        const int o = lane + k * 64;
        if (o < P) {
            h8 r;
#pragma unroll
            for (int e = 0; e < 8; ++e) {
                const int c = (o << 3) + e;
                r[e] = (half_t)(((float)v[k][e] - mean) * rstd * gamma[c] + beta[c]);
            }
            *(h8*)(out + (size_t)row * C + (o << 3)) = r;
        }
    }
}

int layernorm_launch(const half_t* x, int rows, int C, const float* gamma, const float* beta, float eps,
                     half_t* out, hipStream_t s) {
    if ((C & 7) || C > 2048 || rows <= 0) return FGDM_ERR_ARG;
    const dim3 grid((rows + 3) / 4), block(256);
    if (C <= 512) FGDM_LAUNCH(ln_kernel<1>, grid, block, 0, s, x, rows, C, gamma, beta, eps, out);
    else if (C <= 1024) FGDM_LAUNCH(ln_kernel<2>, grid, block, 0, s, x, rows, C, gamma, beta, eps, out);
    else FGDM_LAUNCH(ln_kernel<4>, grid, block, 0, s, x, rows, C, gamma, beta, eps, out);
    return hipGetLastError() == hipSuccess ? FGDM_OK : FGDM_ERR_HIP;
}

template <typename OUT>
__global__ __launch_bounds__(256) void ln32_kernel(const float* __restrict__ x, int rows, int C, const float* __restrict__ gamma,
                                                   const float* __restrict__ beta, float eps, OUT* __restrict__ out) {
    const int lane = threadIdx.x & 63;
    const int row = blockIdx.x * 4 + (threadIdx.x >> 6);
    if (row >= rows) return;
    const float* xr = x + (size_t)row * C;
    float sum = 0.f;
    for (int c = lane * 4; c < C; c += 256) { const f32x4 v = *(const f32x4*)(xr + c); sum += v[0] + v[1] + v[2] + v[3]; }
#pragma unroll
    for (int off = 32; off > 0; off >>= 1) sum += __shfl_xor(sum, off);
    const float mean = sum / (float)C;
    float sq = 0.f;
    for (int c = lane * 4; c < C; c += 256) {
        const f32x4 v = *(const f32x4*)(xr + c);
#pragma unroll
        for (int e = 0; e < 4; ++e) { const float d = v[e] - mean; sq += d * d; }
    }
#pragma unroll
    for (int off = 32; off > 0; off >>= 1) sq += __shfl_xor(sq, off);
    const float rstd = rsqrtf(sq / (float)C + eps);
    for (int c = lane * 4; c < C; c += 256) {
        const f32x4 v = *(const f32x4*)(xr + c);
#pragma unroll
        for (int e = 0; e < 4; ++e) out[(size_t)row * C + c + e] = (OUT)((v[e] - mean) * rstd * gamma[c + e] + beta[c + e]);
    }
}
int layernorm32_launch(const float* x, int rows, int C, const float* gamma, const float* beta, float eps, half_t* out16,
                       float* out32, hipStream_t s) {
    if ((C & 3) || rows <= 0 || (!out16 == !out32)) return FGDM_ERR_ARG;
    const dim3 grid((rows + 3) / 4), block(256);
    if (out16) FGDM_LAUNCH(ln32_kernel<half_t>, grid, block, 0, s, x, rows, C, gamma, beta, eps, out16);
    else FGDM_LAUNCH(ln32_kernel<float>, grid, block, 0, s, x, rows, C, gamma, beta, eps, out32);
    return hipGetLastError() == hipSuccess ? FGDM_OK : FGDM_ERR_HIP;
}

__global__ __launch_bounds__(256) void row_stats_kernel(const half_t* __restrict__ x, int rows, int C, int slots,
                                                        float* __restrict__ stats) {
    const size_t i = (size_t)blockIdx.x * 256 + threadIdx.x;
    if (i >= (size_t)rows * slots) return;
    const size_t row = i / slots;
    const int slot = (int)(i - row * slots), w = C / slots;
    const half_t* p = x + row * C + (size_t)slot * w;
    float sm = 0.f, sq = 0.f;
    for (int k = 0; k < (w >> 3); ++k) {
        const h8 v = *(const h8*)(p + (k << 3));
        float cs = 0.f, cq = 0.f;
#pragma unroll
        for (int e = 0; e < 8; ++e) { const float f = (float)v[e]; cs += f; cq += f * f; }
        sm += cs; sq += cq;
    }
    stats[i * 2] = sm; stats[i * 2 + 1] = sq;
}
int row_stats_slots(int C) { return (C % 160) == 0 ? C / 160 : 1; }
int row_stats_launch(const half_t* x, int rows, int C, float* stats, hipStream_t s) {
    if ((C & 7) || rows <= 0) return FGDM_ERR_ARG;
    const int slots = row_stats_slots(C);
    const size_t n = (size_t)rows * slots;
    FGDM_LAUNCH(row_stats_kernel, dim3((unsigned)((n + 255) / 256)), dim3(256), 0, s, x, rows, C, slots, stats);
    return hipGetLastError() == hipSuccess ? FGDM_OK : FGDM_ERR_HIP;
}
```

Baseline: 8.082.

## Group attention, two-pass GroupNorm and split-K reduce launches across recorded streams

Turns the attention, two-pass GroupNorm and split-K reduce kernels into device bodies with grouped wrappers that index a per-problem argument array by blockIdx. When recording, these ops register generic group functions so the replayer can merge matching launches from parallel recorded lists (such as the CFG and ControlNet branches) into one launch. The replayer also learns to fuse multi-launch profiled units as a whole. This is meant to cut the number of kernel launches and raise occupancy for small grids. In exchange it adds more argument copying and more matching logic, and the grouped kernels can raise register pressure.

```diff
diff --git a/fgdm_amd/csrc/attention.hip b/fgdm_amd/csrc/attention.hip
--- a/fgdm_amd/csrc/attention.hip
+++ b/fgdm_amd/csrc/attention.hip
@@ -7,7 +7,7 @@
 #define ATT_THR 8.0f
 
 template <int D>
-__global__ __launch_bounds__(256) void attn_kernel(const half_t* __restrict__ Q, int ldq,
+__device__ __forceinline__ void attn_body(const half_t* __restrict__ Q, int ldq,
                                                    const half_t* __restrict__ K, int ldk,
                                                    const half_t* __restrict__ Vt, int ldvt,
                                                    half_t* __restrict__ O, int ldo,
@@ -297,7 +297,7 @@
 
 
 template <int D>
-__global__ __launch_bounds__(256) void attn_cross_kernel(const half_t* __restrict__ Q, int ldq,
+__device__ __forceinline__ void attn_cross_body(const half_t* __restrict__ Q, int ldq,
                                                          const half_t* __restrict__ K, int ldk,
                                                          const half_t* __restrict__ Vt, int ldvt,
                                                          half_t* __restrict__ O, int ldo,
@@ -527,7 +527,7 @@
 }
 
 template <int D>
-__global__ __launch_bounds__(512) void attn_pp_kernel(const half_t* __restrict__ Q, int ldq,
+__device__ __forceinline__ void attn_pp_body(const half_t* __restrict__ Q, int ldq,
                                                       const half_t* __restrict__ K, int ldk,
                                                       const half_t* __restrict__ Vt, int ldvt,
                                                       half_t* __restrict__ O, int ldo,
@@ -1098,7 +1098,7 @@
 }
 
 template <int D, int NW, int ABL = 0>
-__global__ __launch_bounds__(NW * 64, D <= 40 ? 2 : 1) void attn_dq32_kernel(const half_t* __restrict__ Q, int ldq,
+__device__ __forceinline__ void attn_dq32_body(const half_t* __restrict__ Q, int ldq,
                                                            const half_t* __restrict__ K, int ldk,
                                                            const half_t* __restrict__ Vt, int ldvt,
                                                            half_t* __restrict__ O, int ldo,
@@ -1372,11 +1372,72 @@
     }
 }
 
+struct AttnArgs {
+    const half_t* Q; const half_t* K; const half_t* Vt; half_t* O;
+    int ldq, ldk, ldvt, ldo, H, T, Tk, cpw;
+    float sl2e;
+};
+struct AttnArgsG { AttnArgs p[FGDM_MAX_GROUP]; };
+static_assert(sizeof(AttnArgs) <= FGDM_GROUP_BLOB, "attention record must fit the recorder's blob");
+#define ATT_SIG const half_t* __restrict__ Q, int ldq, const half_t* __restrict__ K, int ldk, const half_t* __restrict__ Vt, int ldvt, \
+                half_t* __restrict__ O, int ldo, int H, int T, int Tk, float sl2e
+#define ATT_FWD Q, ldq, K, ldk, Vt, ldvt, O, ldo, H, T, Tk, sl2e
+#define ATT_FWD_G(a) a.Q, a.ldq, a.K, a.ldk, a.Vt, a.ldvt, a.O, a.ldo, a.H, a.T, a.Tk, a.sl2e
+
+template <int D>
+__global__ __launch_bounds__(256) void attn_kernel(ATT_SIG) { attn_body<D>(ATT_FWD); }
+template <int D>
+__global__ __launch_bounds__(256) void attn_group_kernel(const AttnArgsG g) { const AttnArgs& a = g.p[blockIdx.y]; attn_body<D>(ATT_FWD_G(a)); }
+template <int D>
+__global__ __launch_bounds__(256) void attn_cross_kernel(ATT_SIG, int cpw) { attn_cross_body<D>(ATT_FWD, cpw); }
+template <int D>
+__global__ __launch_bounds__(256) void attn_cross_group_kernel(const AttnArgsG g) {
+    const AttnArgs& a = g.p[blockIdx.y];
+    attn_cross_body<D>(ATT_FWD_G(a), a.cpw);
+}
+template <int D>
+__global__ __launch_bounds__(512) void attn_pp_kernel(ATT_SIG) { attn_pp_body<D>(ATT_FWD); }
+template <int D>
+__global__ __launch_bounds__(512) void attn_pp_group_kernel(const AttnArgsG g) { const AttnArgs& a = g.p[blockIdx.y]; attn_pp_body<D>(ATT_FWD_G(a)); }
+template <int D, int NW, int ABL = 0>
+__global__ __launch_bounds__(NW * 64, D <= 40 ? 2 : 1) void attn_dq32_kernel(ATT_SIG) { attn_dq32_body<D, NW, ABL>(ATT_FWD); }
+template <int D, int NW>
+__global__ __launch_bounds__(NW * 64, D <= 40 ? 2 : 1) void attn_dq32_group_kernel(const AttnArgsG g) {
+    const AttnArgs& a = g.p[blockIdx.y];
+    attn_dq32_body<D, NW, 0>(ATT_FWD_G(a));
+}
+
+template <void (*GROUP)(AttnArgsG), int NTHR, typename SingleFn>
+static int attn_go(const AttnArgs& a, unsigned grid, hipStream_t s, SingleFn single) {
+    if (!fgdm_recording() || !fgdm_group_ext()) {
+        if (!fgdm_recording()) return single(a, grid, s);
+        fgdm_record([a, grid, single](hipStream_t rs) -> int { return single(a, grid, rs); });
+        return FGDM_OK;
+    }
+    GenericGroupFn gf = [](const void* const* av, int n, unsigned gx, hipStream_t rs) -> int {
+        if (n < 2 || n > FGDM_MAX_GROUP) return FGDM_ERR_ARG;
+        AttnArgsG g;
+        for (int i = 0; i < FGDM_MAX_GROUP; ++i) g.p[i] = *(const AttnArgs*)av[i < n ? i : 0];
+        hipLaunchKernelGGL(GROUP, dim3(gx, n), dim3(NTHR), 0, rs, g);
+        return hipGetLastError() == hipSuccess ? FGDM_OK : FGDM_ERR_HIP;
+    };
+    unsigned long long h = 1469598103934665603ull;
+    const int v[5] = {a.H, a.T, a.Tk, a.cpw, NTHR};
+    for (int i = 0; i < 5; ++i) { h ^= (unsigned)v[i]; h *= 1099511628211ull; }
+    fgdm_record_generic([a, grid, single](hipStream_t rs) -> int { return single(a, grid, rs); }, (const void*)GROUP, gf, &a, sizeof(a),
+                        grid, h);
+    return FGDM_OK;
+}
+#define ATT_SINGLE(KERNEL, NTHR, ...) [](const AttnArgs& a, unsigned gx, hipStream_t st) -> int {                                       \
+        hipLaunchKernelGGL(KERNEL, dim3(gx), dim3(NTHR), 0, st, ATT_FWD_G(a) __VA_ARGS__);                                             \
+        return hipGetLastError() == hipSuccess ? FGDM_OK : FGDM_ERR_HIP; }
+
 int attention_launch(const half_t* Q, int ldq, const half_t* K, int ldk, const half_t* Vt, int ldvt, half_t* O,
                      int ldo, int B, int H, int T, int Tk, int d, int q_prescaled, hipStream_t s) {
     if (B <= 0 || H <= 0 || T <= 0 || Tk <= 0) return FGDM_ERR_ARG;
     if (ldvt < (Tk + 63) / 64 * 64 || (ldvt & 7) || (ldq & 7) || (ldk & 7) || (ldo & 3)) return FGDM_ERR_ARG;
     const float sl2e = q_prescaled ? 1.0f : 1.4426950408889634f / sqrtf((float)d);
+    AttnArgs aa{Q, K, Vt, O, ldq, ldk, ldvt, ldo, H, T, Tk, 0, sl2e};
     static const bool pp_on = !(getenv("FGDM_ATTN_PP") && atoi(getenv("FGDM_ATTN_PP")) == 0);
     static const int dq = getenv("FGDM_ATTN_DQ") ? atoi(getenv("FGDM_ATTN_DQ")) : 3;
     if (dq > 0 && d == 40 && T % 256 == 0 && Tk % 64 == 0 && Tk >= 128 && (size_t)64 * ldk * 2 < (1u << 31) &&
@@ -1394,40 +1455,37 @@
             return hipGetLastError() == hipSuccess ? FGDM_OK : FGDM_ERR_HIP;
         }
         if (dq == 1) FGDM_LAUNCH((attn_dq_kernel<40, 4>), gridq, blockq, 0, s, Q, ldq, K, ldk, Vt, ldvt, O, ldo, H, T, Tk, sl2e);
-        else FGDM_LAUNCH((attn_dq32_kernel<40, 4>), gridq, blockq, 0, s, Q, ldq, K, ldk, Vt, ldvt, O, ldo, H, T, Tk, sl2e);
+        else return attn_go<attn_dq32_group_kernel<40, 4>, 256>(aa, gridq.x, s, ATT_SINGLE((attn_dq32_kernel<40, 4>), 256));
         return hipGetLastError() == hipSuccess ? FGDM_OK : FGDM_ERR_HIP;
     }
     static const int dq80 = getenv("FGDM_ATTN_DQ80") ? atoi(getenv("FGDM_ATTN_DQ80")) : 1;
     if (dq80 > 0 && d == 80 && T % 256 == 0 && Tk % 64 == 0 && Tk >= 128 && (size_t)64 * ldk * 2 < (1u << 31) &&
         (size_t)d * ldvt * 2 < (1u << 31)) {
         const dim3 gridq((T / 256) * H * B), blockq(256);
-        FGDM_LAUNCH((attn_dq32_kernel<80, 4>), gridq, blockq, 0, s, Q, ldq, K, ldk, Vt, ldvt, O, ldo, H, T, Tk, sl2e);
-        return hipGetLastError() == hipSuccess ? FGDM_OK : FGDM_ERR_HIP;
+        return attn_go<attn_dq32_group_kernel<80, 4>, 256>(aa, gridq.x, s, ATT_SINGLE((attn_dq32_kernel<80, 4>), 256));
     }
     if (pp_on && T >= 256 && Tk >= 256 && (d == 40 || d == 80)) {
         const dim3 grid2(((T + 255) / 256) * H * B), block2(512);
-        if (d == 40) FGDM_LAUNCH(attn_pp_kernel<40>, grid2, block2, 0, s, Q, ldq, K, ldk, Vt, ldvt, O, ldo, H, T, Tk, sl2e);
-        else FGDM_LAUNCH(attn_pp_kernel<80>, grid2, block2, 0, s, Q, ldq, K, ldk, Vt, ldvt, O, ldo, H, T, Tk, sl2e);
-        return hipGetLastError() == hipSuccess ? FGDM_OK : FGDM_ERR_HIP;
+        if (d == 40) return attn_go<attn_pp_group_kernel<40>, 512>(aa, grid2.x, s, ATT_SINGLE(attn_pp_kernel<40>, 512));
+        return attn_go<attn_pp_group_kernel<80>, 512>(aa, grid2.x, s, ATT_SINGLE(attn_pp_kernel<80>, 512));
     }
     static const int cross = getenv("FGDM_ATTN_CROSS") ? atoi(getenv("FGDM_ATTN_CROSS")) : 4;
     if (cross > 0 && Tk > 64 && Tk <= 96 && ldvt >= 96 && T >= 128) {
         const int cpw = std::min(cross, T / 128);
         const dim3 gridc(((T + 128 * cpw - 1) / (128 * cpw)) * H * B), blockc(256);
+        aa.cpw = cpw;
         switch (d) {
-            case 40: FGDM_LAUNCH(attn_cross_kernel<40>, gridc, blockc, 0, s, Q, ldq, K, ldk, Vt, ldvt, O, ldo, H, T, Tk, sl2e, cpw); break;
-            case 80: FGDM_LAUNCH(attn_cross_kernel<80>, gridc, blockc, 0, s, Q, ldq, K, ldk, Vt, ldvt, O, ldo, H, T, Tk, sl2e, cpw); break;
-            case 160: FGDM_LAUNCH(attn_cross_kernel<160>, gridc, blockc, 0, s, Q, ldq, K, ldk, Vt, ldvt, O, ldo, H, T, Tk, sl2e, cpw); break;
+            case 40: return attn_go<attn_cross_group_kernel<40>, 256>(aa, gridc.x, s, ATT_SINGLE(attn_cross_kernel<40>, 256, , a.cpw));
+            case 80: return attn_go<attn_cross_group_kernel<80>, 256>(aa, gridc.x, s, ATT_SINGLE(attn_cross_kernel<80>, 256, , a.cpw));
+            case 160: return attn_go<attn_cross_group_kernel<160>, 256>(aa, gridc.x, s, ATT_SINGLE(attn_cross_kernel<160>, 256, , a.cpw));
             default: return FGDM_ERR_ARG;
         }
-        return hipGetLastError() == hipSuccess ? FGDM_OK : FGDM_ERR_HIP;
     }
     const dim3 grid(((T + 127) / 128) * H * B), block(256);
     switch (d) {
-        case 40: FGDM_LAUNCH(attn_kernel<40>, grid, block, 0, s, Q, ldq, K, ldk, Vt, ldvt, O, ldo, H, T, Tk, sl2e); break;
-        case 80: FGDM_LAUNCH(attn_kernel<80>, grid, block, 0, s, Q, ldq, K, ldk, Vt, ldvt, O, ldo, H, T, Tk, sl2e); break;
-        case 160: FGDM_LAUNCH(attn_kernel<160>, grid, block, 0, s, Q, ldq, K, ldk, Vt, ldvt, O, ldo, H, T, Tk, sl2e); break;
+        case 40: return attn_go<attn_group_kernel<40>, 256>(aa, grid.x, s, ATT_SINGLE(attn_kernel<40>, 256));
+        case 80: return attn_go<attn_group_kernel<80>, 256>(aa, grid.x, s, ATT_SINGLE(attn_kernel<80>, 256));
+        case 160: return attn_go<attn_group_kernel<160>, 256>(aa, grid.x, s, ATT_SINGLE(attn_kernel<160>, 256));
         default: return FGDM_ERR_ARG;
     }
-    return hipGetLastError() == hipSuccess ? FGDM_OK : FGDM_ERR_HIP;
 }
diff --git a/fgdm_amd/csrc/common.h b/fgdm_amd/csrc/common.h
--- a/fgdm_amd/csrc/common.h
+++ b/fgdm_amd/csrc/common.h
@@ -151,6 +151,17 @@
 typedef int (*GenericGroupFn)(const void* const* args, int n, unsigned grid_x, hipStream_t s);
 void fgdm_record_generic(std::function<int(hipStream_t)> run, const void* key, GenericGroupFn fn, const void* args, size_t nbytes,
                          unsigned grid_x, unsigned long long shape);
+bool fgdm_group_ext();
+void fgdm_set_group_ext(bool on);
+static inline int fgdm_smem_attr(const void* kernel, int bytes, unsigned long long& done) {
+    int dev = 0;
+    HIP_TRY(hipGetDevice(&dev));
+    const unsigned long long bit = dev < 64 ? 1ull << dev : 0ull;
+    if (bit && (done & bit)) return FGDM_OK;
+    HIP_TRY(hipFuncSetAttribute(kernel, hipFuncAttributeMaxDynamicSharedMemorySize, bytes));
+    done |= bit;
+    return FGDM_OK;
+}
 #define FGDM_LAUNCH(kernel, grid, block, smem, stream, ...)                                                                  \
     do {                                                                                                                     \
         if (fgdm_recording()) {                                                                                              \
diff --git a/fgdm_amd/csrc/engine.hip b/fgdm_amd/csrc/engine.hip
--- a/fgdm_amd/csrc/engine.hip
+++ b/fgdm_amd/csrc/engine.hip
@@ -239,6 +239,9 @@
 }
 
 bool fgdm_recording() { return g_rec != nullptr; }
+static thread_local bool g_group_ext = true;
+bool fgdm_group_ext() { return g_group_ext; }
+void fgdm_set_group_ext(bool on) { g_group_ext = on; }
 void fgdm_record(std::function<int(hipStream_t)> run, const void* pair_key, IgemmGroupFn pair, const IgemmArgs* ia, unsigned grid_x) {
     RecOp o;
     o.run = std::move(run);
@@ -288,6 +291,7 @@
     bool pair_launch = true;
     int group_max = FGDM_MAX_GROUP;
     bool gn_group = true;
+    bool group_ext = true;
     long paired_launches = 0, replayed_launches = 0, paired_problems = 0;
     struct Deferred { const GemmW* w; Tensor src; int idx; float scale; Arena* owner; };
     Prof prof;
@@ -1474,12 +1478,27 @@
             default: ++replayed_launches; return o.run(s);
         }
     }
-    struct Unit { size_t first, last; long launch; };
+    struct Unit { size_t first, last; long launch; int nl; };
+    static bool fusable(const RecOp& o) { return o.kind == RecOp::RUN && (o.pair || o.gfn); }
     static Unit unit_at(std::vector<RecOp>& v, size_t i) {
         if (v[i].kind == RecOp::PROF_BEGIN && i + 2 < v.size() + 0 && v[i + 1].kind == RecOp::RUN && v[i + 2].kind == RecOp::PROF_END)
-            return Unit{i, i + 2, (v[i + 1].pair || v[i + 1].gfn) ? (long)(i + 1) : -1};
-        if (v[i].kind == RecOp::RUN) return Unit{i, i, (v[i].pair || v[i].gfn) ? (long)i : -1};
-        return Unit{i, i, -1};
+            return Unit{i, i + 2, fusable(v[i + 1]) ? (long)(i + 1) : -1, 1};
+        if (v[i].kind == RecOp::PROF_BEGIN) {
+            size_t j = i + 1;
+            while (j < v.size() && fusable(v[j]) && j - i <= FGDM_MAX_GROUP) ++j;
+            if (j > i + 2 && j < v.size() && v[j].kind == RecOp::PROF_END) return Unit{i, j, (long)(i + 1), (int)(j - i - 1)};
+        }
+        if (v[i].kind == RecOp::RUN) return Unit{i, i, fusable(v[i]) ? (long)i : -1, 1};
+        return Unit{i, i, -1, 0};
+    }
+    static bool same_launches(const std::vector<RecOp>& A, const Unit& ua, const std::vector<RecOp>& B, const Unit& ub) {
+        if (ub.launch < 0 || ub.nl != ua.nl) return false;
+        for (int j = 0; j < ua.nl; ++j) {
+            const RecOp& a = A[ua.launch + j];
+            const RecOp& b = B[ub.launch + j];
+            if (b.pair_key != a.pair_key || b.grid_x != a.grid_x || b.gshape != a.gshape) return false;
+        }
+        return true;
     }
     int run_unit(std::vector<RecOp>& v, const Unit& u) {
         for (size_t k = u.first; k <= u.last; ++k) CHK(run_op(v[k]));
@@ -1507,8 +1526,7 @@
                         size_t jj = at[m];
                         for (int d = 0; d < LOOK && jj < B.size(); ++d) {
                             const Unit u = unit_at(B, jj);
-                            if (u.launch >= 0 && B[u.launch].pair_key == A[ua.launch].pair_key && B[u.launch].grid_x == A[ua.launch].grid_x &&
-                                B[u.launch].gshape == A[ua.launch].gshape) {
+                            if (same_launches(A, ua, B, u)) {
                                 who[n] = m; un[n++] = u;
                                 break;
                             }
@@ -1521,21 +1539,27 @@
                     std::vector<RecOp>& B = *L[who[k]];
                     while (at[who[k]] < un[k].first) { const Unit u = unit_at(B, at[who[k]]); CHK(run_unit(B, u)); at[who[k]] = u.last + 1; }
                 }
-                const IgemmArgs* av[FGDM_MAX_GROUP];
-                const void* gv[FGDM_MAX_GROUP];
                 double w = 0.0, bytes = 0.0;
                 const RecOp* br = nullptr;
                 for (int k = 0; k < n; ++k) {
                     std::vector<RecOp>& B = *L[who[k]];
-                    av[k] = &B[un[k].launch].ia;
-                    gv[k] = B[un[k].launch].gargs;
                     if (un[k].first != un[k].last) { w += B[un[k].first].w; bytes += B[un[k].first].bytes; if (!br) br = &B[un[k].first]; }
                 }
                 if (br) prof.begin(br->cls, s, w, br->tag, bytes);
-                if (A[ua.launch].pair) CHK(A[ua.launch].pair(av, n, A[ua.launch].grid_x, s));
-                else CHK(A[ua.launch].gfn(gv, n, A[ua.launch].grid_x, s));
+                for (int j = 0; j < ua.nl; ++j) {
+                    const IgemmArgs* av[FGDM_MAX_GROUP];
+                    const void* gv[FGDM_MAX_GROUP];
+                    for (int k = 0; k < n; ++k) {
+                        std::vector<RecOp>& B = *L[who[k]];
+                        av[k] = &B[un[k].launch + j].ia;
+                        gv[k] = B[un[k].launch + j].gargs;
+                    }
+                    const RecOp& a = A[ua.launch + j];
+                    if (a.pair) CHK(a.pair(av, n, a.grid_x, s));
+                    else CHK(a.gfn(gv, n, a.grid_x, s));
+                    ++paired_launches; ++replayed_launches; paired_problems += n;
+                }
                 if (br) prof.end(s);
-                ++paired_launches; ++replayed_launches; paired_problems += n;
                 for (int k = 0; k < n; ++k) at[who[k]] = un[k].last + 1;
             }
         }
@@ -1663,6 +1687,7 @@
             static const bool fat = !(getenv("FGDM_PAIR_FAT_TILES") && atoi(getenv("FGDM_PAIR_FAT_TILES")) == 0);
             if (fat) igemm_set_pair_hint(std::min<int>(group_max, 1 + (int)cns.size()));
             groupnorm_set_group(gn_group);
+            fgdm_set_group_ext(group_ext);
             int rc = FGDM_OK;
             for (size_t c = 0; c < cns.size() && rc == FGDM_OK; ++c) {
                 ar = cn_arena[c].get();
@@ -2020,6 +2045,7 @@
     if (const char* v = getenv("FGDM_PAIR_LAUNCH")) e->pair_launch = atoi(v) != 0;
     if (const char* v = getenv("FGDM_GROUP_MAX")) e->group_max = std::max(2, std::min(FGDM_MAX_GROUP, atoi(v)));
     if (const char* v = getenv("FGDM_GN_GROUP")) e->gn_group = atoi(v) != 0;
+    if (const char* v = getenv("FGDM_GROUP_EXT")) e->group_ext = atoi(v) != 0;
     if (e->twin_streams && !e->cns.empty()) {
         if (hipStreamCreateWithFlags(&e->s2, hipStreamNonBlocking) != hipSuccess ||
             hipEventCreateWithFlags(&e->ev_fork, hipEventDisableTiming) != hipSuccess ||
diff --git a/fgdm_amd/csrc/igemm2.hip b/fgdm_amd/csrc/igemm2.hip
--- a/fgdm_amd/csrc/igemm2.hip
+++ b/fgdm_amd/csrc/igemm2.hip
@@ -1031,13 +1031,13 @@
             hipLaunchKernelGGL(k, dim3(gx), dim3(WM * WN * 64), smem, rs, a);
             return hipGetLastError() == hipSuccess ? FGDM_OK : FGDM_ERR_HIP;
         };
-        if constexpr (PIPE != 0 && PATH != 0 && !SPLIT && !ABL && MS == 16) {
-            static bool pair_attr_set = false;
+        constexpr bool pairable = PIPE != 0 && !ABL && MS == 16 && (SPLIT ? PATH == 0 : PATH != 0);
+        if constexpr (pairable) {
+            if (SPLIT && !fgdm_group_ext()) { fgdm_record(single); return FGDM_OK; }
+            static unsigned long long pair_attr_dev = 0;
             auto kp = igemm2_pair_kernel<BM, BN, WM, WN, STAGES, CONV, GEGLU, SPLIT, MS, LN, PATH, PIPE, ABL>;
-            if (!pair_attr_set) {
-                HIP_TRY(hipFuncSetAttribute((const void*)kp, hipFuncAttributeMaxDynamicSharedMemorySize, smem));
-                pair_attr_set = true;
-            }
+            const int rc = fgdm_smem_attr((const void*)kp, smem, pair_attr_dev);
+            if (rc != FGDM_OK) return rc;
             IgemmGroupFn pf = [](const IgemmArgs* const* av, int n, unsigned grid_x, hipStream_t rs) -> int {
                 if (n < 2 || n > FGDM_MAX_GROUP) return FGDM_ERR_ARG;
                 IgemmArgsG pg;
@@ -1107,7 +1107,7 @@
     return launch2m<BM, BN, false, MS, PIPE, WM, WN>(a, s);
 }
 
-__global__ __launch_bounds__(256) void splitk_reduce_kernel(const IgemmArgs a) {
+__device__ __forceinline__ void splitk_reduce_body(const IgemmArgs& a) {
     const size_t total4 = (size_t)a.M * a.N / 4, plane = (size_t)a.M * a.N;
     for (size_t i = (size_t)blockIdx.x * 256 + threadIdx.x; i < total4; i += (size_t)gridDim.x * 256) {
         const size_t e0 = i * 4;
@@ -1133,6 +1133,8 @@
         *(h4*)((half_t*)a.out + (size_t)row * a.ld_out + col) = o;
     }
 }
+__global__ __launch_bounds__(256) void splitk_reduce_kernel(const IgemmArgs a) { splitk_reduce_body(a); }
+__global__ __launch_bounds__(256) void splitk_reduce_group_kernel(const IgemmArgsG p) { splitk_reduce_body(p.g[blockIdx.y]); }
 
 }
 
@@ -1150,6 +1152,20 @@
 int igemm_splitk_reduce(const IgemmArgs& a, hipStream_t s) {
     const size_t total4 = (size_t)a.M * a.N / 4;
     const int grid = (int)std::min<size_t>(2048, (total4 + 255) / 256);
+    if (fgdm_recording() && fgdm_group_ext()) {
+        IgemmGroupFn pf = [](const IgemmArgs* const* av, int n, unsigned grid_x, hipStream_t rs) -> int {
+            if (n < 2 || n > FGDM_MAX_GROUP) return FGDM_ERR_ARG;
+            IgemmArgsG pg;
+            for (int i = 0; i < FGDM_MAX_GROUP; ++i) pg.g[i] = *av[i < n ? i : 0];
+            hipLaunchKernelGGL(splitk_reduce_group_kernel, dim3(grid_x, n), dim3(256), 0, rs, pg);
+            return hipGetLastError() == hipSuccess ? FGDM_OK : FGDM_ERR_HIP;
+        };
+        fgdm_record([=](hipStream_t rs) -> int {
+            hipLaunchKernelGGL(splitk_reduce_kernel, dim3(grid), dim3(256), 0, rs, a);
+            return hipGetLastError() == hipSuccess ? FGDM_OK : FGDM_ERR_HIP;
+        }, (const void*)splitk_reduce_group_kernel, pf, &a, (unsigned)grid);
+        return FGDM_OK;
+    }
     FGDM_LAUNCH(splitk_reduce_kernel, dim3(grid), dim3(256), 0, s, a);
     return hipGetLastError() == hipSuccess ? FGDM_OK : FGDM_ERR_HIP;
 }
diff --git a/fgdm_amd/csrc/norm.hip b/fgdm_amd/csrc/norm.hip
--- a/fgdm_amd/csrc/norm.hip
+++ b/fgdm_amd/csrc/norm.hip
@@ -11,7 +11,7 @@
     return c < C0 ? x0 + pix * C0 + c : x1 + pix * C1 + (c - C0);
 }
 
-__global__ __launch_bounds__(256) void gn_stats_kernel(const half_t* __restrict__ x0, int C0,
+__device__ __forceinline__ void gn_stats_body(const half_t* __restrict__ x0, int C0,
                                                         const half_t* __restrict__ x1, int C1, int HW,
                                                         float* __restrict__ partial, int pix_per_chunk) {
     extern __shared__ float red[];
@@ -63,7 +63,7 @@
     }
 }
 
-__global__ __launch_bounds__(256) void gn_apply_kernel(const half_t* __restrict__ x0, int C0,
+__device__ __forceinline__ void gn_apply_body(const half_t* __restrict__ x0, int C0,
                                                         const half_t* __restrict__ x1, int C1, int HW,
                                                         const float* __restrict__ partial, int nchunk,
                                                         float inv_count, float eps,
@@ -129,6 +129,33 @@
             *(h8*)(out + ((size_t)b * HW + pix[u]) * C + (oct[u] << 3)) = r;
         }
     }
+}
+
+__global__ __launch_bounds__(256) void gn_stats_kernel(const half_t* __restrict__ x0, int C0,
+                                                        const half_t* __restrict__ x1, int C1, int HW,
+                                                        float* __restrict__ partial, int pix_per_chunk) {
+    gn_stats_body(x0, C0, x1, C1, HW, partial, pix_per_chunk);
+}
+__global__ __launch_bounds__(256) void gn_apply_kernel(const half_t* __restrict__ x0, int C0,
+                                                        const half_t* __restrict__ x1, int C1, int HW,
+                                                        const float* __restrict__ partial, int nchunk,
+                                                        float inv_count, float eps,
+                                                        const float* __restrict__ gamma,
+                                                        const float* __restrict__ beta, int silu,
+                                                        half_t* __restrict__ out) {
+    gn_apply_body(x0, C0, x1, C1, HW, partial, nchunk, inv_count, eps, gamma, beta, silu, out);
+}
+struct Gn2Prob { const half_t* x0; const half_t* x1; float* partial; const float* gamma; const float* beta; half_t* out;
+                 int C0, C1, HW, B, ppc_or_nchunk, silu; float inv_count, eps; unsigned smem; };
+struct Gn2ArgsG { Gn2Prob p[FGDM_MAX_GROUP]; };
+static_assert(sizeof(Gn2Prob) <= FGDM_GROUP_BLOB, "two-pass GroupNorm record must fit the recorder's blob");
+__global__ __launch_bounds__(256) void gn_stats_group_kernel(const Gn2ArgsG g) {
+    const Gn2Prob& p = g.p[blockIdx.z];
+    gn_stats_body(p.x0, p.C0, p.x1, p.C1, p.HW, p.partial, p.ppc_or_nchunk);
+}
+__global__ __launch_bounds__(256) void gn_apply_group_kernel(const Gn2ArgsG g) {
+    const Gn2Prob& p = g.p[blockIdx.z];
+    gn_apply_body(p.x0, p.C0, p.x1, p.C1, p.HW, p.partial, p.ppc_or_nchunk, p.inv_count, p.eps, p.gamma, p.beta, p.silu, p.out);
 }
 
 struct GnProb { const half_t* x0; const half_t* x1; const float* gamma; const float* beta; half_t* out; };
@@ -402,6 +429,31 @@
     fgdm_record_generic([rc, grid_x](hipStream_t rs) -> int { const void* a1[1] = {&rc}; return gn_group_fn(a1, 1, grid_x, rs); },
                         (const void*)&gn_group_fn, g_gn_group ? gn_group_fn : nullptr, &r, sizeof(r), grid_x, gn_shape_hash(r, r.np_sel));
     return FGDM_OK;
+}
+
+static unsigned long long gn2_shape_hash(const Gn2Prob& r, int kind) {
+    unsigned long long h = 1469598103934665603ull;
+    unsigned e, ic;
+    memcpy(&e, &r.eps, 4); memcpy(&ic, &r.inv_count, 4);
+    const unsigned v[10] = {(unsigned)kind, (unsigned)r.C0, (unsigned)r.C1, (unsigned)r.HW, (unsigned)r.B, (unsigned)r.ppc_or_nchunk,
+                            (unsigned)r.silu, r.smem, e, ic};
+    for (int i = 0; i < 10; ++i) { h ^= v[i]; h *= 1099511628211ull; }
+    return h;
+}
+template <int KIND>
+static int gn2_group_fn(const void* const* args, int n, unsigned grid_x, hipStream_t s) {
+    if (n < 2 || n > FGDM_MAX_GROUP) return FGDM_ERR_ARG;
+    const Gn2Prob& r0 = *(const Gn2Prob*)args[0];
+    Gn2ArgsG g{};
+    for (int k = 0; k < n; ++k) {
+        g.p[k] = *(const Gn2Prob*)args[k];
+        const Gn2Prob& r = g.p[k];
+        if (r.C0 != r0.C0 || r.C1 != r0.C1 || r.HW != r0.HW || r.B != r0.B || r.ppc_or_nchunk != r0.ppc_or_nchunk || r.smem != r0.smem)
+            return FGDM_ERR_ARG;
+    }
+    if (KIND == 0) hipLaunchKernelGGL(gn_stats_group_kernel, dim3(grid_x, r0.B, n), dim3(256), r0.smem, s, g);
+    else hipLaunchKernelGGL(gn_apply_group_kernel, dim3(grid_x, r0.B, n), dim3(256), r0.smem, s, g);
+    return hipGetLastError() == hipSuccess ? FGDM_OK : FGDM_ERR_HIP;
 }
 
 size_t groupnorm_ws_floats(int B, int HW) {
@@ -487,14 +539,35 @@
     const int nchunk = (HW + ppc - 1) / ppc;
     float* partial = ws;
     const int P = C >> 3, PI = P <= 256 ? 256 / P : 1;
-    FGDM_LAUNCH(gn_stats_kernel, dim3(nchunk, B), dim3(256), (size_t)PI * C * 2 * sizeof(float), s, x0, C0, x1,
-                       C1, HW, partial, ppc);
+    const bool grouped = fgdm_recording() && fgdm_group_ext();
     const float inv_count = 1.0f / ((float)HW * (float)(C / 32));
+    if (grouped) {
+        const Gn2Prob r{x0, x1, partial, gamma, beta, out, C0, C1, HW, B, ppc, silu, inv_count, eps,
+                        (unsigned)((size_t)PI * C * 2 * sizeof(float))};
+        fgdm_record_generic([r, nchunk](hipStream_t rs) -> int {
+            hipLaunchKernelGGL(gn_stats_kernel, dim3(nchunk, r.B), dim3(256), r.smem, rs, r.x0, r.C0, r.x1, r.C1, r.HW, r.partial,
+                               r.ppc_or_nchunk);
+            return hipGetLastError() == hipSuccess ? FGDM_OK : FGDM_ERR_HIP;
+        }, (const void*)gn_stats_group_kernel, gn2_group_fn<0>, &r, sizeof(r), (unsigned)nchunk, gn2_shape_hash(r, 0));
+    } else {
+        FGDM_LAUNCH(gn_stats_kernel, dim3(nchunk, B), dim3(256), (size_t)PI * C * 2 * sizeof(float), s, x0, C0, x1,
+                           C1, HW, partial, ppc);
+    }
     const size_t total = (size_t)HW * (C >> 3);
     int gx = (int)((total + 1023) / 1024);
     const int cap = 256 / (B < 8 ? B : 8);
     if (gx > cap) gx = cap;
     if (gx < 1) gx = 1;
+    if (grouped) {
+        const Gn2Prob r{x0, x1, partial, gamma, beta, out, C0, C1, HW, B, nchunk, silu, inv_count, eps,
+                        (unsigned)((2 * C + 64) * sizeof(float))};
+        fgdm_record_generic([r, gx](hipStream_t rs) -> int {
+            hipLaunchKernelGGL(gn_apply_kernel, dim3(gx, r.B), dim3(256), r.smem, rs, r.x0, r.C0, r.x1, r.C1, r.HW, r.partial,
+                               r.ppc_or_nchunk, r.inv_count, r.eps, r.gamma, r.beta, r.silu, r.out);
+            return hipGetLastError() == hipSuccess ? FGDM_OK : FGDM_ERR_HIP;
+        }, (const void*)gn_apply_group_kernel, gn2_group_fn<1>, &r, sizeof(r), (unsigned)gx, gn2_shape_hash(r, 1));
+        return FGDM_OK;
+    }
     FGDM_LAUNCH(gn_apply_kernel, dim3(gx, B), dim3(256), (2 * C + 64) * sizeof(float), s, x0, C0, x1, C1, HW,
                        partial, nchunk, inv_count, eps, gamma, beta, silu, out);
     return hipGetLastError() == hipSuccess ? FGDM_OK : FGDM_ERR_HIP;
```

Result: no change. 8.125 (median of 6 runs) (+0.5%).
